# RayforceDB/rayforce

Measured on AMD Instinct MI355X. Metric: rows/s on filter→group-by→sum, 1e9-row i64/f64; % HBM roofline at 1/2/4/8 GPU, higher is better.
Workload: dtype f64

## Files before the change

### include/rfx_hip.h

```cpp
#ifndef RFX_HIP_H
#define RFX_HIP_H

#ifndef __HIPCC_RTC__
#include <stddef.h>
#endif
#include <stdint.h>

#ifdef __cplusplus
extern "C" {
#endif
#ifndef __HIPCC_RTC__
#pragma GCC visibility push(default)
#endif

enum {
    RFX_OK = 0,
    RFX_ENODEV = -1,
    RFX_EINVAL = -2,
    RFX_ENOMEM = -3,
    RFX_EHIP = -4,
    RFX_ELIMIT = -5,
    RFX_ESTATE = -6
};

enum { RFX_B8 = 1, RFX_I64 = 5, RFX_F64 = 10 };

enum { RFX_EQ = 0, RFX_NE = 1, RFX_LT = 2, RFX_GT = 3, RFX_LE = 4, RFX_GE = 5 };

enum { RFX_AND = 0, RFX_OR = 1 };

enum {
    RFX_AGG_SUM = 0,
    RFX_AGG_MIN = 1,
    RFX_AGG_MAX = 2,
    RFX_AGG_COUNT = 3,
    RFX_AGG_AVG = 4,
    RFX_AGG_FIRST = 5
};

#define RFX_MAX_PREDS 8
#define RFX_MAX_AGGS 8
#define RFX_MAX_COLS 8
#define RFX_MAX_KEYS 8
#define RFX_MAX_EXPRS 4

#define RFX_PRED_TREE 256
#define RFX_PRED_LEAF(depth, close) (RFX_PRED_TREE | (depth) | ((close) << 4))
typedef struct rfx_pred {
    const void *d_col;
    const void *d_rhs_col;
    int32_t col_type;
    int32_t rhs_type;
    int32_t op;
    int32_t more;
    union {
        int64_t rhs_i;
        double rhs_f;
    };
} rfx_pred_t;

enum { RFX_X_NONE = 0, RFX_X_ADD = 1, RFX_X_SUB = 2, RFX_X_MUL = 3, RFX_X_FDIV = 4, RFX_X_DIV = 5, RFX_X_MOD = 6 };
#define RFX_XOP_RESULT_F64(op, l_f64, r_f64) ((op) == RFX_X_FDIV ? 1 : ((op) == RFX_X_DIV ? ((l_f64) != 0) : ((l_f64) || (r_f64))))
enum { RFX_XF_SWAP = 1 };

#define RFX_MAX_XNODES 4
enum { RFX_XK_COL = 0, RFX_XK_ATOM = 1, RFX_XK_NODE = 2 };
typedef struct rfx_xoperand {
    int32_t kind;
    int32_t type;
    const void *d_col;
    union {
        int64_t i;
        double f;
        int64_t node;
    };
} rfx_xoperand_t;
typedef struct rfx_xnode {
    int32_t op;
    int32_t _pad;
    rfx_xoperand_t l, r;
} rfx_xnode_t;

typedef struct rfx_agg {
    const void *d_col;
    int32_t col_type;
    int32_t kind;
    int32_t xop;
    int32_t xflags;
    const void *d_xrhs_col;
    int32_t xrhs_type;
    int32_t nxnodes;
    union {
        int64_t xrhs_i;
        double xrhs_f;
    };
    const rfx_xnode_t *xnodes;
} rfx_agg_t;
int rfx_agg_input_type(const rfx_agg_t *a);

typedef struct rfx_partial {
    int64_t isum;
    double fsum;
    int64_t cnt;
    int64_t ext;
    int64_t pos;
    int64_t _rsv[3];
} rfx_partial_t;

typedef struct rfx_value {
    int32_t type;
    int32_t is_null;
    union {
        int64_t i;
        double f;
    };
} rfx_value_t;

typedef struct rfx_ctx rfx_ctx_t;

int rfx_hip_device_count(void);
const char *rfx_hip_last_error(void);
const char *rfx_hip_version(void);
#define RFX_STREAM_LEGACY ((void *)(uintptr_t)1)
int rfx_hip_ctx_create(int device, void *stream, rfx_ctx_t **out);
int rfx_hip_ctx_destroy(rfx_ctx_t *ctx);
int rfx_hip_ctx_sync(rfx_ctx_t *ctx);
int rfx_hip_ctx_set_stream(rfx_ctx_t *ctx, void *stream);
enum {
    RFX_TUNE_NO_LDS_TABLES = 1,
    RFX_TUNE_NO_PARTITION = 2,
    RFX_TUNE_NO_BIG_LDS = 4,
    RFX_TUNE_PART_3WG = 8,
    RFX_TUNE_NO_WRITE_COMBINE = 16,
    RFX_TUNE_DIRECT_WC = 32,
    RFX_TUNE_FUSED_KEYS = 64,
    RFX_TUNE_NO_FUSED_SCOPE = 128,
    RFX_TUNE_NO_SOA_WC = 2048,
    RFX_TUNE_NO_LDS_SPLIT = 1024,
    RFX_TUNE_NO_EMIT_WC = 512,
    RFX_TUNE_NO_SEL_COMPACT = 256,
    RFX_TUNE_NO_DEEP_GROUP = 4096,
    RFX_TUNE_NO_LDS_REPLICAS = 8192,
    RFX_TUNE_NO_CHUNK = 16384,
    RFX_TUNE_CHUNK_SMALL = 32768,
    RFX_TUNE_CHUNK_CONTIG = 65536,
    RFX_TUNE_CHUNK_QUEUE = 131072,
    RFX_TUNE_CHUNK_BINS = 262144,
    RFX_TUNE_NO_RTC = 524288,
    RFX_TUNE_NO_PLANE = 1048576,
    RFX_TUNE_NO_WHERE_ONCE = 2097152
};
int rfx_hip_ctx_tune(rfx_ctx_t *ctx, int blocks_per_cu, int flags);
enum {
    RFX_STAT_PLANE_SCATTER = 0,
    RFX_STAT_PLANE_FALLBACK = 1,
    RFX_STAT_PLANE_AGGREGATE = 2,
    RFX_STAT_CHUNK_SCATTER = 3,
    RFX_STAT_CHUNK_AGGREGATE = 4,
    RFX_STAT_MASK_PASSES = 5,
    RFX_STAT_WHERE_ONCE = 6
};
int64_t rfx_hip_ctx_stat(rfx_ctx_t *ctx, int which);

int rfx_hip_malloc(rfx_ctx_t *ctx, void **d_ptr, size_t bytes);
int rfx_hip_free(rfx_ctx_t *ctx, void *d_ptr);
int rfx_hip_ctx_trim(rfx_ctx_t *ctx);
int rfx_hip_h2d(rfx_ctx_t *ctx, void *d_dst, const void *src, size_t bytes);
int rfx_hip_d2h(rfx_ctx_t *ctx, void *dst, const void *d_src, size_t bytes);
int rfx_hip_d2h_async(rfx_ctx_t *ctx, void *dst, const void *d_src, size_t bytes);
int rfx_hip_memset(rfx_ctx_t *ctx, void *d_dst, int byte, size_t bytes);
int rfx_hip_fill_i64(rfx_ctx_t *ctx, int64_t *d_dst, int64_t n, int64_t value);
void rfx_hip_rtc_stats(int64_t *launches, int64_t *compiles);
void rfx_hip_rtc_cache_stats(int64_t *loaded_from_disk, int64_t *written_to_disk);
int rfx_hip_rtc_prewarm_filter_aggr(const rfx_pred_t *preds, int npred, int logic, const rfx_agg_t *aggs, int nagg);
int rfx_hip_rtc_prewarm_where(const rfx_pred_t *preds, int npred, int logic);

int rfx_hip_h2d_pipelined(rfx_ctx_t *ctx, void *d_dst, const void *src, size_t bytes);
int rfx_hip_d2h_pipelined(rfx_ctx_t *ctx, void *dst, const void *d_src, size_t bytes);
int rfx_column_file_stat(const char *path, int32_t *type, int64_t *len);
int rfx_hip_column_file_load(rfx_ctx_t *ctx, const char *path, void *d_dst, int64_t nrows);
int rfx_hip_widen_i32(rfx_ctx_t *ctx, const int32_t *d_in, int64_t n, int64_t *d_out);
int rfx_hip_widen_b8(rfx_ctx_t *ctx, const int8_t *d_in, int64_t n, int64_t *d_out);

int rfx_hip_timer_start(rfx_ctx_t *ctx);
int rfx_hip_timer_stop(rfx_ctx_t *ctx, float *ms);
int rfx_hip_ctx_profile(rfx_ctx_t *ctx, int enable);
int rfx_hip_last_kernel_ms(rfx_ctx_t *ctx, float *ms);
int rfx_hip_profile_kernels(rfx_ctx_t *ctx, float *ms, int cap, int *n);

int rfx_hip_gen_i64(rfx_ctx_t *ctx, int64_t *d_out, int64_t n, uint64_t seed, int64_t row0, uint64_t modulus);
int rfx_hip_gen_f64(rfx_ctx_t *ctx, double *d_out, int64_t n, uint64_t seed, int64_t row0);

int rfx_hip_filter_aggr(rfx_ctx_t *ctx, const rfx_pred_t *preds, int npred, int logic, const rfx_agg_t *aggs,
                        int nagg, int64_t nrows, int64_t row0, rfx_partial_t *d_out);
void rfx_partial_merge(int kind, int col_type, rfx_partial_t *into, const rfx_partial_t *from);
void rfx_partial_identity(rfx_partial_t *p);
int rfx_agg_finalize(int kind, int col_type, const rfx_partial_t *p, rfx_value_t *out);
int rfx_hip_filter_aggr_host(rfx_ctx_t *ctx, const rfx_pred_t *preds, int npred, int logic, const rfx_agg_t *aggs,
                             int nagg, int64_t nrows, rfx_value_t *values, int64_t *selected);

int rfx_hip_cmp_mask(rfx_ctx_t *ctx, const rfx_pred_t *pred, int64_t nrows, int8_t *d_mask);
int rfx_hip_mask_logic(rfx_ctx_t *ctx, int logic, int8_t *d_acc, const int8_t *d_next, int scalar, int64_t nrows);

int rfx_hip_where_begin(rfx_ctx_t *ctx, const rfx_pred_t *preds, int npred, int logic, const int8_t *d_mask,
                        int64_t nrows, int64_t *count);
int rfx_hip_where_emit(rfx_ctx_t *ctx, int64_t row0, int64_t *d_ids);
int rfx_hip_where_estimate(rfx_ctx_t *ctx, const rfx_pred_t *preds, int npred, int logic, int64_t nrows, int64_t *upper);
int rfx_hip_where_once(rfx_ctx_t *ctx, const rfx_pred_t *preds, int npred, int logic, int64_t nrows, int64_t row0, int64_t *d_ids,
                       int64_t cap, int64_t *count);

int rfx_hip_gather(rfx_ctx_t *ctx, const void *d_col, const int64_t *d_ids, int64_t m, void *d_out);
int rfx_hip_gather_many(rfx_ctx_t *ctx, const void *const *d_cols, int ncols, const int64_t *d_ids, int64_t m, void *const *d_outs);
int rfx_hip_gather_checked(rfx_ctx_t *ctx, const void *d_col, int64_t col_len, int32_t col_type, const int64_t *d_ids, int64_t m, void *d_out);

int rfx_hip_scope_i64(rfx_ctx_t *ctx, const int64_t *d_key, const rfx_pred_t *preds, int npred, int logic,
                      int64_t nrows, int64_t *min, int64_t *max, int64_t *count);

int rfx_hip_group_scope(rfx_ctx_t *ctx, const int64_t *d_key, const rfx_pred_t *preds, int npred, int logic,
                        const rfx_agg_t *aggs, int nagg, int64_t nrows, int64_t *min, int64_t *max, int64_t *count);

typedef struct rfx_group_tables {
    int64_t kmin;
    int64_t range;
    int32_t nagg;
    int32_t _pad;
    int64_t *d_first;
    void *d_acc[RFX_MAX_AGGS];
    int64_t *d_cnt[RFX_MAX_AGGS];
} rfx_group_tables_t;

int rfx_hip_group_table_arrays(const rfx_agg_t *aggs, int nagg, int *n_arrays);
int rfx_hip_group_tables_init(rfx_ctx_t *ctx, const rfx_agg_t *aggs, const rfx_group_tables_t *t);
int rfx_hip_group_dense_accumulate(rfx_ctx_t *ctx, const int64_t *d_key, const rfx_pred_t *preds, int npred,
                                   int logic, const rfx_agg_t *aggs, int64_t nrows, int64_t row0,
                                   const rfx_group_tables_t *t);
int rfx_hip_group_rank(rfx_ctx_t *ctx, const rfx_group_tables_t *t, int64_t total_rows, int64_t *ngroups);
#define RFX_SCOPE_SAMPLE_ROWS (1 << 18)
#define RFX_SCOPE_SAMPLE_MAX_RANGE 16384
int rfx_hip_scope_sample_i64(rfx_ctx_t *ctx, const int64_t *d_key, int64_t nrows, int64_t *min, int64_t *max);
int rfx_hip_ctx_speculative(rfx_ctx_t *ctx, int on);
int rfx_hip_group_out_of_scope(rfx_ctx_t *ctx, int *violated);
#define RFX_RANK_SMALL 2048
int rfx_hip_group_rank_emit_small(rfx_ctx_t *ctx, const rfx_agg_t *aggs, const rfx_group_tables_t *t, int64_t row0, int64_t local_rows, int64_t *d_block);
int rfx_hip_group_emit(rfx_ctx_t *ctx, const rfx_agg_t *aggs, const rfx_group_tables_t *t, int64_t *d_keys,
                       int64_t *d_first_ids, void *const *d_results);
int rfx_hip_group_emit_sharded(rfx_ctx_t *ctx, const rfx_agg_t *aggs, const rfx_group_tables_t *t, int64_t row0, int64_t local_rows,
                               int64_t *d_keys, int64_t *d_first_ids, void *const *d_results);
#define RFX_RANK_EMIT_MAX (1 << 22)
#define RFX_SLICE_G0(g, i, nsl) ((int64_t)(i) * ((g) / (nsl)) + ((int64_t)(i) < (g) % (nsl) ? (int64_t)(i) : (g) % (nsl)))
#define RFX_SLICE_GN(g, i, nsl) ((g) / (nsl) + ((int64_t)(i) < (g) % (nsl) ? 1 : 0))
int rfx_hip_group_rank_emit(rfx_ctx_t *ctx, const rfx_agg_t *aggs, const rfx_group_tables_t *t, int64_t total_rows, int64_t row0, int64_t local_rows,
                            int nsl, int si, int64_t out_cap, int64_t *d_keys, int64_t *d_first_ids, void *const *d_results, int64_t *ngroups);
int rfx_hip_ctx_emit_window(rfx_ctx_t *ctx, int64_t g0, int64_t n);

typedef struct rfx_hash_tables {
    int64_t capacity;
    int32_t nagg;
    int32_t _pad;
    int64_t *d_keys;
    int64_t *d_first;
    void *d_acc[RFX_MAX_AGGS];
    int64_t *d_cnt[RFX_MAX_AGGS];
} rfx_hash_tables_t;
int rfx_hip_hash_tables_init(rfx_ctx_t *ctx, const rfx_agg_t *aggs, const rfx_hash_tables_t *t);
int rfx_hip_group_hash_accumulate(rfx_ctx_t *ctx, const int64_t *d_key, const rfx_pred_t *preds, int npred, int logic,
                                  const rfx_agg_t *aggs, int64_t nrows, int64_t row0, const rfx_hash_tables_t *t);
int rfx_hip_group_hash_accumulate_slots(rfx_ctx_t *ctx, const int64_t *d_key, const rfx_pred_t *preds, int npred, int logic, const rfx_agg_t *aggs, int64_t nrows,
                                        int64_t row0, const rfx_hash_tables_t *t, int64_t *d_row_slots, int *recorded);
int rfx_hip_hash_slot_first(rfx_ctx_t *ctx, const rfx_hash_tables_t *t, const int64_t *d_row_slots, int64_t nrows, int64_t *d_ids);
int rfx_hip_hash_tables_init_packed(rfx_ctx_t *ctx, const rfx_agg_t *aggs, const rfx_hash_tables_t *t, int stride);
int rfx_hip_group_hash_accumulate_packed(rfx_ctx_t *ctx, const int64_t *d_key, const rfx_pred_t *preds, int npred, int logic, const rfx_agg_t *aggs, int64_t nrows,
                                         int64_t row0, const rfx_hash_tables_t *t, int stride, int64_t *d_row_slots);
int rfx_hip_hash_tables_merge(rfx_ctx_t *ctx, const rfx_agg_t *aggs, const rfx_hash_tables_t *into,
                              const rfx_hash_tables_t *from);
int rfx_hip_hash_rank(rfx_ctx_t *ctx, const rfx_hash_tables_t *t, int64_t total_rows, int64_t *ngroups);
int rfx_hip_hash_emit(rfx_ctx_t *ctx, const rfx_agg_t *aggs, const rfx_hash_tables_t *t, int64_t *d_keys,
                      int64_t *d_first_ids, void *const *d_results);
int rfx_hip_hash_emit_sharded(rfx_ctx_t *ctx, const rfx_agg_t *aggs, const rfx_hash_tables_t *t, int64_t row0, int64_t local_rows,
                              int64_t *d_keys, int64_t *d_first_ids, void *const *d_results);
int rfx_hip_hash_rows_begin(rfx_ctx_t *ctx, const int64_t *d_probe_first, int64_t nrows, int64_t *ngroups);
int rfx_hip_hash_rows_emit(rfx_ctx_t *ctx, const rfx_agg_t *aggs, const rfx_hash_tables_t *t, const int64_t *d_row_slots, const int64_t *d_row_keys, int64_t row0,
                           int64_t local_rows, int64_t ngroups, int64_t *d_keys, int64_t *d_first_ids, void *const *d_results);
int rfx_hip_hash_rank_emit(rfx_ctx_t *ctx, const rfx_agg_t *aggs, const rfx_hash_tables_t *t, int64_t total_rows, int64_t row0, int64_t local_rows,
                           int nsl, int si, int64_t out_cap, int64_t *d_keys, int64_t *d_first_ids, void *const *d_results, int64_t *ngroups);

int rfx_hip_group_ids_dense(rfx_ctx_t *ctx, const int64_t *d_key, int64_t nrows, const rfx_group_tables_t *t,
                            int64_t *d_gids);
int rfx_hip_group_ids_table(rfx_ctx_t *ctx, const int64_t *d_key, int64_t nrows, int64_t kmin, int64_t range, const int64_t *d_table, int64_t *d_gids);

int rfx_hip_group_ids_first(rfx_ctx_t *ctx, const int64_t *d_probe_first, int64_t nrows, const int64_t *d_first, int64_t groups, int64_t *d_gids);
int rfx_hip_group_slot_ids(rfx_ctx_t *ctx, const rfx_group_tables_t *t, int64_t *d_out);

int rfx_composite_plan(const int64_t *mins, const int64_t *maxs, int nkeys, int64_t *mults, int64_t *total_max);
int rfx_hip_composite_key(rfx_ctx_t *ctx, const void *const *d_cols, const int64_t *mins, const int64_t *mults, int nkeys,
                          int64_t nrows, int64_t *d_out);
int rfx_hip_composite_decode(rfx_ctx_t *ctx, const int64_t *d_comp, int64_t n, int64_t min, int64_t mult, int64_t range,
                             int64_t *d_out);
int rfx_hip_group_dense_accumulate_keys(rfx_ctx_t *ctx, const void *const *d_keys, const int64_t *mins, const int64_t *mults,
                                        int nkeys, const rfx_pred_t *preds, int npred, int logic, const rfx_agg_t *aggs,
                                        int64_t nrows, int64_t row0, const rfx_group_tables_t *t);

int rfx_hip_row_hash(rfx_ctx_t *ctx, const void *const *d_cols, int nkeys, int64_t nrows, int value_first, int64_t *d_out);
int rfx_hip_replace_null_i64(rfx_ctx_t *ctx, const int64_t *d_col, int64_t nrows, int64_t repl, int64_t *d_out);
int rfx_hip_replace_i64(rfx_ctx_t *ctx, const int64_t *d_col, int64_t nrows, int64_t from, int64_t to, int64_t *d_out);

int rfx_hip_eval_expr(rfx_ctx_t *ctx, const rfx_agg_t *expr, int64_t nrows, void *d_out, int32_t *out_type);

int rfx_hip_join_probe_dense(rfx_ctx_t *ctx, const int64_t *d_left_keys, int64_t nleft, int64_t kmin, int64_t range, const int64_t *d_first,
                             int64_t *d_ids);
int rfx_hip_join_probe_hash(rfx_ctx_t *ctx, const int64_t *d_left_keys, int64_t nleft, const rfx_hash_tables_t *t, int64_t *d_ids);
int rfx_hip_join_probe_hash_slots(rfx_ctx_t *ctx, const int64_t *d_left_keys, int64_t nleft, const rfx_hash_tables_t *t, int64_t *d_ids, int64_t *d_slots);
int rfx_hip_tuple_check(rfx_ctx_t *ctx, const void *const *d_keys, int nk, const int64_t *d_first_of_row, int64_t nrows, int64_t *differ);
int rfx_hip_gather_or(rfx_ctx_t *ctx, const void *d_right, const void *d_left, const int64_t *d_ids, int64_t n, uint64_t fill_bits, void *d_out);

#define RFX_DIST_ID_BYTES 128
int rfx_dist_unique_id(void *id128);
int rfx_dist_init(rfx_ctx_t *ctx, int world, int rank, const void *id128);
int rfx_dist_finalize(rfx_ctx_t *ctx);
int rfx_dist_world(rfx_ctx_t *ctx, int *world, int *rank);
int rfx_dist_scope(rfx_ctx_t *ctx, int64_t *kmin, int64_t *kmax, int64_t *seen);
int rfx_dist_group_tables_allreduce(rfx_ctx_t *ctx, const rfx_agg_t *aggs, const rfx_group_tables_t *t);
int rfx_dist_partials_allgather(rfx_ctx_t *ctx, const rfx_partial_t *d_local, int n, rfx_partial_t *d_all);
int rfx_dist_filter_aggr_host(rfx_ctx_t *ctx, const rfx_pred_t *preds, int npred, int logic, const rfx_agg_t *aggs, int nagg,
                              int64_t nrows, int64_t row0, rfx_value_t *values, int64_t *selected);
int rfx_dist_allreduce_i64(rfx_ctx_t *ctx, int64_t *d_buf, int64_t n, int op);
int rfx_dist_allgather(rfx_ctx_t *ctx, const void *d_in, size_t bytes, void *d_out);
int64_t rfx_dist_calls(rfx_ctx_t *ctx);

// ... 52 lines not shown
```

### rayforce_amd/_lib.py

```python
from __future__ import annotations

import ctypes as C
import os

RFX_OK = 0
RFX_ELIMIT = -5
RFX_ESTATE = -6
RFX_B8, RFX_I64, RFX_F64 = 1, 5, 10
RFX_EQ, RFX_NE, RFX_LT, RFX_GT, RFX_LE, RFX_GE = range(6)
RFX_AND, RFX_OR = 0, 1
RFX_AGG_SUM, RFX_AGG_MIN, RFX_AGG_MAX, RFX_AGG_COUNT, RFX_AGG_AVG, RFX_AGG_FIRST = range(6)
RFX_MAX_PREDS = RFX_MAX_AGGS = RFX_MAX_COLS = RFX_MAX_KEYS = 8
RFX_RANK_SMALL = 2048
RFX_MAX_EXPRS = 4
NULL_I64 = -(2**63)
INF_I64 = 2**63 - 1

OPS = {"==": RFX_EQ, "!=": RFX_NE, "<": RFX_LT, ">": RFX_GT, "<=": RFX_LE, ">=": RFX_GE}
AGGS = {"sum": RFX_AGG_SUM, "min": RFX_AGG_MIN, "max": RFX_AGG_MAX, "count": RFX_AGG_COUNT, "avg": RFX_AGG_AVG,
        "first": RFX_AGG_FIRST}


class RfxError(RuntimeError):
    pass
# ... 7 lines not shown
    _anonymous_ = ("u",)
    _fields_ = [("d_col", C.c_void_p), ("d_rhs_col", C.c_void_p), ("col_type", C.c_int32), ("rhs_type", C.c_int32),
                ("op", C.c_int32), ("more", C.c_int32), ("u", _RhsUnion)]


class _XRhsUnion(C.Union):
    _fields_ = [("xrhs_i", C.c_int64), ("xrhs_f", C.c_double)]


class _XOpUnion(C.Union):
    _fields_ = [("i", C.c_int64), ("f", C.c_double), ("node", C.c_int64)]


class XOperand(C.Structure):
    _anonymous_ = ("u",)
    _fields_ = [("kind", C.c_int32), ("type", C.c_int32), ("d_col", C.c_void_p), ("u", _XOpUnion)]


class XNode(C.Structure):
    _fields_ = [("op", C.c_int32), ("_pad", C.c_int32), ("l", XOperand), ("r", XOperand)]


class Agg(C.Structure):
    _anonymous_ = ("xu",)
    _fields_ = [("d_col", C.c_void_p), ("col_type", C.c_int32), ("kind", C.c_int32), ("xop", C.c_int32), ("xflags", C.c_int32),
                ("d_xrhs_col", C.c_void_p), ("xrhs_type", C.c_int32), ("nxnodes", C.c_int32), ("xu", _XRhsUnion), ("xnodes", C.POINTER(XNode))]


RFX_XK_COL, RFX_XK_ATOM, RFX_XK_NODE = 0, 1, 2
RFX_MAX_XNODES = 4
XOPS = {"+": 1, "-": 2, "*": 3, "div": 4, "/": 5, "%": 6}
RFX_XF_SWAP = 1


def agg_input_type(a: "Agg") -> int:
    if a.xop == 0 and a.nxnodes == 0:
        return a.col_type
    return load_library().rfx_agg_input_type(C.byref(a))


class Partial(C.Structure):
    _fields_ = [("isum", C.c_int64), ("fsum", C.c_double), ("cnt", C.c_int64), ("ext", C.c_int64), ("pos", C.c_int64),
                ("_rsv", C.c_int64 * 3)]


class _ValUnion(C.Union):
    _fields_ = [("i", C.c_int64), ("f", C.c_double)]


RFX_MED_GROUPED, RFX_MED_SCALAR = 0, 1


class MedRows(C.Structure):
    _fields_ = [("preds", C.c_void_p), ("npred", C.c_int32), ("logic", C.c_int32), ("d_mask", C.c_void_p), ("d_gids", C.c_void_p),
                ("d_key", C.c_void_p), ("d_table", C.c_void_p), ("kmin", C.c_int64), ("range", C.c_int64)]


class Value(C.Structure):
    _anonymous_ = ("u",)
    _fields_ = [("type", C.c_int32), ("is_null", C.c_int32), ("u", _ValUnion)]


class GroupTables(C.Structure):
    _fields_ = [("kmin", C.c_int64), ("range", C.c_int64), ("nagg", C.c_int32), ("_pad", C.c_int32),
                ("d_first", C.c_void_p), ("d_acc", C.c_void_p * RFX_MAX_AGGS), ("d_cnt", C.c_void_p * RFX_MAX_AGGS)]


class HashTables(C.Structure):
    _fields_ = [("capacity", C.c_int64), ("nagg", C.c_int32), ("_pad", C.c_int32), ("d_keys", C.c_void_p),
                ("d_first", C.c_void_p), ("d_acc", C.c_void_p * RFX_MAX_AGGS), ("d_cnt", C.c_void_p * RFX_MAX_AGGS)]


assert C.sizeof(Pred) == 40 and C.sizeof(Agg) == 56 and C.sizeof(XNode) == 56 and C.sizeof(Partial) == 64 and C.sizeof(Value) == 16

RFX_MAX_SHARDS = 16
RFX_EXEC_MAX_AGGS = 32
RFX_PRED_TREE = 256
RFX_Q_NO_SAMPLED_SCOPE, RFX_Q_REFUSE_NULL_KEY, RFX_Q_WANT_FIRST, RFX_Q_NO_SMALL, RFX_Q_PROBE_FIRST, RFX_Q_SLICED = 1, 2, 4, 8, 16, 32
RFX_PATH_DENSE, RFX_PATH_DENSE_SMALL, RFX_PATH_HASH, RFX_PATH_ROWHASH = 1, 2, 3, 4
RFX_XSTAT_SCOPE_SAMPLED, RFX_XSTAT_SCOPE_RETRIED, RFX_XSTAT_SCOPE_REMEMBERED, RFX_XSTAT_HASH_GROWN, RFX_XSTAT_MERGES_KERNEL, RFX_XSTAT_MERGES_RCCL, \
    RFX_XSTAT_MERGES_TRANSPORT, RFX_XSTAT_QUERIES, RFX_XSTAT_SLICED, RFX_XSTAT_NS_SCOPE, RFX_XSTAT_NS_PASS, RFX_XSTAT_NS_MERGE, RFX_XSTAT_NS_RANK, \
    RFX_XSTAT_NS_EMIT, RFX_XSTAT_NS_FETCH, RFX_XSTAT_NS_TOTAL = range(16)
RFX_XSTAT_PHASES = (("scope", 9), ("pass", 10), ("merge", 11), ("rank", 12), ("emit", 13), ("fetch", 14), ("total", 15))


class QCol(C.Structure):
    _fields_ = [("d", C.c_void_p * RFX_MAX_SHARDS)]


class Query(C.Structure):
    _fields_ = [("preds", C.POINTER(Pred)), ("npred", C.c_int32), ("logic", C.c_int32), ("d_mask", C.c_void_p), ("aggs", C.POINTER(Agg)),
                ("nagg", C.c_int32), ("nkeys", C.c_int32), ("d_keys", C.POINTER(C.c_void_p)), ("kxbar", C.POINTER(C.c_int64)), ("nrows", C.c_int64),
                ("cols", C.POINTER(QCol)), ("ncols", C.c_int32), ("flags", C.c_int32), ("key_scope", C.POINTER(C.c_int64)), ("row0", C.c_int64),
                ("d_sel_ids", C.POINTER(C.c_void_p)), ("sel_count", C.POINTER(C.c_int64))]


class Ids(C.Structure):
    _fields_ = [("nshards", C.c_int32), ("total", C.c_int64), ("count", C.c_int64 * RFX_MAX_SHARDS), ("d_ids", C.c_void_p * RFX_MAX_SHARDS)]


class GSlice(C.Structure):
    _fields_ = [("shard", C.c_int32), ("g0", C.c_int64), ("n", C.c_int64), ("d_keys", C.c_void_p), ("d_first", C.c_void_p),
                ("d_keycols", C.c_void_p * RFX_MAX_KEYS), ("d_results", C.c_void_p * RFX_EXEC_MAX_AGGS)]


_GROUPS_OWN = RFX_MAX_SHARDS * (4 + 2 * RFX_MAX_KEYS + RFX_EXEC_MAX_AGGS)


class Groups(C.Structure):
    _fields_ = [("groups", C.c_int64), ("path", C.c_int32), ("nkeys", C.c_int32), ("nagg", C.c_int32), ("d_keys", C.c_void_p),
                ("d_keycols", C.c_void_p * RFX_MAX_KEYS), ("d_first", C.c_void_p), ("d_results", C.c_void_p * RFX_EXEC_MAX_AGGS),
                ("result_type", C.c_int32 * RFX_EXEC_MAX_AGGS), ("d_probe", C.c_void_p), ("capacity", C.c_int64), ("d_block", C.c_void_p),
                ("h_block", C.c_void_p), ("block_bytes", C.c_size_t), ("own", C.c_void_p * _GROUPS_OWN), ("own_shard", C.c_int8 * _GROUPS_OWN), ("nown", C.c_int32),
                ("nslices", C.c_int32), ("slice", GSlice * RFX_MAX_SHARDS)]


TR_WORLD_RANK = C.CFUNCTYPE(C.c_int, C.c_void_p, C.POINTER(C.c_int), C.POINTER(C.c_int))
TR_ALLGATHER_HOST = C.CFUNCTYPE(C.c_int, C.c_void_p, C.c_void_p, C.c_size_t, C.c_void_p)
TR_ALLREDUCE = C.CFUNCTYPE(C.c_int, C.c_void_p, C.c_void_p, C.c_int64, C.c_int, C.c_int)
TR_ALLGATHER_DEV = C.CFUNCTYPE(C.c_int, C.c_void_p, C.c_void_p, C.c_size_t, C.c_void_p)


class Transport(C.Structure):
    _fields_ = [("user", C.c_void_p), ("world_rank", TR_WORLD_RANK), ("allgather_host", TR_ALLGATHER_HOST), ("allreduce", TR_ALLREDUCE),
                ("allgather_dev", TR_ALLGATHER_DEV)]


_P = C.POINTER
_ctx = C.c_void_p

PROTOTYPES = {
    "rfx_hip_device_count": (C.c_int, []),
    "rfx_hip_last_error": (C.c_char_p, []),
    "rfx_hip_version": (C.c_char_p, []),
    "rfx_hip_ctx_create": (C.c_int, [C.c_int, C.c_void_p, _P(_ctx)]),
    "rfx_hip_ctx_destroy": (C.c_int, [_ctx]),
    "rfx_hip_ctx_sync": (C.c_int, [_ctx]),
    "rfx_hip_ctx_set_stream": (C.c_int, [_ctx, C.c_void_p]),
    "rfx_hip_ctx_tune": (C.c_int, [_ctx, C.c_int, C.c_int]),
    "rfx_hip_ctx_stat": (C.c_int64, [_ctx, C.c_int]),
    "rfx_hip_malloc": (C.c_int, [_ctx, _P(C.c_void_p), C.c_size_t]),
    "rfx_hip_free": (C.c_int, [_ctx, C.c_void_p]),
    "rfx_hip_ctx_trim": (C.c_int, [_ctx]),
    "rfx_hip_h2d": (C.c_int, [_ctx, C.c_void_p, C.c_void_p, C.c_size_t]),
    "rfx_hip_d2h": (C.c_int, [_ctx, C.c_void_p, C.c_void_p, C.c_size_t]),
    "rfx_hip_d2h_async": (C.c_int, [_ctx, C.c_void_p, C.c_void_p, C.c_size_t]),
    "rfx_hip_d2h_pipelined": (C.c_int, [_ctx, C.c_void_p, C.c_void_p, C.c_size_t]),
    "rfx_hip_memset": (C.c_int, [_ctx, C.c_void_p, C.c_int, C.c_size_t]),
    "rfx_hip_fill_i64": (C.c_int, [_ctx, C.c_void_p, C.c_int64, C.c_int64]),
    "rfx_hip_rtc_stats": (None, [_P(C.c_int64), _P(C.c_int64)]),
    "rfx_hip_rtc_cache_stats": (None, [_P(C.c_int64), _P(C.c_int64)]),
    "rfx_hip_rtc_prewarm_filter_aggr": (C.c_int, [_P(Pred), C.c_int, C.c_int, _P(Agg), C.c_int]),
    "rfx_hip_rtc_prewarm_where": (C.c_int, [_P(Pred), C.c_int, C.c_int]),
    "rfx_hip_timer_start": (C.c_int, [_ctx]),
    "rfx_hip_timer_stop": (C.c_int, [_ctx, _P(C.c_float)]),
    "rfx_hip_ctx_profile": (C.c_int, [_ctx, C.c_int]),
    "rfx_hip_last_kernel_ms": (C.c_int, [_ctx, _P(C.c_float)]),
    "rfx_hip_profile_kernels": (C.c_int, [_ctx, _P(C.c_float), C.c_int, _P(C.c_int)]),
    "rfx_hip_gen_i64": (C.c_int, [_ctx, C.c_void_p, C.c_int64, C.c_uint64, C.c_int64, C.c_uint64]),
    "rfx_hip_gen_f64": (C.c_int, [_ctx, C.c_void_p, C.c_int64, C.c_uint64, C.c_int64]),
    "rfx_hip_filter_aggr": (C.c_int, [_ctx, _P(Pred), C.c_int, C.c_int, _P(Agg), C.c_int, C.c_int64, C.c_int64, C.c_void_p]),
    "rfx_partial_merge": (None, [C.c_int, C.c_int, _P(Partial), _P(Partial)]),
    "rfx_partial_identity": (None, [_P(Partial)]),
    "rfx_agg_finalize": (C.c_int, [C.c_int, C.c_int, _P(Partial), _P(Value)]),
    "rfx_hip_filter_aggr_host": (C.c_int, [_ctx, _P(Pred), C.c_int, C.c_int, _P(Agg), C.c_int, C.c_int64, _P(Value), _P(C.c_int64)]),
    "rfx_hip_cmp_mask": (C.c_int, [_ctx, _P(Pred), C.c_int64, C.c_void_p]),
    "rfx_hip_mask_logic": (C.c_int, [_ctx, C.c_int, C.c_void_p, C.c_void_p, C.c_int, C.c_int64]),
    "rfx_hip_where_begin": (C.c_int, [_ctx, _P(Pred), C.c_int, C.c_int, C.c_void_p, C.c_int64, _P(C.c_int64)]),
    "rfx_hip_where_emit": (C.c_int, [_ctx, C.c_int64, C.c_void_p]),
    "rfx_hip_widen_i32": (C.c_int, [_ctx, C.c_void_p, C.c_int64, C.c_void_p]),
    "rfx_hip_widen_b8": (C.c_int, [_ctx, C.c_void_p, C.c_int64, C.c_void_p]),
    "rfx_hip_where_estimate": (C.c_int, [_ctx, _P(Pred), C.c_int, C.c_int, C.c_int64, _P(C.c_int64)]),
    "rfx_hip_where_once": (C.c_int, [_ctx, _P(Pred), C.c_int, C.c_int, C.c_int64, C.c_int64, C.c_void_p, C.c_int64, _P(C.c_int64)]),
    "rfx_hip_gather": (C.c_int, [_ctx, C.c_void_p, C.c_void_p, C.c_int64, C.c_void_p]),
    "rfx_hip_gather_many": (C.c_int, [_ctx, _P(C.c_void_p), C.c_int, C.c_void_p, C.c_int64, _P(C.c_void_p)]),
    "rfx_hip_gather_checked": (C.c_int, [_ctx, C.c_void_p, C.c_int64, C.c_int32, C.c_void_p, C.c_int64, C.c_void_p]),
    "rfx_hip_scope_i64": (C.c_int, [_ctx, C.c_void_p, _P(Pred), C.c_int, C.c_int, C.c_int64, _P(C.c_int64), _P(C.c_int64), _P(C.c_int64)]),
    "rfx_hip_group_scope": (C.c_int, [_ctx, C.c_void_p, _P(Pred), C.c_int, C.c_int, _P(Agg), C.c_int, C.c_int64, _P(C.c_int64), _P(C.c_int64), _P(C.c_int64)]),
    "rfx_hip_group_table_arrays": (C.c_int, [_P(Agg), C.c_int, _P(C.c_int)]),
    "rfx_hip_group_tables_init": (C.c_int, [_ctx, _P(Agg), _P(GroupTables)]),
    "rfx_hip_group_dense_accumulate": (C.c_int, [_ctx, C.c_void_p, _P(Pred), C.c_int, C.c_int, _P(Agg), C.c_int64, C.c_int64, _P(GroupTables)]),
    "rfx_hip_group_rank": (C.c_int, [_ctx, _P(GroupTables), C.c_int64, _P(C.c_int64)]),
    "rfx_hip_group_emit": (C.c_int, [_ctx, _P(Agg), _P(GroupTables), C.c_void_p, C.c_void_p, _P(C.c_void_p)]),
    "rfx_hip_scope_sample_i64": (C.c_int, [_ctx, C.c_void_p, C.c_int64, _P(C.c_int64), _P(C.c_int64)]),
    "rfx_hip_ctx_speculative": (C.c_int, [_ctx, C.c_int]),
    "rfx_hip_ctx_emit_window": (C.c_int, [_ctx, C.c_int64, C.c_int64]),
    "rfx_hip_group_rank_emit": (C.c_int, [_ctx, _P(Agg), _P(GroupTables), C.c_int64, C.c_int64, C.c_int64, C.c_int, C.c_int, C.c_int64, C.c_void_p, C.c_void_p,
                                          _P(C.c_void_p), _P(C.c_int64)]),
    "rfx_hip_hash_rank_emit": (C.c_int, [_ctx, _P(Agg), _P(HashTables), C.c_int64, C.c_int64, C.c_int64, C.c_int, C.c_int, C.c_int64, C.c_void_p, C.c_void_p,
                                         _P(C.c_void_p), _P(C.c_int64)]),
    "rfx_hip_group_out_of_scope": (C.c_int, [_ctx, _P(C.c_int)]),
    "rfx_hip_group_rank_emit_small": (C.c_int, [_ctx, _P(Agg), _P(GroupTables), C.c_int64, C.c_int64, C.c_void_p]),
    "rfx_hip_group_emit_sharded": (C.c_int, [_ctx, _P(Agg), _P(GroupTables), C.c_int64, C.c_int64, C.c_void_p, C.c_void_p, _P(C.c_void_p)]),
    "rfx_hip_hash_emit_sharded": (C.c_int, [_ctx, _P(Agg), _P(HashTables), C.c_int64, C.c_int64, C.c_void_p, C.c_void_p, _P(C.c_void_p)]),
    "rfx_hip_hash_tables_init": (C.c_int, [_ctx, _P(Agg), _P(HashTables)]),
    "rfx_hip_group_hash_accumulate": (C.c_int, [_ctx, C.c_void_p, _P(Pred), C.c_int, C.c_int, _P(Agg), C.c_int64, C.c_int64, _P(HashTables)]),
    "rfx_hip_group_hash_accumulate_slots": (C.c_int, [_ctx, C.c_void_p, _P(Pred), C.c_int, C.c_int, _P(Agg), C.c_int64, C.c_int64, _P(HashTables), C.c_void_p, _P(C.c_int)]),
    "rfx_hip_hash_slot_first": (C.c_int, [_ctx, _P(HashTables), C.c_void_p, C.c_int64, C.c_void_p]),
    "rfx_hip_hash_tables_init_packed": (C.c_int, [_ctx, _P(Agg), _P(HashTables), C.c_int]),
    "rfx_hip_group_hash_accumulate_packed": (C.c_int, [_ctx, C.c_void_p, _P(Pred), C.c_int, C.c_int, _P(Agg), C.c_int64, C.c_int64, _P(HashTables), C.c_int, C.c_void_p]),
    "rfx_hip_hash_tables_merge": (C.c_int, [_ctx, _P(Agg), _P(HashTables), _P(HashTables)]),
    "rfx_hip_hash_rank": (C.c_int, [_ctx, _P(HashTables), C.c_int64, _P(C.c_int64)]),
    "rfx_hip_hash_emit": (C.c_int, [_ctx, _P(Agg), _P(HashTables), C.c_void_p, C.c_void_p, _P(C.c_void_p)]),
    "rfx_hip_group_slot_ids": (C.c_int, [_ctx, _P(GroupTables), C.c_void_p]),
    "rfx_hip_group_ids_dense": (C.c_int, [_ctx, C.c_void_p, C.c_int64, _P(GroupTables), C.c_void_p]),
    "rfx_hip_group_ids_table": (C.c_int, [_ctx, C.c_void_p, C.c_int64, C.c_int64, C.c_int64, C.c_void_p, C.c_void_p]),
    "rfx_hip_group_ids_first": (C.c_int, [_ctx, C.c_void_p, C.c_int64, C.c_void_p, C.c_int64, C.c_void_p]),
    "rfx_hip_update_set": (C.c_int, [_ctx, C.c_void_p, C.c_void_p, C.c_int64, C.c_void_p, C.c_uint64]),
    "rfx_hip_update_select": (C.c_int, [_ctx, C.c_void_p, C.c_void_p, C.c_uint64, C.c_void_p, C.c_void_p, C.c_uint64, C.c_int64]),
    "rfx_hip_absmax_f64": (C.c_int, [_ctx, C.c_void_p, C.c_int64, _P(C.c_double), _P(C.c_int)]),
    "rfx_hip_fix_f64": (C.c_int, [_ctx, C.c_void_p, C.c_int64, C.c_int, C.c_void_p]),
    "rfx_hip_fix_f64_low": (C.c_int, [_ctx, C.c_void_p, C.c_int64, C.c_int, C.c_int, C.c_void_p]),
    "rfx_hip_unfix_f64": (C.c_int, [_ctx, C.c_void_p, C.c_void_p, C.c_void_p, C.c_int64, C.c_double, C.c_double]),
    "rfx_hip_update_group": (C.c_int, [_ctx, C.c_void_p, C.c_void_p, C.c_void_p, C.c_int64, _P(Agg), _P(GroupTables)]),
    "rfx_dist_unique_id": (C.c_int, [C.c_void_p]),
    "rfx_dist_init": (C.c_int, [_ctx, C.c_int, C.c_int, C.c_void_p]),
    "rfx_dist_finalize": (C.c_int, [_ctx]),
    "rfx_dist_world": (C.c_int, [_ctx, _P(C.c_int), _P(C.c_int)]),
    "rfx_dist_scope": (C.c_int, [_ctx, _P(C.c_int64), _P(C.c_int64), _P(C.c_int64)]),
    "rfx_dist_group_tables_allreduce": (C.c_int, [_ctx, _P(Agg), _P(GroupTables)]),
    "rfx_dist_partials_allgather": (C.c_int, [_ctx, C.c_void_p, C.c_int, C.c_void_p]),
    "rfx_dist_filter_aggr_host": (C.c_int, [_ctx, _P(Pred), C.c_int, C.c_int, _P(Agg), C.c_int, C.c_int64, C.c_int64, _P(Value), _P(C.c_int64)]),
    "rfx_dist_allreduce_i64": (C.c_int, [_ctx, C.c_void_p, C.c_int64, C.c_int]),
    "rfx_dist_allgather": (C.c_int, [_ctx, C.c_void_p, C.c_size_t, C.c_void_p]),
    "rfx_dist_calls": (C.c_int64, [_ctx]),
    "rfx_hip_hash_fnv1a_i64": (C.c_int, [_ctx, C.c_void_p, C.c_int64, C.c_void_p]),
    "rfx_hip_hash_mix_u64": (C.c_int, [_ctx, C.c_void_p, C.c_int64, C.c_uint64, C.c_void_p]),
    "rfx_agg_input_type": (C.c_int, [_P(Agg)]),
    "rfx_hip_xbar_i64": (C.c_int, [_ctx, C.c_void_p, C.c_int64, C.c_int64, C.c_void_p]),
    "rfx_hip_group_median": (C.c_int, [_ctx, _P(MedRows), C.c_void_p, C.c_int32, C.c_int64, C.c_int64, C.c_int32, C.c_void_p]),
    "rfx_hip_median": (C.c_int, [_ctx, C.c_void_p, C.c_int, C.c_int, C.c_void_p, C.c_void_p, C.c_int64, _P(Value)]),
    "rfx_hip_median_keys": (C.c_int, [_ctx, C.c_void_p, C.c_int32, C.c_int64, C.c_void_p]),
    "rfx_hip_key_slot_table": (C.c_int, [_ctx, C.c_void_p, C.c_int64, C.c_int64, C.c_int64, C.c_void_p]),
    "rfx_hip_eval_expr": (C.c_int, [_ctx, _P(Agg), C.c_int64, C.c_void_p, _P(C.c_int32)]),
    "rfx_hip_join_probe_dense": (C.c_int, [_ctx, C.c_void_p, C.c_int64, C.c_int64, C.c_int64, C.c_void_p, C.c_void_p]),
    "rfx_hip_join_probe_hash": (C.c_int, [_ctx, C.c_void_p, C.c_int64, _P(HashTables), C.c_void_p]),
    "rfx_hip_join_probe_hash_slots": (C.c_int, [_ctx, C.c_void_p, C.c_int64, C.c_void_p, C.c_void_p, C.c_void_p]),
    "rfx_hip_tuple_check": (C.c_int, [_ctx, _P(C.c_void_p), C.c_int, C.c_void_p, C.c_int64, _P(C.c_int64)]),
    "rfx_hip_hash_rows_begin": (C.c_int, [_ctx, C.c_void_p, C.c_int64, _P(C.c_int64)]),
    "rfx_hip_hash_rows_emit": (C.c_int, [_ctx, C.c_void_p, C.c_void_p, C.c_void_p, C.c_void_p, C.c_int64, C.c_int64, C.c_int64, C.c_void_p, C.c_void_p, _P(C.c_void_p)]),
    "rfx_hip_gather_or": (C.c_int, [_ctx, C.c_void_p, C.c_void_p, C.c_void_p, C.c_int64, C.c_uint64, C.c_void_p]),
    "rfx_hip_row_hash": (C.c_int, [_ctx, C.POINTER(C.c_void_p), C.c_int, C.c_int64, C.c_int, C.c_void_p]),
    "rfx_hip_replace_null_i64": (C.c_int, [_ctx, C.c_void_p, C.c_int64, C.c_int64, C.c_void_p]),
    "rfx_hip_replace_i64": (C.c_int, [_ctx, C.c_void_p, C.c_int64, C.c_int64, C.c_int64, C.c_void_p]),
    "rfx_hip_h2d_pipelined": (C.c_int, [_ctx, C.c_void_p, C.c_void_p, C.c_size_t]),
    "rfx_column_file_stat": (C.c_int, [C.c_char_p, C.POINTER(C.c_int32), C.POINTER(C.c_int64)]),
    "rfx_hip_column_file_load": (C.c_int, [_ctx, C.c_char_p, C.c_void_p, C.c_int64]),
    "rfx_composite_plan": (C.c_int, [C.POINTER(C.c_int64), C.POINTER(C.c_int64), C.c_int, C.POINTER(C.c_int64), C.POINTER(C.c_int64)]),
    "rfx_hip_composite_key": (C.c_int, [_ctx, C.POINTER(C.c_void_p), C.POINTER(C.c_int64), C.POINTER(C.c_int64), C.c_int, C.c_int64, C.c_void_p]),
    "rfx_hip_group_dense_accumulate_keys": (C.c_int, [_ctx, C.POINTER(C.c_void_p), C.POINTER(C.c_int64), C.POINTER(C.c_int64), C.c_int, _P(Pred),
                                                      C.c_int, C.c_int, _P(Agg), C.c_int64, C.c_int64, _P(GroupTables)]),
    "rfx_hip_composite_decode": (C.c_int, [_ctx, C.c_void_p, C.c_int64, C.c_int64, C.c_int64, C.c_int64, C.c_void_p]),
    "rfx_dist_init_all": (C.c_int, [_P(_ctx), C.c_int]),
    "rfx_dist_is_local": (C.c_int, [_ctx]),
    "rfx_dist_has_comm": (C.c_int, [_ctx]),
    "rfx_dist_group_tables_allreduce_all": (C.c_int, [_P(_ctx), C.c_int, _P(Agg), _P(_P(GroupTables))]),
    "rfx_dist_allreduce_i64_all": (C.c_int, [_P(_ctx), C.c_int, _P(C.c_void_p), C.c_int64, C.c_int]),
    "rfx_dist_allgather_all": (C.c_int, [_P(_ctx), C.c_int, _P(C.c_void_p), C.c_size_t, _P(C.c_void_p)]),
    "rfx_dist_allgather_host": (C.c_int, [_ctx, C.c_void_p, C.c_size_t, C.c_void_p]),
    "rfx_hip_group_tables_merge": (C.c_int, [_ctx, _P(Agg), _P(GroupTables), _P(GroupTables)]),
    "rfx_hip_add_i64": (C.c_int, [_ctx, C.c_void_p, C.c_void_p, C.c_int64]),
    "rfx_hip_d2d": (C.c_int, [_ctx, C.c_void_p, C.c_void_p, C.c_size_t]),
    "rfx_hip_ctx_bind_thread": (C.c_int, [_ctx]),
    "rfx_hip_ctx_device": (C.c_int, [_ctx]),
}

_exec = C.c_void_p
EXEC_PROTOTYPES = {
    "rfx_exec_create": (C.c_int, [_P(_ctx), C.c_int, _P(_exec)]),
    "rfx_exec_destroy": (C.c_int, [_exec]),
    "rfx_exec_shards": (C.c_int, [_exec]),
    "rfx_exec_ctx": (_ctx, [_exec, C.c_int]),
    "rfx_exec_split": (None, [C.c_int64, C.c_int, C.c_int, _P(C.c_int64), _P(C.c_int64)]),
    "rfx_exec_comm_init_all": (C.c_int, [_exec]),
    "rfx_exec_set_transport": (C.c_int, [_exec, _P(Transport)]),
    "rfx_exec_ranks": (C.c_int, [_exec, _P(C.c_int)]),
    "rfx_exec_groups_window": (C.c_int, [_P(Groups), C.c_int64, C.c_int64, _P(Groups)]),
    "rfx_exec_allgather_host": (C.c_int, [_exec, C.c_void_p, C.c_size_t, C.c_void_p]),
    "rfx_exec_filter_aggr": (C.c_int, [_exec, _P(Query), _P(Value), _P(C.c_int64)]),
    "rfx_exec_where": (C.c_int, [_exec, _P(Query), _P(Ids)]),
    "rfx_exec_ids_free": (None, [_exec, _P(Ids)]),
    "rfx_exec_group_by": (C.c_int, [_exec, _P(Query), _P(Groups)]),
    "rfx_exec_groups_fetch": (C.c_int, [_exec, _P(Groups), C.c_void_p, C.c_void_p, C.c_size_t]),
    "rfx_exec_groups_fetch_all": (C.c_int, [_exec, _P(Groups), C.c_int, _P(C.c_void_p), _P(C.c_void_p)]),
    "rfx_exec_groups_free": (None, [_exec, _P(Groups)]),
    "rfx_exec_timing": (None, [_exec, C.c_int]),
    "rfx_exec_probe_handover_us": (C.c_double, [C.c_int, C.c_int]),
    "rfx_exec_median": (C.c_int, [_exec, C.c_void_p, C.c_void_p, C.c_int32, _P(Value)]),
    "rfx_exec_group_median": (C.c_int, [_exec, C.c_void_p, C.c_void_p, C.c_void_p, C.c_int32, C.c_void_p]),
    "rfx_exec_join_index": (C.c_int, [_exec, _P(C.c_void_p), _P(C.c_void_p), C.c_int, C.c_int64, C.c_int64, C.c_void_p, _P(C.c_int)]),
    "rfx_exec_join_index_shard": (C.c_int, [_exec, C.c_int, _P(C.c_void_p), _P(C.c_void_p), C.c_int, C.c_int64, C.c_int64, C.c_void_p, _P(C.c_int)]),
    "rfx_exec_stat": (C.c_int64, [_exec, C.c_int]),
    "rfx_exec_run": (C.c_int, [_exec, C.c_void_p, C.c_void_p]),
    "rfx_exec_forget_scopes": (None, [_exec]),
    "rfx_exec_last_error": (C.c_char_p, [_exec]),
}
PROTOTYPES.update(EXEC_PROTOTYPES)

_LIB = None


def lib_path() -> str:
    return os.environ.get("RFX_LIB") or os.path.join(os.path.dirname(os.path.abspath(__file__)), "librfx.so")


def load_library() -> C.CDLL:
# ... 27 lines not shown
```

### rayforce_amd/csrc/rfx_common.hpp

```cpp
#pragma once
#ifndef __HIPCC_RTC__
#include <hip/hip_runtime.h>
#include <stdio.h>
#include <string.h>
#endif
#include <stdint.h>
#include "../../include/rfx_hip.h"

#define RFX_WAVE 64
#define RFX_BLOCK 256
#define RFX_NULL_I64_D ((int64_t)0x8000000000000000LL)
#define RFX_INF_I64_D ((int64_t)0x7FFFFFFFFFFFFFFFLL)
#define RFX_NAN_BITS 0x7FF8000000000000ULL
#define RFX_PINF_BITS 0x7FF0000000000000ULL

typedef unsigned long long u64;
typedef long long i64;

#ifndef __HIPCC_RTC__
void rfx_set_error(const char *fmt, ...);

#define RFX_HIP_CHECK(expr)                                                                       \
    do {                                                                                          \
        hipError_t _e = (expr);                                                                   \
        if (_e != hipSuccess) {                                                                   \
            rfx_set_error("%s:%d: %s -> %s", __FILE__, __LINE__, #expr, hipGetErrorString(_e));   \
            return (_e == hipErrorOutOfMemory) ? RFX_ENOMEM : RFX_EHIP;                           \
        }                                                                                         \
    } while (0)

#define RFX_REQUIRE(cond, code, msg)                      \
    do {                                                  \
        if (!(cond)) {                                    \
            rfx_set_error("%s: %s", __func__, msg);       \
            return (code);                                \
        }                                                 \
    } while (0)

struct rfx_ctx {
    int device;
    hipStream_t stream;
    bool own_stream;
    int num_cus;
    int blocks_per_cu;
    int flags;
    hipEvent_t ev0, ev1;
    hipEvent_t evk[8][2];
    int evk_n;
    int profile;
    int evk_valid;
    void *d_ws;
    size_t ws_bytes;
    void *h_pin;
    size_t pin_bytes;
    u64 *d_bitmap;
    size_t bitmap_cap;
    i64 *d_blksum;
    size_t blksum_cap;
    i64 where_n;
    i64 where_count;
    i64 rank_rows;
    i64 rank_groups;
    i64 *d_gid;
    size_t gid_cap;
    void *d_part;
    size_t part_bytes;
    void *d_comp;
    size_t comp_bytes;
    void *io_stage[4];
    hipEvent_t io_done[4];
    void *d_expr;
    size_t expr_bytes;
    void *d_sel;
    size_t sel_bytes;
    u64 *d_pc_counts;
    int pc_valid, pc_npred, pc_logic, pc_nwg;
    int pc_bitmap;
    const void *pc_key;
    i64 pc_nrows;
    i64 pc_seen;
    u64 pc_sig[RFX_MAX_PREDS][6];
    void *d_chunk;
    size_t chunk_bytes;
    int ck_valid, ck_npred, ck_logic, ck_nwg, ck_chs;
    const void *ck_key, *ck_val;
    i64 ck_nrows, ck_tpw;
    size_t ck_max_chunks;
    u64 ck_sig[RFX_MAX_PREDS][6];
    void *comm;
    int world, rank;
    void *d_dist;
    size_t dist_bytes;
    i64 dist_calls;
    void *ext_p[8];
    i64 ext_i[8];
};

struct CtxExt {
    i64 emit_g0, emit_gn;
    i64 spare[30];
};
static inline CtxExt *rfx_ext(rfx_ctx *c) { return (CtxExt *)c->ext_p[7]; }

int rfx_ws_reserve(rfx_ctx *ctx, size_t bytes);
int rfx_bitmap_reserve(rfx_ctx *ctx, i64 nrows);
int rfx_gid_reserve(rfx_ctx *ctx, i64 slots);
int rfx_part_reserve(rfx_ctx *ctx, size_t bytes);
int rfx_comp_reserve(rfx_ctx *ctx, size_t bytes);
int rfx_expr_reserve(rfx_ctx *ctx, size_t bytes);
void rfx_io_release(rfx_ctx *ctx);
int rfx_sel_reserve(rfx_ctx *ctx, size_t bytes);
int rfx_chunk_reserve(rfx_ctx *ctx, size_t bytes);
int rfx_plan_add_col(struct Plan *P, const void *col);
#define RFX_KERNEL_BEGIN(c) do { if ((c)->profile) { (void)hipEventRecord((c)->evk[(c)->evk_n & 7][0], (c)->stream); } } while (0)
#define RFX_KERNEL_END(c) do { if ((c)->profile) { (void)hipEventRecord((c)->evk[(c)->evk_n & 7][1], (c)->stream); (c)->evk_n++; (c)->evk_valid = 1; } } while (0)
static inline int rfx_grid(const rfx_ctx *ctx) { return ctx->num_cus * ctx->blocks_per_cu; }
int rfx_rtc_filter_aggr(rfx_ctx *c, const struct Plan &P, int grid, void *ws, int *na_stride);
#else
struct rfx_ctx;
#endif

struct PlanPred {
    int col;
    int rhs_col;
    int op;
    int dom_f64;
    int lhs_cvt;
    int rhs_cvt;
    u64 rhs_bits;
    int more;
    int tree;
};
#define RFX_XCOL 64
struct PlanAgg {
    int col;
    int f64;
    int kind;
    int skipnull;
};
struct PlanXNode {
    int op;
    int o_f64;
    int l_kind, r_kind;
    int l_idx, r_idx;
    int l_f64, r_f64;
    u64 l_atom, r_atom;
};
struct PlanExpr {
    int nops;
    int out_f64;
    PlanXNode ops[RFX_MAX_XNODES];
};
struct Plan {
    int ncols, npred, nagg, logic;
    const u64 *cols[RFX_MAX_COLS];
    PlanPred preds[RFX_MAX_PREDS];
    PlanAgg aggs[RFX_MAX_AGGS];
    i64 nrows;
    i64 row0;
    int nx, _pad;
    PlanExpr xs[RFX_MAX_EXPRS];
};
int rfx_plan_materialise_exprs(rfx_ctx *c, Plan *P);
static inline bool rfx_plan_has_deep_expr(const Plan &P) {
    for (int i = 0; i < P.nx; i++)
        if (P.xs[i].nops > 1) return true;
    return false;
}

int rfx_plan_build(Plan *P, const rfx_pred_t *preds, int npred, int logic, const rfx_agg_t *aggs, int nagg,
                   const void *extra_col, int *extra_idx, i64 nrows, i64 row0);

__device__ __forceinline__ double rfx_as_f64(u64 b) { return __longlong_as_double((i64)b); }
__device__ __forceinline__ u64 rfx_as_u64(double d) { return (u64)__double_as_longlong(d); }

__device__ __forceinline__ bool rfx_isnan_bits(u64 u) {
    return (u & 0x7FF0000000000000ULL) == 0x7FF0000000000000ULL && (u & 0x000FFFFFFFFFFFFFULL) != 0;
}
__device__ __forceinline__ u64 rfx_i64_to_f64_bits(u64 x) {
    return ((i64)x == RFX_NULL_I64_D) ? RFX_NAN_BITS : rfx_as_u64((double)(i64)x);
}

__device__ __forceinline__ u64 rfx_expr_eval(int op, int out_f64, int l_f64, int r_f64, u64 lx, u64 rx) {
    if (op >= RFX_X_DIV) {
        if (!l_f64 && !r_f64) {
            const i64 x = (i64)lx, y = (i64)rx;
            if (y == 0 || x == RFX_NULL_I64_D || y == RFX_NULL_I64_D) return (u64)RFX_NULL_I64_D;
            i64 q = x / y;
            if (((x < 0) != (y < 0)) && q * y != x) q -= 1;
            return op == RFX_X_DIV ? (u64)q : (u64)(x - q * y);
        }
        const u64 lb = l_f64 ? lx : rfx_i64_to_f64_bits(lx), rb = r_f64 ? rx : rfx_i64_to_f64_bits(rx);
        const double a = rfx_as_f64(lb), b = rfx_as_f64(rb);
        double r = 0.0;
        bool null = b == 0.0 || rfx_isnan_bits(lb) || rfx_isnan_bits(rb);
        if (!null) {
            const double q = floor(a / b);
            r = op == RFX_X_DIV ? q : fma(-q, b, a);
            null = rfx_isnan_bits(rfx_as_u64(r));
        }
        if (out_f64) return null ? RFX_NAN_BITS : rfx_as_u64(r);
        if (null || !(r > -9223372036854775808.0 && r < 9223372036854775808.0)) return (u64)RFX_NULL_I64_D;
        return (u64)(i64)r;
    }
    if (!out_f64) {
        if ((i64)lx == RFX_NULL_I64_D || (i64)rx == RFX_NULL_I64_D) return (u64)RFX_NULL_I64_D;
        return op == RFX_X_ADD ? lx + rx : (op == RFX_X_SUB ? lx - rx : lx * rx);
    }
    const u64 lb = l_f64 ? lx : rfx_i64_to_f64_bits(lx), rb = r_f64 ? rx : rfx_i64_to_f64_bits(rx);
    if (rfx_isnan_bits(lb) || rfx_isnan_bits(rb)) return RFX_NAN_BITS;
    const double a = rfx_as_f64(lb), b = rfx_as_f64(rb);
    double r;
    switch (op) {
        case RFX_X_ADD: r = a + b; break;
        case RFX_X_SUB: r = a - b; break;
        case RFX_X_MUL: r = a * b; break;
        default:
            if (b == 0.0) return RFX_NAN_BITS;
            r = a / b;
            break;
    }
    return rfx_as_u64(r);
}

__device__ __forceinline__ bool rfx_cmp_i64(int op, i64 x, i64 y) {
    switch (op) {
        case RFX_EQ: return x == y;
        case RFX_NE: return x != y;
        case RFX_LT: return x < y;
        case RFX_GT: return x > y;
        case RFX_LE: return x <= y;
        default: return x >= y;
    }
}
__device__ __forceinline__ bool rfx_ltf64(u64 xb, u64 yb) {
    bool xn = rfx_isnan_bits(xb), yn = rfx_isnan_bits(yb);
    return xn ? !yn : (yn ? false : rfx_as_f64(xb) < rfx_as_f64(yb));
}
__device__ __forceinline__ bool rfx_gtf64(u64 xb, u64 yb) {
    bool xn = rfx_isnan_bits(xb), yn = rfx_isnan_bits(yb);
    return yn ? !xn : (xn ? false : rfx_as_f64(xb) > rfx_as_f64(yb));
}
__device__ __forceinline__ bool rfx_eqf64(u64 xb, u64 yb) {
    bool xn = rfx_isnan_bits(xb), yn = rfx_isnan_bits(yb);
    return xn ? yn : (yn ? false : rfx_as_f64(xb) == rfx_as_f64(yb));
}
__device__ __forceinline__ bool rfx_cmp_f64(int op, u64 x, u64 y) {
    switch (op) {
        case RFX_EQ: return rfx_eqf64(x, y);
        case RFX_NE: return !rfx_eqf64(x, y);
        case RFX_LT: return rfx_ltf64(x, y);
        case RFX_GT: return rfx_gtf64(x, y);
        case RFX_LE: return !rfx_gtf64(x, y);
// ... 28 lines not shown
```

### rayforce_amd/csrc/rfx_ctx.hip

```cpp
#include <pthread.h>
#include "rfx_common.hpp"
#include <stdarg.h>
#include <stdlib.h>

static thread_local char g_err[512] = "";

void rfx_set_error(const char *fmt, ...) {
    va_list ap;
    va_start(ap, fmt);
    vsnprintf(g_err, sizeof(g_err), fmt, ap);
    va_end(ap);
}

extern "C" const char *rfx_hip_last_error(void) { return g_err; }
extern "C" const char *rfx_hip_version(void) { return "rfx-hip 0.1 (gfx950)"; }

extern "C" int rfx_hip_device_count(void) {
    int n = 0;
    if (hipGetDeviceCount(&n) != hipSuccess) return 0;
    return n;
}

extern "C" int rfx_hip_ctx_create(int device, void *stream, rfx_ctx_t **out) {
    RFX_REQUIRE(out != NULL, RFX_EINVAL, "out is NULL");
    int n = 0;
    if (hipGetDeviceCount(&n) != hipSuccess || n <= 0) {
        rfx_set_error("no HIP device visible (hipGetDeviceCount failed or returned 0) -- the MI355X path has no CPU fallback");
        return RFX_ENODEV;
    }
    RFX_REQUIRE(device >= 0 && device < n, RFX_EINVAL, "device ordinal out of range");
    RFX_HIP_CHECK(hipSetDevice(device));
    hipDeviceProp_t prop;
    RFX_HIP_CHECK(hipGetDeviceProperties(&prop, device));
    rfx_ctx *c = (rfx_ctx *)calloc(1, sizeof(rfx_ctx));
    RFX_REQUIRE(c != NULL, RFX_ENOMEM, "host calloc failed");
    c->device = device;
    c->ext_p[7] = calloc(1, sizeof(CtxExt));
    RFX_REQUIRE(c->ext_p[7] != NULL, RFX_ENOMEM, "host calloc failed");
    c->num_cus = prop.multiProcessorCount > 0 ? prop.multiProcessorCount : 256;
    c->blocks_per_cu = 2;
    if (stream) {
        c->stream = (stream == RFX_STREAM_LEGACY) ? (hipStream_t)0 : (hipStream_t)stream;
        c->own_stream = false;
    } else {
        RFX_HIP_CHECK(hipStreamCreateWithFlags(&c->stream, hipStreamNonBlocking));
        c->own_stream = true;
    }
    RFX_HIP_CHECK(hipEventCreate(&c->ev0));
    RFX_HIP_CHECK(hipEventCreate(&c->ev1));
    for (int i = 0; i < 8; i++) {
        RFX_HIP_CHECK(hipEventCreate(&c->evk[i][0]));
        RFX_HIP_CHECK(hipEventCreate(&c->evk[i][1]));
    }
    c->pin_bytes = 1 << 16;
    RFX_HIP_CHECK(hipHostMalloc(&c->h_pin, c->pin_bytes, hipHostMallocDefault));
    int rc = rfx_ws_reserve(c, 4u << 20);
    if (rc != RFX_OK) return rc;
    *out = c;
    return RFX_OK;
}

static void pool_release(rfx_ctx *c);
void rfx_plane_release(rfx_ctx *c);
void rfx_plane_invalidate(rfx_ctx *c);
extern "C" int rfx_hip_ctx_destroy(rfx_ctx_t *c) {
    if (!c) return RFX_OK;
    (void)hipSetDevice(c->device);
    (void)hipStreamSynchronize(c->stream);
    (void)rfx_dist_finalize(c);
    if (c->d_dist) (void)hipFree(c->d_dist);
    if (c->d_ws) (void)hipFree(c->d_ws);
    if (c->d_bitmap) (void)hipFree(c->d_bitmap);
    if (c->d_blksum) (void)hipFree(c->d_blksum);
    if (c->d_gid) (void)hipFree(c->d_gid);
    if (c->d_part) (void)hipFree(c->d_part);
    if (c->d_comp) (void)hipFree(c->d_comp);
    if (c->d_sel) (void)hipFree(c->d_sel);
    if (c->d_expr) (void)hipFree(c->d_expr);
    if (c->d_chunk) (void)hipFree(c->d_chunk);
    rfx_io_release(c);
    pool_release(c);
    if (c->ext_p[1]) (void)hipFree(c->ext_p[1]);
    free(c->ext_p[7]);
    free(c->ext_p[5]);
    free(c->ext_p[6]);
    rfx_plane_release(c);
    if (c->d_pc_counts) (void)hipFree(c->d_pc_counts);
    if (c->h_pin) (void)hipHostFree(c->h_pin);
    (void)hipEventDestroy(c->ev0);
    (void)hipEventDestroy(c->ev1);
    for (int i = 0; i < 8; i++) {
        (void)hipEventDestroy(c->evk[i][0]);
        (void)hipEventDestroy(c->evk[i][1]);
    }
    if (c->own_stream) (void)hipStreamDestroy(c->stream);
    free(c);
    return RFX_OK;
}

extern "C" int64_t rfx_hip_ctx_stat(rfx_ctx_t *c, int which) {
    if (!c || which < 0 || which > 6) return -1;
    if (which == 6) return (int64_t)(uintptr_t)c->ext_p[4];
    return which == RFX_STAT_MASK_PASSES ? c->ext_i[0] : c->ext_i[3 + which];
}

extern "C" int rfx_hip_ctx_sync(rfx_ctx_t *c) {
    RFX_REQUIRE(c, RFX_EINVAL, "ctx is NULL");
    RFX_HIP_CHECK(hipStreamSynchronize(c->stream));
    return RFX_OK;
}

extern "C" int rfx_hip_ctx_set_stream(rfx_ctx_t *c, void *stream) {
    RFX_REQUIRE(c, RFX_EINVAL, "ctx is NULL");
    RFX_REQUIRE(stream, RFX_EINVAL, "stream is NULL");
    if (c->own_stream) {
        (void)hipStreamSynchronize(c->stream);
        (void)hipStreamDestroy(c->stream);
        c->own_stream = false;
    }
    c->stream = (stream == RFX_STREAM_LEGACY) ? (hipStream_t)0 : (hipStream_t)stream;
    return RFX_OK;
}

extern "C" int rfx_hip_ctx_tune(rfx_ctx_t *c, int blocks_per_cu, int flags) {
    RFX_REQUIRE(c, RFX_EINVAL, "ctx is NULL");
    if (blocks_per_cu > 0) {
        RFX_REQUIRE(blocks_per_cu <= 64, RFX_EINVAL, "blocks_per_cu > 64");
        c->blocks_per_cu = blocks_per_cu;
    }
    c->flags = flags;
    return RFX_OK;
}

int rfx_ws_reserve(rfx_ctx *c, size_t bytes) {
    if (c->ws_bytes >= bytes) return RFX_OK;
    RFX_HIP_CHECK(hipStreamSynchronize(c->stream));
    if (c->d_ws) RFX_HIP_CHECK(hipFree(c->d_ws));
    c->d_ws = NULL;
    c->ws_bytes = 0;
    RFX_HIP_CHECK(hipMalloc(&c->d_ws, bytes));
    c->ws_bytes = bytes;
    return RFX_OK;
}

int rfx_bitmap_reserve(rfx_ctx *c, i64 nrows) {
    size_t words = (size_t)((nrows + 63) / 64) + 64;
    size_t blocks = (size_t)((nrows + 2047) / 2048) + 2;
    if (c->bitmap_cap < words) {
        RFX_HIP_CHECK(hipStreamSynchronize(c->stream));
        if (c->d_bitmap) RFX_HIP_CHECK(hipFree(c->d_bitmap));
        c->d_bitmap = NULL;
        c->bitmap_cap = 0;
        RFX_HIP_CHECK(hipMalloc((void **)&c->d_bitmap, words * 8));
        c->bitmap_cap = words;
    }
    if (c->blksum_cap < blocks) {
        RFX_HIP_CHECK(hipStreamSynchronize(c->stream));
        if (c->d_blksum) RFX_HIP_CHECK(hipFree(c->d_blksum));
        c->d_blksum = NULL;
        c->blksum_cap = 0;
        RFX_HIP_CHECK(hipMalloc((void **)&c->d_blksum, blocks * 8));
        c->blksum_cap = blocks;
    }
    return RFX_OK;
}

int rfx_gid_reserve(rfx_ctx *c, i64 slots) {
    if (c->gid_cap >= (size_t)slots) return RFX_OK;
    RFX_HIP_CHECK(hipStreamSynchronize(c->stream));
    if (c->d_gid) RFX_HIP_CHECK(hipFree(c->d_gid));
    c->d_gid = NULL;
    c->gid_cap = 0;
    RFX_HIP_CHECK(hipMalloc((void **)&c->d_gid, (size_t)slots * 8));
    c->gid_cap = (size_t)slots;
    return RFX_OK;
}

int rfx_part_reserve(rfx_ctx *c, size_t bytes) {
    if (c->part_bytes >= bytes) return RFX_OK;
    RFX_HIP_CHECK(hipStreamSynchronize(c->stream));
    if (c->d_part) RFX_HIP_CHECK(hipFree(c->d_part));
    c->d_part = NULL;
    c->part_bytes = 0;
    RFX_HIP_CHECK(hipMalloc(&c->d_part, bytes));
    c->part_bytes = bytes;
    return RFX_OK;
}

int rfx_expr_reserve(rfx_ctx *c, size_t bytes) {
    if (c->expr_bytes >= bytes) return RFX_OK;
    RFX_HIP_CHECK(hipStreamSynchronize(c->stream));
    if (c->d_expr) RFX_HIP_CHECK(hipFree(c->d_expr));
    c->d_expr = NULL;
    c->expr_bytes = 0;
    RFX_HIP_CHECK(hipMalloc(&c->d_expr, bytes));
    c->expr_bytes = bytes;
    return RFX_OK;
}

int rfx_sel_reserve(rfx_ctx *c, size_t bytes) {
    if (c->sel_bytes >= bytes) return RFX_OK;
    RFX_HIP_CHECK(hipStreamSynchronize(c->stream));
    if (c->d_sel) RFX_HIP_CHECK(hipFree(c->d_sel));
    c->d_sel = NULL;
    c->sel_bytes = 0;
    RFX_HIP_CHECK(hipMalloc(&c->d_sel, bytes));
    c->sel_bytes = bytes;
    return RFX_OK;
}

int rfx_chunk_reserve(rfx_ctx *c, size_t bytes) {
    if (c->chunk_bytes >= bytes) return RFX_OK;
    RFX_HIP_CHECK(hipStreamSynchronize(c->stream));
    if (c->d_chunk) RFX_HIP_CHECK(hipFree(c->d_chunk));
    c->d_chunk = NULL;
    c->chunk_bytes = 0;
    RFX_HIP_CHECK(hipMalloc(&c->d_chunk, bytes));
    c->chunk_bytes = bytes;
    return RFX_OK;
}

int rfx_comp_reserve(rfx_ctx *c, size_t bytes) {
    if (c->comp_bytes >= bytes) return RFX_OK;
    RFX_HIP_CHECK(hipStreamSynchronize(c->stream));
    if (c->d_comp) RFX_HIP_CHECK(hipFree(c->d_comp));
    c->d_comp = NULL;
    c->comp_bytes = 0;
    RFX_HIP_CHECK(hipMalloc(&c->d_comp, bytes));
    c->comp_bytes = bytes;
    return RFX_OK;
}

struct DeriveArgs {
    PlanExpr x;
    const u64 *cols[RFX_MAX_COLS];
    u64 *out;
};
__device__ __forceinline__ u64 derive_operand(int kind, u64 colval, u64 atom, int idx, const u64 (&res)[RFX_MAX_XNODES]) {
    if (kind == RFX_XK_COL) return colval;
    if (kind == RFX_XK_ATOM) return atom;
    return res[idx];
}
__global__ __launch_bounds__(RFX_BLOCK) void k_derive(const DeriveArgs A, i64 nrows) {
    const i64 npairs = nrows / 2;
    const int nops = A.x.nops;
    for (i64 i = blockIdx.x * (i64)RFX_BLOCK + threadIdx.x; i < npairs; i += (i64)gridDim.x * RFX_BLOCK) {
        u64 r0[RFX_MAX_XNODES] = {0, 0, 0, 0}, r1[RFX_MAX_XNODES] = {0, 0, 0, 0};
        for (int k = 0; k < nops; k++) {
            const PlanXNode n = A.x.ops[k];
            u64x2 lc, rc;
            lc.x = lc.y = rc.x = rc.y = 0;
            if (n.l_kind == RFX_XK_COL) lc = rfx_ld2(A.cols[n.l_idx] + 2 * i);
            if (n.r_kind == RFX_XK_COL) rc = rfx_ld2(A.cols[n.r_idx] + 2 * i);
            r0[k] = rfx_expr_eval(n.op, n.o_f64, n.l_f64, n.r_f64, derive_operand(n.l_kind, lc.x, n.l_atom, n.l_idx, r0),
// ... 547 lines not shown
```

### rayforce_amd/csrc/rfx_group_plane.hip

```cpp
#include "rfx_part_common.hpp"
#include <stdlib.h>

#define PL_T 1024
#define PL_WAVES (PL_T / RFX_WAVE)
#define PL_WROWS 512
#define PL_BLOCK_ROWS (1 << 18)
#define PL_DELTA_BITS 18
#define PL_SLOT_BITS 14
#define PL_QCAP 320
#define PL_QFLUSH 24
#define PL_SPIN_LIMIT (1u << 14)
#define PL_MAX_NV 3
#ifndef PL_META64_PLAIN
#define PL_META64_PLAIN 1
#endif

struct PlaneArgs {
    int nblk;
    int nv;
    unsigned pmask;
    i64 block_rows;
    unsigned c0;
    u64 *vals[PL_MAX_NV];
    unsigned *meta;
    unsigned *cnt;
    unsigned *ctl;
};
struct PlSh {
    unsigned dead, _pad[3];
    i64 red[3][PL_WAVES];
};
template <int PBITS, int VGL, bool HK>
__host__ __device__ constexpr int pl_parts() { return (HK && PBITS == 8 && VGL == 4) ? 192 : (1 << PBITS); }
template <int NV, int PBITS, int VGL, bool HK = false>
__host__ __device__ constexpr size_t pl_lds_bytes() {
    return (size_t)pl_parts<PBITS, VGL, HK>() * ((size_t)(2 << VGL) * (NV * 8 + 4) + 8 + 4) + (size_t)PL_WAVES * PL_QCAP * 4 + sizeof(PlSh) + 64;
}
typedef u64 pl_v2 __attribute__((ext_vector_type(2)));
typedef unsigned pl_m2 __attribute__((ext_vector_type(2)));
#define PL_LD(ptr) __hip_atomic_load((ptr), __ATOMIC_RELAXED, __HIP_MEMORY_SCOPE_WORKGROUP)
#define PL_ST(ptr, v) __hip_atomic_store((ptr), (v), __ATOMIC_RELAXED, __HIP_MEMORY_SCOPE_WORKGROUP)

template <int NC, int NP, int NV, int PBITS, int VGL, bool HK = false>
__global__ __launch_bounds__(PL_T) void k_plane_scatter(const Plan P, const PlaneArgs A) {
    constexpr int PARTS = pl_parts<PBITS, VGL, HK>();
    constexpr bool P192 = PARTS != (1 << PBITS);
    constexpr unsigned VG = 1u << VGL, RING = 2u << VGL;
    constexpr bool KVI = HK && NV == 2 && PBITS == 8 && VGL == 3;
    constexpr unsigned LPD = VG / 2;
    extern __shared__ __attribute__((aligned(16))) unsigned char pl_smem[];
    u64 *vring = (u64 *)pl_smem;
    unsigned *mring = (unsigned *)(vring + (size_t)NV * PARTS * RING);
    unsigned *words = mring + (size_t)PARTS * RING;
    unsigned *tail = words + PARTS * 2;
    unsigned *fq = tail + PARTS;
    PlSh &L = *(PlSh *)(fq + PL_WAVES * PL_QCAP);
    PredSet<NP> S;
    predset_load<NP>(P, S);
    const int tid = threadIdx.x, lane = tid & 63, wv = tid >> 6;
    unsigned *myq = fq + wv * PL_QCAP;
    const i64 r0 = (i64)blockIdx.x * A.block_rows;
    const i64 r1 = (r0 + A.block_rows < P.nrows) ? r0 + A.block_rows : P.nrows;
    const u64 region = ((u64)blockIdx.x * (u64)PARTS) * A.c0;
    for (int i = tid; i < PARTS; i += PL_T) {
        tail[i] = 0;
        words[2 * i] = 0;
        words[2 * i + 1] = 0;
    }
    if (tid == 0) L.dead = 0;
    __syncthreads();
    i64 mn = RFX_INF_I64_D, mx = RFX_NULL_I64_D;
    unsigned nsel = 0;
    int qn = 0;

    auto flush_queue = [&]() __attribute__((always_inline)) {
        asm volatile("" ::: "memory");
        for (int i0 = 0; i0 < qn; i0 += 64 / (int)LPD) {
            const int idx = i0 + (lane / (int)LPD);
            if (idx < qn) {
                const unsigned d = myq[idx];
                const unsigned p = d & 0xFFu, gi = (d >> 8) & 0x3FFFFFu, pl = d >> 30, sub = lane & (LPD - 1u);
                if (pl < 3) {
                    const pl_v2 x = *(const pl_v2 *)(vring + ((size_t)pl * PARTS + p) * RING + (gi & 1u) * VG + sub * 2);
                    if constexpr (KVI) {
                        __builtin_nontemporal_store(x, (pl_v2 *)(A.vals[0] + 2 * (region + (u64)p * A.c0 + (u64)gi * VG) + (u64)pl * VG + sub * 2));
                    } else {
                        u64 *dst = (NV == 1 ? A.vals[0] : (pl == 0 ? A.vals[0] : (pl == 1 ? A.vals[1] : A.vals[2])));
                        __builtin_nontemporal_store(x, (pl_v2 *)(dst + region + (u64)p * A.c0 + (u64)gi * VG + sub * 2));
                    }
                } else if (sub < LPD / 2) {
                    const pl_v2 x = *(const pl_v2 *)(mring + (size_t)p * RING + (gi & 1u) * VG + sub * 4);
                    if constexpr (KVI || (VGL == 4 && PL_META64_PLAIN)) *(pl_v2 *)(A.meta + region + (u64)p * A.c0 + (u64)gi * VG + sub * 4) = x;
                    else __builtin_nontemporal_store(x, (pl_v2 *)(A.meta + region + (u64)p * A.c0 + (u64)gi * VG + sub * 4));
                }
            }
        }
        asm volatile("" ::: "memory");
        for (int i = lane; i < qn; i += 64) {
            const unsigned d = myq[i];
            if ((d >> 30) == 3u) atomicAdd(&words[2 * (d & 0xFFu) + ((d >> 8) & 1u)], 256u - VG);
        }
        qn = 0;
    };

    auto place = [&](const bool on, const u64 key, const u64 (&val)[NV], const unsigned delta) __attribute__((always_inline)) {
        const u64 kh = HK ? rfx_hash_index_u64(RFX_U64_HASH_SEED, key) : key;
        const unsigned p = P192 ? (unsigned)(((kh >> 32) * (u64)PARTS) >> 32) : (HK ? (unsigned)(kh >> (64 - PBITS)) : ((unsigned)key & (unsigned)(PARTS - 1)));
        unsigned seq = 0;
        if (on) {
            const i64 k = (i64)key;
            mn = k < mn ? k : mn;
            mx = k > mx ? k : mx;
            seq = atomicAdd(&tail[p], 1u);
            if (seq >= A.c0) PL_ST(&L.dead, 1u);
        }
        const unsigned g = seq >> VGL;
        unsigned *w = &words[2 * p + (g & 1u)];
        bool todo = on && seq < A.c0;
        for (unsigned it = 0;; it++) {
            bool ready = false;
            if (todo) ready = (PL_LD(w) >> 8) == (g >> 1);
            bool comp = false;
            if (ready) {
                const unsigned at = p * RING + (seq & (RING - 1u));
#pragma unroll
                for (int j = 0; j < NV; j++) vring[(size_t)j * PARTS * RING + at] = val[j];
                mring[at] = ((unsigned)(P192 ? (kh >> 18) : (HK ? (kh >> (64 - PBITS - PL_SLOT_BITS)) : (key >> PBITS))) & ((1u << PL_SLOT_BITS) - 1u)) | (delta << PL_SLOT_BITS);
                asm volatile("" ::: "memory");
                comp = (atomicAdd(w, 1u) & 0xFFu) == VG - 1u;
                todo = false;
            }
            const u64 cb = __ballot(comp);
            if (cb) {
                if (comp) {
                    const unsigned at = (unsigned)qn + (unsigned)(NV + 1) * __builtin_amdgcn_mbcnt_hi((unsigned)(cb >> 32), __builtin_amdgcn_mbcnt_lo((unsigned)cb, 0u));
#pragma unroll
                    for (int j = 0; j < NV; j++) myq[at + j] = p | (g << 8) | ((unsigned)j << 30);
                    myq[at + NV] = p | (g << 8) | (3u << 30);
                }
                qn += (NV + 1) * __popcll(cb);
            }
            if (!__any(todo)) break;
            flush_queue();
            if (PL_LD(&L.dead) || it > PL_SPIN_LIMIT) {
                PL_ST(&L.dead, 1u);
                break;
            }
            if (it) __builtin_amdgcn_s_sleep(4);
        }
        if (qn >= PL_QFLUSH) flush_queue();
    };

    bool alive = true;
    auto step = [&](const u64 (&v)[NC][8], const unsigned m, const i64 sbase) __attribute__((always_inline)) {
        const unsigned dbase = (unsigned)(sbase - r0);
        const unsigned valid = m;
        if constexpr (NP == 0) {
            nsel += (unsigned)__popc(valid);
#pragma unroll
            for (int e = 0; e < 8; e++) {
                u64 val[NV];
#pragma unroll
                for (int j = 0; j < NV; j++) val[j] = v[1 + j][e];
                place((valid >> e) & 1u, v[0][e], val, dbase + (unsigned)((e >> 1) * 128 + (e & 1)));
            }
        } else {
            unsigned rem = m;
            nsel += (unsigned)__popc(rem);
            u64 t[1 + NV][8];
#pragma unroll
            for (int c = 0; c < 1 + NV; c++) {
#pragma unroll
                for (int q = 0; q < 8; q++) {
                    t[c][q] = v[c][q];
                    if constexpr (NV > 1) asm volatile("" : "+v"(t[c][q]));
                }
            }
            while (__any(rem != 0u)) {
                const bool on = rem != 0u;
                const unsigned e = (unsigned)__builtin_ctz(rem | 0x100u);
                rem &= rem - 1u;
                u64 key = t[0][0], val[NV];
#pragma unroll
                for (int j = 0; j < NV; j++) val[j] = t[1 + j][0];
#pragma unroll
                for (int q = 1; q < 8; q++) {
                    const bool is = e == (unsigned)q;
                    key = is ? t[0][q] : key;
#pragma unroll
                    for (int j = 0; j < NV; j++) val[j] = is ? t[1 + j][q] : val[j];
                }
                place(on, key, val, dbase + (e >> 1) * 128u + (e & 1u));
            }
        }
        flush_queue();
        if (PL_LD(&L.dead)) alive = false;
    };

    const i64 nsteps = (r1 - r0 + PL_WROWS - 1) / PL_WROWS;
    const i64 nfull = (r1 - r0) / PL_WROWS;
    {
        u64 va[NC][8];
        for (i64 s = wv; s < nfull && alive; s += PL_WAVES) {
            const i64 base = r0 + s * PL_WROWS + lane * 2;
            if constexpr (NP == 0) {
#pragma unroll
                for (int c = 0; c < NC; c++) {
#pragma unroll
                    for (int j = 0; j < 4; j++) {
                        const u64x2 t = rfx_ld2(P.cols[c] + base + j * 128);
                        va[c][2 * j] = t.x;
                        va[c][2 * j + 1] = t.y;
                    }
                }
                step(va, 0xffu, base);
            } else {
#pragma unroll
                for (int c = 0; c < NC; c++) {
                    if ((A.pmask >> c) & 1u) {
#pragma unroll
                        for (int j = 0; j < 4; j++) {
                            const u64x2 t = rfx_ld2(P.cols[c] + base + j * 128);
                            va[c][2 * j] = t.x;
                            va[c][2 * j + 1] = t.y;
                        }
                    } else {
#pragma unroll
                        for (int e = 0; e < 8; e++) va[c][e] = 0;
                    }
                }
                const unsigned m = eval_preds<NC, 8, NP>(S, va, 0xffu);
#pragma unroll
                for (int c = 0; c < NC; c++) {
                    if (!((A.pmask >> c) & 1u)) {
#pragma unroll
                        for (int j = 0; j < 4; j++) {
                            if ((m >> (2 * j)) & 3u) {
                                const u64x2 t = rfx_ld2(P.cols[c] + base + j * 128);
                                va[c][2 * j] = t.x;
                                va[c][2 * j + 1] = t.y;
                            }
                        }
                    }
                }
                step(va, m, base);
            }
        }
    }
    if (nfull < nsteps && (nfull % PL_WAVES) == wv && alive) {
        u64 va[NC][8];
        const i64 base = r0 + nfull * PL_WROWS + lane * 2;
        unsigned valid = 0;
#pragma unroll
        for (int e = 0; e < 8; e++) {
            const i64 row = base + (e >> 1) * 128 + (e & 1);
            const bool in = row < r1;
            valid |= (unsigned)in << e;
#pragma unroll
            for (int c = 0; c < NC; c++) va[c][e] = in ? P.cols[c][row] : 0ULL;
        }
        step(va, (NP == 0) ? valid : eval_preds<NC, 8, NP>(S, va, valid), base);
    }
    __syncthreads();
    if (L.dead) {
        if (tid == 0) atomicExch(&A.ctl[1], 1u);
        return;
    }
    for (int i = tid; i < PARTS * (NV + 1) * (int)LPD; i += PL_T) {
        const unsigned sub = (unsigned)i & (LPD - 1u), p = ((unsigned)i / LPD) % (unsigned)PARTS, pl = ((unsigned)i / LPD) / (unsigned)PARTS;
        const unsigned t = tail[p];
        if (!(t & (VG - 1u))) continue;
        const unsigned gi = t >> VGL;
        if (pl < (unsigned)NV) {
            const pl_v2 x = *(const pl_v2 *)(vring + ((size_t)pl * PARTS + p) * RING + (gi & 1u) * VG + sub * 2);
            if constexpr (KVI) {
                *(pl_v2 *)(A.vals[0] + 2 * (region + (u64)p * A.c0 + (u64)gi * VG) + (u64)pl * VG + sub * 2) = x;
            } else {
                u64 *dst = (NV == 1 ? A.vals[0] : (pl == 0 ? A.vals[0] : (pl == 1 ? A.vals[1] : A.vals[2])));
                *(pl_v2 *)(dst + region + (u64)p * A.c0 + (u64)gi * VG + sub * 2) = x;
            }
        } else if (sub < LPD / 2) {
            const pl_v2 x = *(const pl_v2 *)(mring + (size_t)p * RING + (gi & 1u) * VG + sub * 4);
            *(pl_v2 *)(A.meta + region + (u64)p * A.c0 + (u64)gi * VG + sub * 4) = x;
        }
    }
    for (int i = tid; i < PARTS; i += PL_T) A.cnt[(size_t)blockIdx.x * PARTS + i] = tail[i];
    i64 sel = (i64)nsel;
    for (int s2 = 32; s2 >= 1; s2 >>= 1) {
        const i64 omn = (i64)rfx_shfl_xor_u64((u64)mn, s2), omx = (i64)rfx_shfl_xor_u64((u64)mx, s2);
        mn = omn < mn ? omn : mn;
        mx = omx > mx ? omx : mx;
        sel += (i64)rfx_shfl_xor_u64((u64)sel, s2);
    }
    if (lane == 0) {
        L.red[0][wv] = mn;
        L.red[1][wv] = mx;
        L.red[2][wv] = sel;
    }
    __syncthreads();
    if (tid == 0) {
        for (int w2 = 1; w2 < PL_WAVES; w2++) {
            mn = L.red[0][w2] < mn ? L.red[0][w2] : mn;
            mx = L.red[1][w2] > mx ? L.red[1][w2] : mx;
            sel += L.red[2][w2];
        }
        unsigned long long *g = (unsigned long long *)A.ctl + 8;
        if (sel > 0) {
            atomicMax(&g[0], ~((unsigned long long)mn ^ 0x8000000000000000ULL));
            atomicMax(&g[1], (unsigned long long)mx ^ 0x8000000000000000ULL);
            atomicAdd(&g[2], (unsigned long long)sel);
        }
    }
}

struct PlaneAggArgs {
    i64 kmin, range;
    i64 local;
    int split;
    int excl;
    int first_read;
    int nblk, pbits;
    int agg_pl[RFX_MAX_AGGS];
    i64 block_rows;
    unsigned c0;
    const u64 *vals[PL_MAX_NV];
    const unsigned *meta;
    const unsigned *cnt;
    u64 *first;
    u64 *acc[RFX_MAX_AGGS];
    u64 *cntt[RFX_MAX_AGGS];
};
#define PL_FIRST_NONE 0xFFFFFFFFu

template <int THREADS, int NVL, bool FAST>
__global__ __launch_bounds__(THREADS) void k_plane_aggregate(const Plan P, const PlaneAggArgs A) {
    extern __shared__ __attribute__((aligned(16))) u64 pl_agg_smem[];
    const int tid = threadIdx.x;
    const int p = blockIdx.x / A.split, s = blockIdx.x % A.split;
    const i64 local = A.local;
    int kind[RFX_MAX_AGGS], f64[RFX_MAX_AGGS], skip[RFX_MAX_AGGS], cnt_of[RFX_MAX_AGGS], apl[RFX_MAX_AGGS];
    int ncnt = 0;
#pragma unroll
    for (int a = 0; a < RFX_MAX_AGGS; a++) {
        kind[a] = (a < P.nagg) ? P.aggs[a].kind : -1;
        f64[a] = (a < P.nagg) ? P.aggs[a].f64 : 0;
        skip[a] = (a < P.nagg) ? P.aggs[a].skipnull : 0;
        apl[a] = (a < P.nagg) ? A.agg_pl[a] : -1;
        cnt_of[a] = -1;
        if (kind[a] >= 0 && agg_has_cnt(kind[a], f64[a])) cnt_of[a] = ncnt++;
    }
    u64 *accs = pl_agg_smem;
    unsigned *first = (unsigned *)(accs + (i64)P.nagg * local);
    unsigned *cnts = first + local;
    for (i64 i = tid; i < local; i += THREADS) first[i] = PL_FIRST_NONE;
#pragma unroll
    for (int a = 0; a < RFX_MAX_AGGS; a++) {
        if (kind[a] < 0) continue;
        const u64 id = acc_identity(kind[a], f64[a]);
        for (i64 i = tid; i < local; i += THREADS) accs[(i64)a * local + i] = id;
        if (cnt_of[a] >= 0) {
            for (i64 i = tid; i < local; i += THREADS) cnts[(i64)cnt_of[a] * local + i] = 0u;
        }
    }
    __syncthreads();
    const unsigned shift = (unsigned)(((i64)p - A.kmin) >> A.pbits);
    auto apply = [&](unsigned mm, i64 rbase, const u64 (&x)[NVL]) __attribute__((always_inline)) {
        const unsigned mask = (1u << PL_SLOT_BITS) - 1u;
        const unsigned slot = ((mm & mask) + shift) & mask;
        if ((i64)slot >= local) return;
        const unsigned row = (unsigned)(rbase + (i64)(mm >> PL_SLOT_BITS));
        if (A.first_read) {
            if (row < first[slot]) atomicMin(&first[slot], row);
        } else __hip_atomic_fetch_min(&first[slot], row, __ATOMIC_RELAXED, __HIP_MEMORY_SCOPE_WORKGROUP);
        if constexpr (FAST) {
            unsafeAtomicAdd((double *)&accs[slot], rfx_as_f64(x[0]));
            return;
        }
#pragma unroll
        for (int a = 0; a < RFX_MAX_AGGS; a++) {
            if (kind[a] < 0) continue;
            u64 xv = 0;
#pragma unroll
            for (int j = 0; j < NVL; j++)
                if (apl[a] == j) xv = x[j];
            group_apply(&accs[(i64)a * local + slot], cnt_of[a] >= 0 ? &cnts[(i64)cnt_of[a] * local + slot] : (unsigned *)0, kind[a], f64[a], xv, skip[a]);
        }
    };
    const int lane = tid & 63;
    constexpr int NW = THREADS / 64;
    const int Q = A.split * NW;
    struct Batch {
        pl_v2 val[NVL][2];
        pl_m2 m[2];
        unsigned n, i0;
        int b;
    };
    auto load = [&](bool live, int b, unsigned i0, unsigned n, Batch &B) __attribute__((always_inline)) {
        B.b = live ? b : 0;
        B.i0 = live ? i0 : 0u;
        B.n = live ? n : 0u;
        const u64 base = (((u64)B.b << A.pbits) + (u64)p) * A.c0;
#pragma unroll
        for (int k = 0; k < 2; k++) {
            unsigned i = B.i0 + ((unsigned)k * 64u + (unsigned)lane) * 2u;
            i = i < A.c0 - 2u ? i : A.c0 - 2u;
#pragma unroll
            for (int j = 0; j < NVL; j++) B.val[j][k] = __builtin_nontemporal_load((const pl_v2 *)(A.vals[j] + base + i));
            B.m[k] = __builtin_nontemporal_load((const pl_m2 *)(A.meta + base + i));
        }
    };
    auto consume = [&](const Batch &B) __attribute__((always_inline)) {
        const i64 rbase = (i64)B.b * A.block_rows;
#pragma unroll
        for (int k = 0; k < 2; k++) {
            const unsigned i = B.i0 + ((unsigned)k * 64u + (unsigned)lane) * 2u;
            if (i < B.n) {
                u64 x[NVL];
#pragma unroll
                for (int j = 0; j < NVL; j++) x[j] = B.val[j][k].x;
                apply(B.m[k].x, rbase, x);
                if (i + 1 < B.n) {
#pragma unroll
                    for (int j = 0; j < NVL; j++) x[j] = B.val[j][k].y;
                    apply(B.m[k].y, rbase, x);
                }
            }
        }
    };
    const int q = __builtin_amdgcn_readfirstlane(s * NW + (tid >> 6));
    const int nreg = q < A.nblk ? (A.nblk - q + Q - 1) / Q : 0;
    unsigned *wcnt = cnts + (i64)ncnt * local + (tid >> 6) * 64;
    int r = -1;
    int b = q;
    unsigned i0 = 0, n = 0;
    auto advance = [&]() __attribute__((always_inline)) {
        for (;;) {
            if (r >= 0 && i0 < n) return true;
            r++;
            if (r >= nreg) return false;
            if ((r & 63) == 0) {
                const int r0 = r + lane;
                wcnt[lane] = (r0 < nreg) ? A.cnt[((size_t)(q + r0 * Q) << A.pbits) + p] : 0u;
            }
            n = (unsigned)__builtin_amdgcn_readfirstlane((int)wcnt[r & 63]);
            b = q + r * Q;
            i0 = 0;
        }
    };
    Batch B0, B1;
    bool h0 = advance();
    load(h0, b, i0, n, B0);
    i0 += 256u;
    while (h0) {
        const bool h1 = advance();
        load(h1, b, i0, n, B1);
        i0 += 256u;
        consume(B0);
        if (!h1) break;
        h0 = advance();
        load(h0, b, i0, n, B0);
        i0 += 256u;
        consume(B1);
    }
    __syncthreads();
    for (i64 i = tid; i < local; i += THREADS) {
        const unsigned f = first[i];
        if (f == PL_FIRST_NONE) continue;
        const i64 g = (i << A.pbits) | (i64)(((u64)p - (u64)A.kmin) & (u64)((1 << A.pbits) - 1));
        if (g >= A.range) continue;
        const u64 fr = (u64)P.row0 + (u64)f;
        if (A.excl) {
            if (fr < A.first[g]) A.first[g] = fr;
#pragma unroll
            for (int a = 0; a < RFX_MAX_AGGS; a++) {
                if (kind[a] < 0) continue;
                const bool hc = cnt_of[a] >= 0;
                group_merge_cell_plain(&A.acc[a][g], hc ? &A.cntt[a][g] : (u64 *)0, kind[a], f64[a], accs[(i64)a * local + i], hc ? (u64)cnts[(i64)cnt_of[a] * local + i] : 0ULL);
            }
            continue;
        }
        if (fr < A.first[g]) atomicMin((unsigned long long *)&A.first[g], (unsigned long long)fr);
#pragma unroll
        for (int a = 0; a < RFX_MAX_AGGS; a++) {
            if (kind[a] < 0) continue;
            const bool hc = cnt_of[a] >= 0;
            group_merge_cell(&A.acc[a][g], hc ? &A.cntt[a][g] : (u64 *)0, kind[a], f64[a], accs[(i64)a * local + i], hc ? (u64)cnts[(i64)cnt_of[a] * local + i] : 0ULL);
        }
    }
}

int rfx_chunk_reserve(rfx_ctx *c, size_t bytes);
static size_t pl_al256(size_t x) { return (x + 255) & ~(size_t)255; }

static void plane_layout(rfx_ctx *c, int nblk, int pbits, unsigned c0, int nv, PlaneArgs *A, size_t *total, int parts = 0) {
    const size_t regions = parts ? (size_t)nblk * (size_t)parts : (size_t)nblk << pbits;
    const size_t o_cnt = 256;
    const size_t o_meta = o_cnt + pl_al256(regions * 4), o_val = o_meta + pl_al256(regions * c0 * 4);
    const size_t plane = pl_al256(regions * c0 * 8);
    if (total) *total = o_val + plane * nv;
    char *w = (char *)c->d_chunk;
    A->nblk = nblk;
    A->nv = nv;
    A->c0 = c0;
    A->ctl = (unsigned *)w;
    A->cnt = (unsigned *)(w + o_cnt);
    A->meta = (unsigned *)(w + o_meta);
    for (int j = 0; j < nv; j++) A->vals[j] = (u64 *)(w + o_val + plane * j);
}

template <int NC, int NP, int NV, int PBITS, int VGL, bool HK = false>
static int launch_plane_scatter_inst(rfx_ctx *c, const Plan &P, const PlaneArgs &A) {
    constexpr size_t lds = pl_lds_bytes<NV, PBITS, VGL, HK>();
    static_assert(lds <= 160 * 1024, "rings beyond a CU's LDS");
    static unsigned long long attr_set = 0;
    if (!((attr_set >> (c->device & 63)) & 1ull)) {
        RFX_HIP_CHECK(hipFuncSetAttribute((const void *)k_plane_scatter<NC, NP, NV, PBITS, VGL, HK>, hipFuncAttributeMaxDynamicSharedMemorySize, (int)lds));
        __atomic_fetch_or(&attr_set, 1ull << (c->device & 63), __ATOMIC_RELAXED);
    }
    hipLaunchKernelGGL((k_plane_scatter<NC, NP, NV, PBITS, VGL, HK>), dim3(A.nblk), dim3(PL_T), lds, c->stream, P, A);
    return RFX_OK;
}
template <int NC, int NV, int PBITS, int VGL, bool HK = false>
static int launch_plane_scatter_np(rfx_ctx *c, const Plan &P, const PlaneArgs &A) {
    if (P.npred == 0) return launch_plane_scatter_inst<NC, 0, NV, PBITS, VGL, HK>(c, P, A);
    if (P.npred == 1) return launch_plane_scatter_inst<NC, 1, NV, PBITS, VGL, HK>(c, P, A);
    if (P.npred <= 3) return launch_plane_scatter_inst<NC, 3, NV, PBITS, VGL, HK>(c, P, A);
    return launch_plane_scatter_inst<NC, RFX_MAX_PREDS, NV, PBITS, VGL, HK>(c, P, A);
}
static int launch_plane_scatter(rfx_ctx *c, const Plan &P, const PlaneArgs &A, int pbits) {
    const int extra = P.ncols - 1 - A.nv;
    if (extra < 0 || extra > 2) return RFX_ESTATE;
    if (A.nv == 1) {
        if (pbits == 7) return extra == 0 ? launch_plane_scatter_np<2, 1, 7, 5>(c, P, A) : (extra == 1 ? launch_plane_scatter_np<3, 1, 7, 5>(c, P, A) : launch_plane_scatter_np<4, 1, 7, 5>(c, P, A));
        return extra == 0 ? launch_plane_scatter_np<2, 1, 8, 4>(c, P, A) : (extra == 1 ? launch_plane_scatter_np<3, 1, 8, 4>(c, P, A) : launch_plane_scatter_np<4, 1, 8, 4>(c, P, A));
    }
    if (pbits != 7 || extra > 1) return RFX_ESTATE;
    if (A.nv == 2) return extra == 0 ? launch_plane_scatter_np<3, 2, 7, 4>(c, P, A) : launch_plane_scatter_np<4, 2, 7, 4>(c, P, A);
    return extra == 0 ? launch_plane_scatter_np<4, 3, 7, 4>(c, P, A) : launch_plane_scatter_np<5, 3, 7, 4>(c, P, A);
}

static int plane_value_cols(const Plan &P, int *vcol, int *agg_plane) {
    int nv = 0;
    for (int a = 0; a < P.nagg; a++) {
        const PlanAgg &ag = P.aggs[a];
        agg_plane[a] = -1;
        if (ag.kind == RFX_AGG_COUNT || ag.kind == RFX_AGG_FIRST || ag.col < 0) continue;
        if (ag.col >= RFX_XCOL) return -1;
        int j = 0;
        for (; j < nv; j++)
            if (vcol[j] == ag.col) break;
        if (j == nv) {
            if (nv >= PL_MAX_NV) return -1;
            vcol[nv++] = ag.col;
        }
        agg_plane[a] = j;
    }
    return nv;
}
static size_t plane_agg_lds(const Plan &P, int a0, int a1, i64 local) {
    size_t cells8 = 0, cells4 = 1;
    for (int a = a0; a < a1; a++) {
        cells8++;
        if (agg_has_cnt(P.aggs[a].kind, P.aggs[a].f64)) cells4++;
    }
    return (size_t)local * (cells8 * 8 + cells4 * 4) + 16 * 64 * 4 + 64;
}
#define PL_AGG_LDS_MAX (150 * 1024)
static bool plane_agg_fits(const Plan &P, i64 local) {
    for (int a = 0; a < P.nagg; a++)
        if (plane_agg_lds(P, a, a + 1, local) > PL_AGG_LDS_MAX) return false;
    return P.nagg >= 1;
}

struct PlaneState {
    int valid, npred, logic, nblk, pbits, nv;
    unsigned c0;
    const void *key;
    const void *val[PL_MAX_NV];
    i64 nrows;
    i64 seen;
    u64 sig[RFX_MAX_PREDS][6];
};
static PlaneState *plane_state(rfx_ctx *c) {
    if (!c->ext_p[2]) c->ext_p[2] = calloc(1, sizeof(PlaneState));
    return (PlaneState *)c->ext_p[2];
}
void rfx_plane_invalidate(rfx_ctx *c) {
    if (c->ext_p[2]) ((PlaneState *)c->ext_p[2])->valid = 0;
}
void rfx_plane_release(rfx_ctx *c) {
    free(c->ext_p[2]);
    c->ext_p[2] = NULL;
}
static void plane_pred_sig(const Plan &P, u64 (*sig)[6]) {
    for (int i = 0; i < P.npred; i++) {
        const PlanPred &q = P.preds[i];
        sig[i][0] = (u64)(uintptr_t)P.cols[q.col];
        sig[i][1] = q.rhs_col >= 0 ? (u64)(uintptr_t)P.cols[q.rhs_col] : 0;
        sig[i][2] = (u64)q.op;
        sig[i][3] = (u64)(q.dom_f64 | (q.lhs_cvt << 1) | (q.rhs_cvt << 2) | (q.more << 3) | ((u64)q.tree << 4));
        sig[i][4] = q.rhs_bits;
        sig[i][5] = 0;
    }
}

int rfx_plane_scope(rfx_ctx *c, const Plan &P, int key_idx, const void *d_key, int npred, int logic, unsigned long long est_range, double frac,
                    i64 *kmin, i64 *kmax, i64 *seen) {
    PlaneState *st = plane_state(c);
    if (!st) return RFX_ESTATE;
    st->valid = 0;
    if (c->flags & RFX_TUNE_NO_PLANE) return RFX_ESTATE;
    int vcol[PL_MAX_NV], agg_plane[RFX_MAX_AGGS];
    const int nv = plane_value_cols(P, vcol, agg_plane);
    if (nv < 1 || P.nx > 0) return RFX_ESTATE;
    int pbits = 7;
    {
        static const char *force = getenv("RFX_PLANE_PBITS");
        const i64 l7 = (i64)((est_range + 127) >> 7);
        if (l7 + l7 / 16 > (1 << PL_SLOT_BITS) || !plane_agg_fits(P, l7 + l7 / 16)) pbits = 8;
        if (force && nv == 1) pbits = atoi(force) == 7 ? 7 : 8;
    }
    if (pbits == 8 && nv > 1) return RFX_ESTATE;
    const i64 est_local = (i64)((est_range + (1ULL << pbits) - 1) >> pbits);
    if (est_local > (1 << PL_SLOT_BITS) || !plane_agg_fits(P, est_local)) return RFX_ESTATE;
    const i64 nrows = P.nrows;
    const i64 nblk64 = (nrows + PL_BLOCK_ROWS - 1) / PL_BLOCK_ROWS;
    if (nblk64 > (1 << 20) || nrows >= 0xFFFFFFF0LL) return RFX_ESTATE;
    double share = (double)PL_BLOCK_ROWS / (double)(1 << pbits);
    if (npred > 0) share *= (frac * 1.3 + 0.01 < 1.0 ? frac * 1.3 + 0.01 : 1.0);
    unsigned c0 = (unsigned)(share * 1.25 + 160.0);
    c0 = (c0 + 127u) & ~127u;
    PlaneArgs A;
    memset(&A, 0, sizeof(A));
    size_t need = 0;
    plane_layout(c, (int)nblk64, pbits, c0, nv, &A, &need);
    if (rfx_chunk_reserve(c, need) != RFX_OK) return RFX_ESTATE;
    plane_layout(c, (int)nblk64, pbits, c0, nv, &A, NULL);
    A.block_rows = PL_BLOCK_ROWS;
    Plan Pc = P;
    {
        int perm[RFX_MAX_COLS + PL_MAX_NV], inv[RFX_MAX_COLS], n2 = 0;
        for (int i = 0; i < P.ncols; i++) inv[i] = -1;
        perm[n2++] = key_idx;
        inv[key_idx] = 0;
        for (int j = 0; j < nv; j++) {
            if (inv[vcol[j]] < 0) inv[vcol[j]] = n2;
            perm[n2++] = vcol[j];
        }
        for (int i = 0; i < P.ncols; i++)
            if (inv[i] < 0) {
                inv[i] = n2;
                perm[n2++] = i;
            }
        if (n2 > 1 + nv + 2 || n2 > RFX_MAX_COLS) return RFX_ESTATE;
        Pc.ncols = n2;
        for (int i = 0; i < n2; i++) Pc.cols[i] = P.cols[perm[i]];
        for (int i = 0; i < P.npred; i++) {
            Pc.preds[i].col = inv[P.preds[i].col];
            if (P.preds[i].rhs_col >= 0) Pc.preds[i].rhs_col = inv[P.preds[i].rhs_col];
        }
    }
    for (int i = 0; i < Pc.npred; i++) {
        A.pmask |= 1u << Pc.preds[i].col;
        if (Pc.preds[i].rhs_col >= 0) A.pmask |= 1u << Pc.preds[i].rhs_col;
    }
    if (getenv("RFX_PLANE_LOAD_ALL")) A.pmask = 0xFFu;
    RFX_HIP_CHECK(hipMemsetAsync(A.ctl, 0, 256, c->stream));
    c->ext_i[3 + RFX_STAT_PLANE_SCATTER]++;
    RFX_KERNEL_BEGIN(c);
    int rc = launch_plane_scatter(c, Pc, A, pbits);
    RFX_KERNEL_END(c);
    if (rc != RFX_OK) return rc;
    RFX_HIP_CHECK(hipGetLastError());
    unsigned *hctl = (unsigned *)c->h_pin;
    RFX_HIP_CHECK(hipMemcpyAsync(hctl, A.ctl, 256, hipMemcpyDeviceToHost, c->stream));
    RFX_HIP_CHECK(hipStreamSynchronize(c->stream));
    if (hctl[1]) {
        c->ext_i[3 + RFX_STAT_PLANE_FALLBACK]++;
        return RFX_ESTATE;
    }
    const u64 *hs = (const u64 *)hctl + 8;
    *seen = (i64)hs[2];
    plane_state(c)->seen = *seen;
    *kmin = (i64)(~hs[0] ^ 0x8000000000000000ULL);
    *kmax = (i64)(hs[1] ^ 0x8000000000000000ULL);
    if (*seen > 0 && *kmin == RFX_NULL_I64_D) return RFX_ESTATE;
    if (*seen == 0) return RFX_OK;
    st->valid = 1;
    st->key = d_key;
    for (int j = 0; j < nv; j++) st->val[j] = (const void *)P.cols[vcol[j]];
    st->nrows = nrows;
    st->npred = npred;
    st->logic = logic;
    st->nblk = (int)nblk64;
    st->pbits = pbits;
    st->nv = nv;
    st->c0 = c0;
    plane_pred_sig(P, st->sig);
    return RFX_OK;
}

template <int THREADS, int NVL, bool FAST>
static int launch_plane_aggregate_inst(rfx_ctx *c, const Plan &P, const PlaneAggArgs &G, int grid, size_t lds, int lds_max) {
    static unsigned long long attr_set = 0;
    if (!((attr_set >> (c->device & 63)) & 1ull)) {
        RFX_HIP_CHECK(hipFuncSetAttribute((const void *)k_plane_aggregate<THREADS, NVL, FAST>, hipFuncAttributeMaxDynamicSharedMemorySize, lds_max));
        __atomic_fetch_or(&attr_set, 1ull << (c->device & 63), __ATOMIC_RELAXED);
    }
    hipLaunchKernelGGL((k_plane_aggregate<THREADS, NVL, FAST>), dim3(grid), dim3(THREADS), lds, c->stream, P, G);
    return RFX_OK;
}
template <int THREADS>
static int launch_plane_aggregate(rfx_ctx *c, const Plan &P, const PlaneAggArgs &G, int nvl, bool fast, int grid, size_t lds, int lds_max) {
    if (nvl <= 1) return fast ? launch_plane_aggregate_inst<THREADS, 1, true>(c, P, G, grid, lds, lds_max) : launch_plane_aggregate_inst<THREADS, 1, false>(c, P, G, grid, lds, lds_max);
    if (nvl == 2) return launch_plane_aggregate_inst<THREADS, 2, false>(c, P, G, grid, lds, lds_max);
    return launch_plane_aggregate_inst<THREADS, 3, false>(c, P, G, grid, lds, lds_max);
}

int rfx_plane_accumulate(rfx_ctx *c, const Plan &P, int key_idx, const rfx_group_tables_t *t) {
    PlaneState *st = (PlaneState *)c->ext_p[2];
    if (!st || !st->valid) return RFX_ESTATE;
    int vcol[PL_MAX_NV], agg_plane[RFX_MAX_AGGS];
    bool ok = st->key == (const void *)P.cols[key_idx] && st->nrows == P.nrows && st->npred == P.npred && st->logic == P.logic && P.nx == 0;
    const int nv = ok ? plane_value_cols(P, vcol, agg_plane) : -1;
    ok = ok && nv == st->nv;
    for (int j = 0; ok && j < nv; j++) ok = st->val[j] == (const void *)P.cols[vcol[j]];
    if (ok && P.npred > 0) {
        u64 sig[RFX_MAX_PREDS][6];
        plane_pred_sig(P, sig);
        ok = memcmp(sig, st->sig, sizeof(u64) * 6 * (size_t)P.npred) == 0;
    }
    st->valid = 0;
    if (!ok || t->range <= (1 << st->pbits)) return RFX_ESTATE;
    const i64 local = (t->range + (1 << st->pbits) - 1) >> st->pbits;
    if (local > (1 << PL_SLOT_BITS) || !plane_agg_fits(P, local)) return RFX_ESTATE;
    PlaneArgs A;
    memset(&A, 0, sizeof(A));
    plane_layout(c, st->nblk, st->pbits, st->c0, st->nv, &A, NULL);
    const int nparts = 1 << st->pbits;
    RFX_KERNEL_BEGIN(c);
    int rc = RFX_OK;
    for (int a0 = 0; a0 < P.nagg && rc == RFX_OK;) {
        int a1 = a0 + 1;
        while (a1 < P.nagg && plane_agg_lds(P, a0, a1 + 1, local) <= PL_AGG_LDS_MAX) a1++;
        Plan Ps = P;
        Ps.nagg = a1 - a0;
        PlaneAggArgs G;
        memset(&G, 0, sizeof(G));
        G.kmin = t->kmin;
        G.range = t->range;
        G.local = local;
        {
            static const char *fr = getenv("RFX_PL_FIRST_READ");
            G.first_read = fr ? atoi(fr) : 1;
        }
        G.nblk = st->nblk;
        G.pbits = st->pbits;
        G.block_rows = PL_BLOCK_ROWS;
        G.c0 = st->c0;
        G.meta = A.meta;
        G.cnt = A.cnt;
        G.first = (u64 *)t->d_first;
        int used[PL_MAX_NV] = {-1, -1, -1}, nvl = 0;
        for (int a = a0; a < a1; a++) {
            Ps.aggs[a - a0] = P.aggs[a];
            G.acc[a - a0] = (u64 *)t->d_acc[a];
            G.cntt[a - a0] = (u64 *)t->d_cnt[a];
            G.agg_pl[a - a0] = -1;
            if (agg_plane[a] < 0) continue;
            int j = 0;
            for (; j < nvl; j++)
                if (used[j] == agg_plane[a]) break;
            if (j == nvl) {
                used[nvl] = agg_plane[a];
                G.vals[nvl] = A.vals[agg_plane[a]];
                nvl++;
            }
            G.agg_pl[a - a0] = j;
        }
        for (int a = a1 - a0; a < RFX_MAX_AGGS; a++) {
            Ps.aggs[a].kind = -1;
            G.agg_pl[a] = -1;
        }
        if (nvl == 0) {
            G.vals[0] = A.vals[0];
            nvl = 1;
        }
        const size_t lds = plane_agg_lds(P, a0, a1, local);
        const bool fast = Ps.nagg == 1 && Ps.aggs[0].kind == RFX_AGG_SUM && Ps.aggs[0].f64 && !Ps.aggs[0].skipnull && G.agg_pl[0] == 0;
        c->ext_i[3 + RFX_STAT_PLANE_AGGREGATE]++;
        if (lds > 52 * 1024) {
            G.split = (c->num_cus + nparts - 1) / nparts;
            if (G.split < 1) G.split = 1;
            {
                static const char *fs = getenv("RFX_PLANE_AGG_SPLIT");
                if (fs && atoi(fs) >= 1) G.split = atoi(fs);
                else if (st->seen > 0 && st->seen <= 40000000) G.split = 1;
            }
            G.excl = G.split == 1;
            rc = launch_plane_aggregate<1024>(c, Ps, G, nvl, fast, nparts * G.split, lds, 160 * 1024);
        } else {
            const int per_cu = (int)((156 * 1024) / lds) < 4 ? (int)((156 * 1024) / lds) : 4;
            G.split = (per_cu * c->num_cus + nparts - 1) / nparts;
            if (G.split < 1) G.split = 1;
            rc = launch_plane_aggregate<512>(c, Ps, G, nvl, fast, nparts * G.split, lds, 64 * 1024);
        }
        a0 = a1;
    }
    RFX_KERNEL_END(c);
    if (rc != RFX_OK) return rc;
    RFX_HIP_CHECK(hipGetLastError());
    return RFX_OK;
}

struct PlaneHashArgs {
    HashArgs H;
    int nblk, pbits, hbits;
    int parts;
// ... 226 lines not shown
                const u64 old = atomicCAS((unsigned long long *)&lkey[(size_t)b * 4 + e], (unsigned long long)RFX_NULL_I64_D, (unsigned long long)key);
                if ((i64)old == RFX_NULL_I64_D || old == key) return (int)(b * 4u) + e;
                continue;
            }
            if (++steps >= nb) break;
            b = (b + 1 == nb) ? 0 : b + 1;
        }
        return -1;
    };
    auto consume2 = [&](const Batch &B) __attribute__((always_inline)) {
        const i64 rbase = (i64)B.b * X.block_rows;
        unsigned mm[4], sb[4], lrow[4];
        u64 key[4], val[4];
        pl_v2 q0[4], q1[4];
        bool on[4], cold[4];
        int idx[4];
#pragma unroll
        for (int k = 0; k < 2; k++) {
            const unsigned i = B.i0 + ((unsigned)k * 64u + (unsigned)lane) * 2u;
            mm[2 * k] = B.m[k].x, mm[2 * k + 1] = B.m[k].y;
            key[2 * k] = B.key[k].x, key[2 * k + 1] = B.key[k].y;
            val[2 * k] = B.val[k].x, val[2 * k + 1] = B.val[k].y;
            on[2 * k] = i < B.n && mine_of(mm[2 * k]);
            on[2 * k + 1] = i + 1 < B.n && mine_of(mm[2 * k + 1]);
        }
#pragma unroll
        for (int j = 0; j < 4; j++) {
            sb[j] = start_of(mm[j]) >> 2;
            q0[j] = *(const pl_v2 *)&lkey[(size_t)sb[j] * 4];
            q1[j] = *(const pl_v2 *)&lkey[(size_t)sb[j] * 4 + 2];
        }
#pragma unroll
        for (int j = 0; j < 4; j++) idx[j] = on[j] ? bucket_find(key[j], sb[j], q0[j], q1[j]) : -1;
#pragma unroll
        for (int j = 0; j < 4; j++) {
            lrow[j] = (unsigned)(rbase + (i64)(mm[j] >> PL_SLOT_BITS));
            cold[j] = on[j] && idx[j] < 0;
            if (!on[j] || idx[j] < 0) continue;
            __hip_atomic_fetch_min(&lfirst[idx[j]], lrow[j], __ATOMIC_RELAXED, __HIP_MEMORY_SCOPE_WORKGROUP);
            if constexpr (FAST) unsafeAtomicAdd((double *)&larr[idx[j]], rfx_as_f64(val[j]));
            else {
#pragma unroll
                for (int a = 0; a < RFX_MAX_AGGS; a++) {
                    if (kind[a] < 0) continue;
                    group_apply(&larr[(size_t)arr_of[a] * C + idx[j]], &larr[(size_t)(arr_of[a] + 1) * C + idx[j]], kind[a], f64[a], apl[a] == 1 ? val[j] : 0ULL, skip[a]);
                }
            }
        }
        while (__builtin_expect(__builtin_amdgcn_ballot_w64(cold[0] | cold[1] | cold[2] | cold[3]) != 0, 0)) {
            const bool any = cold[0] | cold[1] | cold[2] | cold[3];
            const int pick = cold[0] ? 0 : cold[1] ? 1 : cold[2] ? 2 : 3;
            const u64 ck = pick == 0 ? key[0] : pick == 1 ? key[1] : pick == 2 ? key[2] : key[3];
            const u64 cv = pick == 0 ? val[0] : pick == 1 ? val[1] : pick == 2 ? val[2] : val[3];
            const unsigned cr = pick == 0 ? lrow[0] : pick == 1 ? lrow[1] : pick == 2 ? lrow[2] : lrow[3];
            cold[0] = cold[0] && pick != 0;
            cold[1] = cold[1] && pick != 1;
            cold[2] = cold[2] && pick != 2;
            cold[3] = cold[3] && pick != 3;
            if (any) fold(-1, cr, 0u, ck, cv);
        }
    };
    auto consume_v = [&](const Batch &B) __attribute__((always_inline)) {
        if constexpr (VAR == 1) consume1(B);
        else if constexpr (VAR == 2) consume2(B);
        else consume(B);
    };
    const int q = __builtin_amdgcn_readfirstlane(tid >> 6);
    const int nreg = q < X.nblk ? (X.nblk - q + NW - 1) / NW : 0;
    unsigned *mywcnt = wcnt + (tid >> 6) * 64;
    int r = -1;
    int b = q;
    unsigned i0 = 0, n = 0;
    auto advance = [&]() __attribute__((always_inline)) {
        for (;;) {
            if (r >= 0 && i0 < n) return true;
            r++;
            if (r >= nreg) return false;
            if ((r & 63) == 0) {
                const int r0 = r + lane;
                mywcnt[lane] = (r0 < nreg) ? X.cnt[(size_t)(q + r0 * NW) * (size_t)X.parts + p] : 0u;
            }
            n = (unsigned)__builtin_amdgcn_readfirstlane((int)mywcnt[r & 63]);
            b = q + r * NW;
            i0 = 0;
        }
    };
    Batch B0, B1;
    bool h0 = advance();
    load(h0, b, i0, n, B0);
    i0 += 256u;
    while (h0) {
        const bool h1 = advance();
        load(h1, b, i0, n, B1);
        i0 += 256u;
        consume_v(B0);
        if (!h1) break;
        h0 = advance();
        load(h0, b, i0, n, B0);
        i0 += 256u;
        consume_v(B1);
    }
    __syncthreads();
    for (unsigned i = tid; i < C; i += PLH_T) {
        const u64 key = lkey[i];
        if ((i64)key == RFX_NULL_I64_D) continue;
        const i64 g = hash_slot(X.H.keys, X.H.capacity, key);
        if (g < 0) {
            atomicExch(X.overflow, 1);
            continue;
        }
        const u64 row = (u64)P.row0 + lfirst[i];
        if (row < X.H.first[g]) atomicMin((unsigned long long *)&X.H.first[g], (unsigned long long)row);
#pragma unroll
        for (int a = 0; a < RFX_MAX_AGGS; a++) {
            if (kind[a] < 0) continue;
            const bool hc = agg_has_cnt(kind[a], f64[a]);
            group_merge_cell(&X.H.acc[a][g], hc ? &X.H.cnt[a][g] : (u64 *)0, kind[a], f64[a], larr[(size_t)arr_of[a] * C + i],
                             hc ? larr[(size_t)(arr_of[a] + 1) * C + i] : 0ULL);
        }
    }
}

static int plh_var() {
    static const char *var_env = getenv("RFX_PLH_VAR");
    return var_env ? atoi(var_env) : 2;
}
int rfx_plane_hash_accumulate(rfx_ctx *c, const Plan &P, int key_idx, const HashArgs &H, double est, int *d_overflow) {
    if (c->flags & (RFX_TUNE_NO_PLANE | RFX_TUNE_NO_PARTITION)) return RFX_ESTATE;
    const i64 nrows = P.nrows;
    if (nrows < ((c->flags & RFX_TUNE_CHUNK_SMALL) ? (1LL << 16) : (1LL << 22)) || nrows >= 0xFFFFFFF0LL || P.nx > 0 || P.nagg < 1) return RFX_ESTATE;
    int vcol[PL_MAX_NV], agg_plane[RFX_MAX_AGGS];
    const int nv = plane_value_cols(P, vcol, agg_plane);
    if (nv < 0 || nv > 1) return RFX_ESTATE;
    int narr = 0;
    for (int a = 0; a < P.nagg; a++) narr += agg_has_cnt(P.aggs[a].kind, P.aggs[a].f64) ? 2 : 1;
    const size_t entry = 8 + (size_t)narr * 8 + 4;
    const unsigned lcap = (unsigned)((((size_t)150 * 1024) - 16 * 64 * 4) / entry) & ~63u;
    if (est < 4096.0) return RFX_ESTATE;
    const double HEAD = plh_var() == 2 ? 1.3 : 1.6;
    int pbits = 7, hbits = 0, parts = 128;
    static const char *force = getenv("RFX_PLANE_HASH_PARTS");
    if (force && atoi(force) == 192 && est * HEAD / 128.0 > (double)lcap && est * 1.2 / 192.0 <= (double)lcap) {
        pbits = 8;
        parts = 192;
    } else {
        if (est * HEAD / (128.0 * 4.0) > (double)lcap) pbits = 8;
        if (est * HEAD / 128.0 > (double)lcap && est * HEAD / 256.0 <= (double)lcap && !(force && atoi(force) == 128)) pbits = 8;
        while (hbits < 2 && est * HEAD / (double)((1 << pbits) << hbits) > (double)lcap) hbits++;
        if (est * HEAD / (double)((1 << pbits) << hbits) > (double)lcap) return RFX_ESTATE;
        parts = 1 << pbits;
    }
    const i64 nblk64 = (nrows + PL_BLOCK_ROWS - 1) / PL_BLOCK_ROWS;
    if (nblk64 > (1 << 20)) return RFX_ESTATE;
    Plan Pc = P;
    {
        int perm[RFX_MAX_COLS + 2], inv[RFX_MAX_COLS], n2 = 0;
        for (int i = 0; i < P.ncols; i++) inv[i] = -1;
        perm[n2++] = key_idx;
        inv[key_idx] = 0;
        perm[n2++] = key_idx;
        perm[n2++] = nv == 1 ? vcol[0] : key_idx;
        if (nv == 1 && inv[vcol[0]] < 0) inv[vcol[0]] = 2;
        for (int i = 0; i < P.ncols; i++)
            if (inv[i] < 0) {
                inv[i] = n2;
                perm[n2++] = i;
            }
        if (n2 > 4 || n2 > RFX_MAX_COLS) return RFX_ESTATE;
        Pc.ncols = n2;
        for (int i = 0; i < n2; i++) Pc.cols[i] = P.cols[perm[i]];
        for (int i = 0; i < P.npred; i++) {
            Pc.preds[i].col = inv[P.preds[i].col];
            if (P.preds[i].rhs_col >= 0) Pc.preds[i].rhs_col = inv[P.preds[i].rhs_col];
        }
    }
    double share = (double)PL_BLOCK_ROWS / (double)parts;
    unsigned c0 = (unsigned)(share * 1.25 + 160.0);
    c0 = (c0 + 127u) & ~127u;
    PlaneArgs A;
    memset(&A, 0, sizeof(A));
    size_t need = 0;
    plane_layout(c, (int)nblk64, pbits, c0, 2, &A, &need, parts);
    if (rfx_chunk_reserve(c, need) != RFX_OK) return RFX_ESTATE;
    plane_layout(c, (int)nblk64, pbits, c0, 2, &A, NULL, parts);
    A.block_rows = PL_BLOCK_ROWS;
    for (int i = 0; i < Pc.npred; i++) {
        A.pmask |= 1u << Pc.preds[i].col;
        if (Pc.preds[i].rhs_col >= 0) A.pmask |= 1u << Pc.preds[i].rhs_col;
    }
    c->ck_valid = 0;
    rfx_plane_invalidate(c);
    RFX_HIP_CHECK(hipMemsetAsync(A.ctl, 0, 256, c->stream));
    c->ext_i[3 + RFX_STAT_PLANE_SCATTER]++;
    RFX_KERNEL_BEGIN(c);
    int rc;
    if (parts == 192) rc = Pc.ncols == 3 ? launch_plane_scatter_np<3, 2, 8, 4, true>(c, Pc, A) : launch_plane_scatter_np<4, 2, 8, 4, true>(c, Pc, A);
    else if (pbits == 7) rc = Pc.ncols == 3 ? launch_plane_scatter_np<3, 2, 7, 4, true>(c, Pc, A) : launch_plane_scatter_np<4, 2, 7, 4, true>(c, Pc, A);
    else rc = Pc.ncols == 3 ? launch_plane_scatter_np<3, 2, 8, 3, true>(c, Pc, A) : launch_plane_scatter_np<4, 2, 8, 3, true>(c, Pc, A);
    if (rc != RFX_OK) return rc;
    RFX_HIP_CHECK(hipGetLastError());
    unsigned *hctl = (unsigned *)c->h_pin;
    RFX_HIP_CHECK(hipMemcpyAsync(hctl, A.ctl, 256, hipMemcpyDeviceToHost, c->stream));
    RFX_HIP_CHECK(hipStreamSynchronize(c->stream));
    if (hctl[1]) {
        c->ext_i[3 + RFX_STAT_PLANE_FALLBACK]++;
        return RFX_ESTATE;
    }
    PlaneHashArgs X;
    memset(&X, 0, sizeof(X));
    X.H = H;
    X.nblk = (int)nblk64;
    X.pbits = pbits;
    X.hbits = hbits;
    X.parts = parts;
    X.block_rows = PL_BLOCK_ROWS;
    X.c0 = c0;
    X.lcap = lcap;
    X.narr = narr;
    for (int a = 0; a < RFX_MAX_AGGS; a++) X.agg_pl[a] = (a < P.nagg && agg_plane[a] == 0) ? 1 : -1;
    X.keys = A.vals[0];
    X.vals = A.vals[1];
    X.kvi = (parts == 256);
    {
        static const char *dbg = getenv("RFX_PLH_DBG");
        X.dbg = dbg ? atoi(dbg) : 0;
    }
    X.meta = A.meta;
    X.cnt = A.cnt;
    X.overflow = d_overflow;
    const size_t lds = (size_t)lcap * entry + 16 * 64 * 4 + 64;
    static unsigned long long attr_set = 0;
    if (!((attr_set >> (c->device & 63)) & 1ull)) {
        RFX_HIP_CHECK(hipFuncSetAttribute((const void *)k_plane_hash_aggregate<false, 0>, hipFuncAttributeMaxDynamicSharedMemorySize, 160 * 1024));
        RFX_HIP_CHECK(hipFuncSetAttribute((const void *)k_plane_hash_aggregate<true, 0>, hipFuncAttributeMaxDynamicSharedMemorySize, 160 * 1024));
        RFX_HIP_CHECK(hipFuncSetAttribute((const void *)k_plane_hash_aggregate<false, 1>, hipFuncAttributeMaxDynamicSharedMemorySize, 160 * 1024));
        RFX_HIP_CHECK(hipFuncSetAttribute((const void *)k_plane_hash_aggregate<true, 1>, hipFuncAttributeMaxDynamicSharedMemorySize, 160 * 1024));
        RFX_HIP_CHECK(hipFuncSetAttribute((const void *)k_plane_hash_aggregate<false, 2>, hipFuncAttributeMaxDynamicSharedMemorySize, 160 * 1024));
        RFX_HIP_CHECK(hipFuncSetAttribute((const void *)k_plane_hash_aggregate<true, 2>, hipFuncAttributeMaxDynamicSharedMemorySize, 160 * 1024));
        __atomic_fetch_or(&attr_set, 1ull << (c->device & 63), __ATOMIC_RELAXED);
    }
    c->ext_i[3 + RFX_STAT_PLANE_AGGREGATE]++;
    const bool fast = P.nagg == 1 && P.aggs[0].kind == RFX_AGG_SUM && P.aggs[0].f64 && !P.aggs[0].skipnull && X.agg_pl[0] == 1;
    const int var = plh_var();
    if (var == 0) {
        if (fast) hipLaunchKernelGGL((k_plane_hash_aggregate<true, 0>), dim3(parts << hbits), dim3(PLH_T), lds, c->stream, Pc, X);
        else hipLaunchKernelGGL((k_plane_hash_aggregate<false, 0>), dim3(parts << hbits), dim3(PLH_T), lds, c->stream, Pc, X);
    } else if (var == 2) {
        if (fast) hipLaunchKernelGGL((k_plane_hash_aggregate<true, 2>), dim3(parts << hbits), dim3(PLH_T), lds, c->stream, Pc, X);
        else hipLaunchKernelGGL((k_plane_hash_aggregate<false, 2>), dim3(parts << hbits), dim3(PLH_T), lds, c->stream, Pc, X);
    } else {
        if (fast) hipLaunchKernelGGL((k_plane_hash_aggregate<true, 1>), dim3(parts << hbits), dim3(PLH_T), lds, c->stream, Pc, X);
        else hipLaunchKernelGGL((k_plane_hash_aggregate<false, 1>), dim3(parts << hbits), dim3(PLH_T), lds, c->stream, Pc, X);
    }
    RFX_KERNEL_END(c);
    RFX_HIP_CHECK(hipGetLastError());
    return RFX_OK;
}
```

### rayforce_amd/csrc/rfx_rtc.hip

```cpp
#include <dlfcn.h>
#include <stdlib.h>
#include <dirent.h>
#include <sys/stat.h>
#include <unistd.h>
#include <functional>
#include <map>
#include <mutex>
#include <string>
#include "rfx_group_common.hpp"
#include "rfx_where_once_kernel.hpp"
#include "build/rfx_rtc_headers.inc"

typedef struct _hiprtcProgram *rtcProgram;
static struct {
    int state;
    int (*create)(rtcProgram *, const char *, const char *, int, const char **, const char **);
    int (*compile)(rtcProgram, int, const char **);
    int (*log_size)(rtcProgram, size_t *);
    int (*log)(rtcProgram, char *);
    int (*code_size)(rtcProgram, size_t *);
    int (*code)(rtcProgram, char *);
    int (*destroy)(rtcProgram *);
    int (*version)(int *, int *);
    std::string cache_dir;
    u64 env_hash[2];
    int cache_files;
} R;
static std::map<std::string, hipFunction_t> *g_cache;
static long long g_launches, g_compiles, g_disk_loads, g_disk_writes;
extern "C" void rfx_hip_rtc_stats(int64_t *launches, int64_t *compiles) {
    if (launches) *launches = g_launches;
    if (compiles) *compiles = g_compiles;
}
extern "C" void rfx_hip_rtc_cache_stats(int64_t *loaded_from_disk, int64_t *written_to_disk) {
    if (loaded_from_disk) *loaded_from_disk = g_disk_loads;
    if (written_to_disk) *written_to_disk = g_disk_writes;
}
static const char *const RTC_OPTS[] = {"--offload-arch=gfx950", "-O3", "-std=c++17", "-fno-fast-math", "-ffp-contract=off"};
static void fnv2(u64 h[2], const void *p, size_t n) {
    const unsigned char *b = (const unsigned char *)p;
    for (size_t i = 0; i < n; i++) {
        h[0] = (h[0] ^ b[i]) * 0x100000001B3ULL;
        h[1] = (h[1] ^ (b[i] + 0x9Eu)) * 0x00000100000001B3ULL + 0x9E3779B97F4A7C15ULL;
    }
}

static bool trace() { return getenv("RFX_TRACE") != NULL; }
static bool rtc_ready_once();
static bool rtc_ready() {
    static std::mutex once;
    std::lock_guard<std::mutex> hold(once);
    return rtc_ready_once();
}
static bool rtc_ready_once() {
    if (R.state) return R.state > 0;
    R.state = -1;
    if (getenv("RFX_NO_RTC")) return false;
    void *h = dlopen("libhiprtc.so", RTLD_NOW | RTLD_LOCAL);
    if (!h) h = dlopen("/opt/rocm/lib/libhiprtc.so", RTLD_NOW | RTLD_LOCAL);
    if (!h) {
        if (trace()) fprintf(stderr, "[rfx] rtc: libhiprtc.so not loadable (%s)\n", dlerror());
        return false;
    }
    *(void **)&R.create = dlsym(h, "hiprtcCreateProgram");
    *(void **)&R.compile = dlsym(h, "hiprtcCompileProgram");
    *(void **)&R.log_size = dlsym(h, "hiprtcGetProgramLogSize");
    *(void **)&R.log = dlsym(h, "hiprtcGetProgramLog");
    *(void **)&R.code_size = dlsym(h, "hiprtcGetCodeSize");
    *(void **)&R.code = dlsym(h, "hiprtcGetCode");
    *(void **)&R.destroy = dlsym(h, "hiprtcDestroyProgram");
    *(void **)&R.version = dlsym(h, "hiprtcVersion");
    if (!R.create || !R.compile || !R.log_size || !R.log || !R.code_size || !R.code || !R.destroy) return false;
    R.env_hash[0] = 0xCBF29CE484222325ULL;
    R.env_hash[1] = 0x84222325CBF29CE4ULL;
    int vmaj = 0, vmin = 0;
    if (R.version) R.version(&vmaj, &vmin);
    fnv2(R.env_hash, &vmaj, sizeof(vmaj));
    fnv2(R.env_hash, &vmin, sizeof(vmin));
    for (size_t i = 0; i < sizeof(RTC_OPTS) / sizeof(RTC_OPTS[0]); i++) fnv2(R.env_hash, RTC_OPTS[i], strlen(RTC_OPTS[i]) + 1);
    for (int i = 0; i < RTC_NHDR; i++) fnv2(R.env_hash, RTC_HDR_TEXTS[i], strlen(RTC_HDR_TEXTS[i]) + 1);
    const char *env = getenv("RFX_RTC_CACHE");
    R.cache_dir.clear();
    if (!env || (strcmp(env, "0") != 0 && env[0])) {
        std::string cand[3];
        int nc = 0;
        if (env) cand[nc++] = env;
        else {
            Dl_info di;
            if (dladdr((const void *)&rtc_ready, &di) && di.dli_fname) {
                std::string so(di.dli_fname);
                const size_t cut = so.find_last_of('/');
                cand[nc++] = (cut == std::string::npos ? std::string(".") : so.substr(0, cut)) + "/rtc_cache";
            }
            const char *xdg = getenv("XDG_CACHE_HOME"), *home = getenv("HOME");
            if (xdg && xdg[0] == '/') cand[nc++] = std::string(xdg) + "/rfx_rtc";
            else if (home && home[0] == '/') cand[nc++] = std::string(home) + "/.cache/rfx_rtc";
            char tmp[64];
            snprintf(tmp, sizeof(tmp), "/tmp/rfx_rtc_cache_%u", (unsigned)getuid());
            cand[nc++] = tmp;
        }
        for (int i = 0; i < nc && R.cache_dir.empty(); i++) {
            (void)mkdir(cand[i].c_str(), 0700);
            struct stat st;
            if (lstat(cand[i].c_str(), &st) != 0 || !S_ISDIR(st.st_mode) || st.st_uid != geteuid() || (st.st_mode & (S_IWGRP | S_IWOTH))) continue;
            if (access(cand[i].c_str(), W_OK | X_OK) == 0) R.cache_dir = cand[i];
        }
        if (!R.cache_dir.empty()) {
            R.cache_files = 0;
            if (DIR *d = opendir(R.cache_dir.c_str())) {
                while (readdir(d)) R.cache_files++;
                closedir(d);
            }
        }
    }
    if (trace()) fprintf(stderr, "[rfx] rtc: ready, code objects cached in %s\n", R.cache_dir.empty() ? "(memory only)" : R.cache_dir.c_str());
    R.state = 1;
    return true;
}

static std::string cache_path(const std::string &src) {
    if (R.cache_dir.empty()) return std::string();
    u64 h[2] = {R.env_hash[0], R.env_hash[1]};
    fnv2(h, src.data(), src.size());
    char name[48];
    snprintf(name, sizeof(name), "/%016llx%016llx.co", h[0], h[1]);
    return R.cache_dir + name;
}
static bool read_code(const std::string &path, std::string &code) {
    FILE *f = path.empty() ? NULL : fopen(path.c_str(), "rb");
    if (!f) return false;
    char buf[1 << 16];
    size_t got;
    code.clear();
    while ((got = fread(buf, 1, sizeof(buf), f)) > 0) code.append(buf, got);
    fclose(f);
    return code.size() > 64 && memcmp(code.data(), "\177ELF", 4) == 0;
}
static void write_code(const std::string &path, const std::string &code) {
    if (path.empty() || R.cache_files > 4096) return;
    char tmp[32];
    snprintf(tmp, sizeof(tmp), ".%d.tmp", (int)getpid());
    const std::string t = path + tmp;
    FILE *f = fopen(t.c_str(), "wb");
    if (!f) return;
    const bool ok = fwrite(code.data(), 1, code.size(), f) == code.size();
    if (fclose(f) != 0 || !ok || rename(t.c_str(), path.c_str()) != 0) {
        (void)unlink(t.c_str());
        return;
    }
    R.cache_files++;
    g_disk_writes++;
}

static void plan_text(const Plan &P, const GroupArgs *G, std::string &o) {
    char b[512];
#define ADD(...) do { snprintf(b, sizeof(b), __VA_ARGS__); o += b; } while (0)
    ADD("#define RTC_PLAN { %d, %d, %d, %d, {}, { ", P.ncols, P.npred, P.nagg, P.logic);
    for (int i = 0; i < P.npred; i++) {
        const bool cnan = P.preds[i].rhs_col < 0 && P.preds[i].dom_f64 && (P.preds[i].rhs_bits & 0x7FF0000000000000ULL) == 0x7FF0000000000000ULL && (P.preds[i].rhs_bits & 0x000FFFFFFFFFFFFFULL) != 0;
        ADD("{ %d, %d, %d, %d, %d, %d, %s, %d, %d }, ", P.preds[i].col, P.preds[i].rhs_col, P.preds[i].op, P.preds[i].dom_f64, P.preds[i].lhs_cvt, P.preds[i].rhs_cvt,
            cnan ? "0x7FF8000000000000ULL" : "0ULL", P.preds[i].more, P.preds[i].tree);
    }
    o += "}, { ";
// ... 32 lines not shown
        return false;
    }
    size_t cs = 0;
    R.code_size(prog, &cs);
    code.assign(cs, 0);
    R.code(prog, &code[0]);
    R.destroy(&prog);
    return cs > 0;
}
static hipFunction_t load(const std::string &code, const char *name) {
    hipModule_t mod;
    hipFunction_t fn = NULL;
    if (hipModuleLoadData(&mod, code.data()) != hipSuccess || hipModuleGetFunction(&fn, mod, name) != hipSuccess) {
        if (trace()) fprintf(stderr, "[rfx] rtc: module load failed\n");
        return NULL;
    }
    return fn;
}

static std::mutex g_rtc_lock;
static hipFunction_t plan_kernel_locked(const std::string &sig, const std::string &src, const char *name, i64 nrows, const char *what);
static hipFunction_t plan_kernel(int device, const std::string &sig0, const std::string &src, const char *name, i64 nrows, const char *what) {
    std::lock_guard<std::mutex> hold(g_rtc_lock);
    char dv[24];
    snprintf(dv, sizeof(dv), "//dev%d\n", device);
    return plan_kernel_locked(std::string(dv) + sig0, src, name, nrows, what);
}
static hipFunction_t plan_kernel_locked(const std::string &sig, const std::string &src, const char *name, i64 nrows, const char *what) {
    if (!g_cache) g_cache = new std::map<std::string, hipFunction_t>();
    auto it = g_cache->find(sig);
    if (it != g_cache->end()) return it->second;
    static std::map<std::string, int> *seen;
    if (!seen) seen = new std::map<std::string, int>();
    const int times = ++(*seen)[sig];
    const std::string path = cache_path(src);
    if (times == 1) {
        if (const char *dump = getenv("RFX_RTC_DUMP")) {
            char fn[512];
            snprintf(fn, sizeof(fn), "%s/%s_%zx.hip", dump, name, std::hash<std::string>()(src));
            if (FILE *f = fopen(fn, "w")) {
                fwrite(src.data(), 1, src.size(), f);
                fclose(f);
            }
        }
    }
    std::string code;
    if (times == 1 && read_code(path, code)) {
        hipFunction_t fn = load(code, name);
        if (fn) {
            g_disk_loads++;
            (*g_cache)[sig] = fn;
            if (trace()) fprintf(stderr, "[rfx] rtc: %s loaded from %s\n", what, path.c_str());
            return fn;
        }
    }
    if (!getenv("RFX_RTC_EAGER") && (times < 2 || nrows < (1LL << 24))) return NULL;
    if (trace()) fprintf(stderr, "[rfx] rtc: compiling %s ...\n", what);
    hipFunction_t fn = NULL;
    if (compile(src, code)) {
        fn = load(code, name);
        if (fn) write_code(path, code);
    }
    (*g_cache)[sig] = fn;
    if (trace()) fprintf(stderr, "[rfx] rtc: %s\n", fn ? "ready" : "not available for this plan: the prebuilt kernel runs");
    return fn;
}

static void filter_aggr_text(const Plan &P, std::string &sig, std::string &src) {
    bool deep = false;
    for (int i = 0; i < P.nx; i++) deep |= P.xs[i].nops > 1;
    const int nc = P.ncols < 1 ? 1 : P.ncols;
    int u = nc <= 4 ? 4 : (nc <= 6 ? 2 : 1);
    if (getenv("RFX_FA_U")) u = atoi(getenv("RFX_FA_U")) >= 4 ? 4 : (atoi(getenv("RFX_FA_U")) >= 2 ? 2 : 1);
    char head[256];
    snprintf(head, sizeof(head), "#define FA_NC %d\n#define FA_NA %d\n#define FA_U %d\n#define FA_NP %d\n#define FA_NX %d\n#define FA_DEEP %s\n", nc, P.nagg, u, P.npred, P.nx,
             deep ? "true" : "false");
    std::string cond;
    plan_text(P, NULL, cond);
    sig = std::string(head) + cond;
    src = sig +
                            "#include \"rfx_scalar_kernel.hpp\"\n"
                            "extern \"C\" __global__ __launch_bounds__(RFX_BLOCK) void k_filter_aggr_plan(const Plan P0, Acc *__restrict__ ws) {\n"
                            "    constexpr Plan D = RTC_PLAN;\n"
                            "    filter_aggr_body<FA_NC, FA_NA, FA_U, FA_NP, FA_NX, FA_DEEP>(D, P0, ws);\n"
                            "}\n";
}

int rfx_rtc_filter_aggr(rfx_ctx *c, const Plan &P, int grid, void *ws, int *na_stride) {
    if (P.nagg < 1 || (c->flags & RFX_TUNE_NO_RTC) || !rtc_ready()) return RFX_ESTATE;
    std::string sig, src;
    filter_aggr_text(P, sig, src);
    hipFunction_t fn = plan_kernel(c->device, sig, src, "k_filter_aggr_plan", P.nrows, "a fused filter + aggregate kernel for this plan");
    if (!fn) return RFX_ESTATE;
    Plan Pv = P;
    void *wsv = ws;
    void *args[] = {&Pv, &wsv};
    RFX_HIP_CHECK(hipModuleLaunchKernel(fn, (unsigned)grid, 1, 1, RFX_BLOCK, 1, 1, 0, c->stream, args, NULL));
    __atomic_fetch_add(&g_launches, 1, __ATOMIC_RELAXED);
    *na_stride = P.nagg + 1;
    return RFX_OK;
}

int rfx_rtc_group_few(rfx_ctx *c, const Plan &P, const GroupArgs &G, int grid) {
    if (G.range < 1 || G.range > RFX_FEW_MAX_GROUPS || P.nagg < 1 || P.nrows >= (1LL << 32)) return RFX_ESTATE;
    if (!rtc_ready()) return RFX_ESTATE;
    const int npt = P.npred == 0 ? 0 : (P.npred <= 2 ? 2 : RFX_MAX_PREDS);
    int u = P.ncols <= 4 ? 2 : 1;
    if (getenv("RFX_FEW_U")) u = atoi(getenv("RFX_FEW_U")) >= 2 ? 2 : 1;
    char head[256];
    snprintf(head, sizeof(head), "#define FEW_NC %d\n#define FEW_NA %d\n#define FEW_NG %d\n#define FEW_NPT %d\n#define FEW_U %d\n#define FEW_FMA %d\n#define FEW_PREFETCH %d\n", P.ncols, P.nagg, (int)G.range, npt, u,
             getenv("RFX_FEW_NO_FMA") ? atoi(getenv("RFX_FEW_NO_FMA")) : 1,
             getenv("RFX_FEW_PREFETCH") ? atoi(getenv("RFX_FEW_PREFETCH")) : 1);
    std::string cond;
    plan_text(P, &G, cond);
    const std::string sig = std::string(head) + cond;
    const std::string src = std::string(head) + cond + "#include \"rfx_group_few_rtc.hpp\"\n";
    hipFunction_t fn = plan_kernel(c->device, sig, src, "k_group_few", P.nrows, "a register-accumulator group-by kernel for this plan");
    if (!fn) return RFX_ESTATE;
    Plan Pv = P;
    GroupArgs Gv = G;
    void *args[] = {&Pv, &Gv};
    RFX_HIP_CHECK(hipModuleLaunchKernel(fn, (unsigned)grid, 1, 1, RFX_BLOCK, 1, 1, 0, c->stream, args, NULL));
    __atomic_fetch_add(&g_launches, 1, __ATOMIC_RELAXED);
    return RFX_OK;
}

static void where_once_text(const Plan &P, std::string &sig, std::string &src) {
    const int nc = P.ncols < 1 ? 1 : P.ncols;
    char head[128];
    snprintf(head, sizeof(head), "#define WOP_NC %d\n#define WOP_NP %d\n", nc, P.npred < 1 ? 1 : P.npred);
    std::string cond;
    plan_text(P, NULL, cond);
    sig = std::string("//where_once\n") + head + cond;
    src = sig +
          "#include \"rfx_where_once_kernel.hpp\"\n"
          "extern \"C\" __global__ __launch_bounds__(WO_T) __attribute__((amdgpu_waves_per_eu(WOP_NC <= 2 ? 5 : 3))) void k_where_once_plan(const Plan P0, const WoArgs A) {\n"
          "    constexpr Plan D = RTC_PLAN;\n"
          "    where_once_body<WOP_NC, WOP_NP>(D, P0, A);\n"
          "}\n";
}
int rfx_rtc_where_once(rfx_ctx *c, const Plan &P, const WoArgs &A, int grid) {
    if (P.npred < 1 || P.npred > 4 || P.ncols > 4 || (c->flags & RFX_TUNE_NO_RTC) || !rtc_ready()) return RFX_ESTATE;
    std::string sig, src;
    where_once_text(P, sig, src);
    hipFunction_t fn = plan_kernel(c->device, sig, src, "k_where_once_plan", P.nrows, "a one-pass where kernel for this plan");
    if (!fn) return RFX_ESTATE;
    Plan Pv = P;
    WoArgs Av = A;
    void *args[] = {&Pv, &Av};
    RFX_HIP_CHECK(hipModuleLaunchKernel(fn, (unsigned)grid, 1, 1, WO_T, 1, 1, 0, c->stream, args, NULL));
    __atomic_fetch_add(&g_launches, 1, __ATOMIC_RELAXED);
    return RFX_OK;
}
extern "C" int rfx_hip_rtc_prewarm_where(const rfx_pred_t *preds, int npred, int logic) {
    Plan P;
    int rc = rfx_plan_build(&P, preds, npred, logic, NULL, 0, NULL, NULL, 1, 0);
    if (rc != RFX_OK) return rc;
    if (P.npred < 1 || P.npred > 4 || P.ncols > 4 || !rtc_ready() || R.cache_dir.empty()) return RFX_ESTATE;
    std::string sig, src, code;
    where_once_text(P, sig, src);
    const std::string path = cache_path(src);
    if (read_code(path, code)) return RFX_OK;
    if (!compile(src, code)) return RFX_ESTATE;
    write_code(path, code);
    return read_code(path, code) ? RFX_OK : RFX_ESTATE;
}

extern "C" int rfx_hip_rtc_prewarm_filter_aggr(const rfx_pred_t *preds, int npred, int logic, const rfx_agg_t *aggs, int nagg) {
    Plan P;
    int rc = rfx_plan_build(&P, preds, npred, logic, aggs, nagg, NULL, NULL, 1, 0);
    if (rc != RFX_OK) return rc;
    if (P.nagg < 1 || !rtc_ready() || R.cache_dir.empty()) return RFX_ESTATE;
    std::string sig, src, code;
    filter_aggr_text(P, sig, src);
    const std::string path = cache_path(src);
    if (read_code(path, code)) return RFX_OK;
    if (!compile(src, code)) return RFX_ESTATE;
    write_code(path, code);
    return read_code(path, code) ? RFX_OK : RFX_ESTATE;
}
```

### rayforce_amd/prewarm.py

```python
from __future__ import annotations

import ctypes as C
from typing import Dict, Optional, Sequence, Tuple

from . import _lib as L

_TYPES = {"i64": L.RFX_I64, "f64": L.RFX_F64}


def _flat(where):
    if where is None:
        return L.RFX_AND, []
    if where[0] in L.OPS:
        return L.RFX_AND, [(where, 0)]
    top = where[0]
    out = []
    for arm in where[1:]:
        if arm[0] in L.OPS:
            out.append((arm, 0))
        else:
            out.extend((s, 1) for s in arm[1:-1])
            out.append((arm[-1], 0))
    return (L.RFX_AND if top == "and" else L.RFX_OR), out


def _preds(where, types, ident):
    logic, preds = _flat(where)
    parr = (L.Pred * max(1, len(preds)))()
    for p, ((op, lhs, rhs), more) in zip(parr, preds):
        p.d_col, p.col_type, p.op, p.more = ident[lhs], _TYPES[types[lhs]], L.OPS[op], more
        if isinstance(rhs, str):
            p.d_rhs_col, p.rhs_type = ident[rhs], _TYPES[types[rhs]]
        elif isinstance(rhs, float):
            p.rhs_type, p.rhs_f = L.RFX_F64, rhs
        else:
            p.rhs_type, p.rhs_i = L.RFX_I64, int(rhs)
    return parr, len(preds), logic


def where(where, types: Dict[str, str]) -> bool:
    lib = L.load_library()
    ident = {name: 4096 * (i + 1) for i, name in enumerate(types)}
    parr, n, logic = _preds(where, types, ident)
    return lib.rfx_hip_rtc_prewarm_where(parr, n, logic) == L.RFX_OK


def filter_aggr(where, aggs: Sequence[Tuple[str, Optional[str]]], types: Dict[str, str]) -> bool:
    lib = L.load_library()
    ident = {name: 4096 * (i + 1) for i, name in enumerate(types)}
    parr, npred, logic = _preds(where, types, ident)
    aarr = (L.Agg * max(1, len(aggs)))()
    for a, (fn, col) in zip(aarr, aggs):
        a.kind = L.AGGS[fn]
        a.d_col, a.col_type = (ident[col], _TYPES[types[col]]) if col is not None else (None, L.RFX_I64)
    return lib.rfx_hip_rtc_prewarm_filter_aggr(parr, npred, logic, aarr, len(aggs)) == L.RFX_OK


BASELINE_PLANS = {
    "c1": (None, [("sum", "v")], {"v": "f64"}),
    "c2": (("<", "a", 100_000), [("sum", "a")], {"a": "i64"}),
    "c2b": (("<", "a", 100_000), [("sum", "b")], {"a": "i64", "b": "f64"}),
    "c5": (("and", ("<", "a", 0.316228), (">", "b", 0.683772), ("!=", "c", 0.25)), [("avg", "d"), ("min", "d"), ("max", "d")],
           {"a": "f64", "b": "f64", "c": "f64", "d": "f64"}),
}


WHERE_PLANS = {
    "w2": (("<", "a", 100_000), {"a": "i64"}),
}


def baseline() -> Dict[str, bool]:
    done = {name: filter_aggr(*plan) for name, plan in BASELINE_PLANS.items()}
    done.update({name: where(*plan) for name, plan in WHERE_PLANS.items()})
    return done


def cache_stats() -> Tuple[int, int]:
    a, b = C.c_int64(), C.c_int64()
    L.load_library().rfx_hip_rtc_cache_stats(C.byref(a), C.byref(b))
    return int(a.value), int(b.value)
```

Baseline: 214.9 billion.

## JIT-compile plane scatter kernel specialized to the query plan via RTC

Moves the plane scatter kernel body into a shared header and adds a runtime-compiled variant that bakes the plan (predicate constants, column mask, shape) in as compile-time constants. The launcher tries the RTC kernel first and falls back to the templated kernel. The aim is to cut per-row predicate evaluation overhead and register pressure in the scatter phase of group-by. In exchange it adds compile latency on first use, plus prewarm and stats plumbing and an ablation env hook.

Result: no change. 215.0 billion (median of 4 runs) (+0.0%).

```diff
diff --git a/include/rfx_hip.h b/include/rfx_hip.h
--- a/include/rfx_hip.h
+++ b/include/rfx_hip.h
@@ -158,7 +158,9 @@
     RFX_STAT_CHUNK_SCATTER = 3,
     RFX_STAT_CHUNK_AGGREGATE = 4,
     RFX_STAT_MASK_PASSES = 5,
-    RFX_STAT_WHERE_ONCE = 6
+    RFX_STAT_WHERE_ONCE = 6,
+    RFX_STAT_PLANE_SCATTER_PLAN = 7,
+    RFX_STAT_PLANE_SCATTER_COMPILES = 8
 };
 int64_t rfx_hip_ctx_stat(rfx_ctx_t *ctx, int which);
 
@@ -174,6 +176,8 @@
 void rfx_hip_rtc_cache_stats(int64_t *loaded_from_disk, int64_t *written_to_disk);
 int rfx_hip_rtc_prewarm_filter_aggr(const rfx_pred_t *preds, int npred, int logic, const rfx_agg_t *aggs, int nagg);
 int rfx_hip_rtc_prewarm_where(const rfx_pred_t *preds, int npred, int logic);
+int rfx_hip_rtc_prewarm_plane_scatter(const rfx_pred_t *preds, int npred, int logic, const rfx_agg_t *aggs, int nagg, const void *d_key,
+                                      int64_t key_range, int sparse_parts);
 
 int rfx_hip_h2d_pipelined(rfx_ctx_t *ctx, void *d_dst, const void *src, size_t bytes);
 int rfx_hip_d2h_pipelined(rfx_ctx_t *ctx, void *dst, const void *d_src, size_t bytes);
diff --git a/rayforce_amd/_lib.py b/rayforce_amd/_lib.py
--- a/rayforce_amd/_lib.py
+++ b/rayforce_amd/_lib.py
@@ -183,6 +183,7 @@
     "rfx_hip_rtc_cache_stats": (None, [_P(C.c_int64), _P(C.c_int64)]),
     "rfx_hip_rtc_prewarm_filter_aggr": (C.c_int, [_P(Pred), C.c_int, C.c_int, _P(Agg), C.c_int]),
     "rfx_hip_rtc_prewarm_where": (C.c_int, [_P(Pred), C.c_int, C.c_int]),
+    "rfx_hip_rtc_prewarm_plane_scatter": (C.c_int, [_P(Pred), C.c_int, C.c_int, _P(Agg), C.c_int, C.c_void_p, C.c_int64, C.c_int]),
     "rfx_hip_timer_start": (C.c_int, [_ctx]),
     "rfx_hip_timer_stop": (C.c_int, [_ctx, _P(C.c_float)]),
     "rfx_hip_ctx_profile": (C.c_int, [_ctx, C.c_int]),
diff --git a/rayforce_amd/csrc/rfx_common.hpp b/rayforce_amd/csrc/rfx_common.hpp
--- a/rayforce_amd/csrc/rfx_common.hpp
+++ b/rayforce_amd/csrc/rfx_common.hpp
@@ -98,7 +98,8 @@
 
 struct CtxExt {
     i64 emit_g0, emit_gn;
-    i64 spare[30];
+    i64 plane_plan_launches, plane_plan_compiles;
+    i64 spare[28];
 };
 static inline CtxExt *rfx_ext(rfx_ctx *c) { return (CtxExt *)c->ext_p[7]; }
 
diff --git a/rayforce_amd/csrc/rfx_ctx.hip b/rayforce_amd/csrc/rfx_ctx.hip
--- a/rayforce_amd/csrc/rfx_ctx.hip
+++ b/rayforce_amd/csrc/rfx_ctx.hip
@@ -99,7 +99,9 @@
 }
 
 extern "C" int64_t rfx_hip_ctx_stat(rfx_ctx_t *c, int which) {
-    if (!c || which < 0 || which > 6) return -1;
+    if (!c || which < 0 || which > 8) return -1;
+    if (which == RFX_STAT_PLANE_SCATTER_PLAN) return rfx_ext(c)->plane_plan_launches;
+    if (which == RFX_STAT_PLANE_SCATTER_COMPILES) return rfx_ext(c)->plane_plan_compiles;
     if (which == 6) return (int64_t)(uintptr_t)c->ext_p[4];
     return which == RFX_STAT_MASK_PASSES ? c->ext_i[0] : c->ext_i[3 + which];
 }
diff --git a/rayforce_amd/csrc/rfx_group_plane.hip b/rayforce_amd/csrc/rfx_group_plane.hip
--- a/rayforce_amd/csrc/rfx_group_plane.hip
+++ b/rayforce_amd/csrc/rfx_group_plane.hip
@@ -1,316 +1,10 @@
 #include "rfx_part_common.hpp"
+#include "rfx_group_plane_kernel.hpp"
 #include <stdlib.h>
-
-#define PL_T 1024
-#define PL_WAVES (PL_T / RFX_WAVE)
-#define PL_WROWS 512
-#define PL_BLOCK_ROWS (1 << 18)
-#define PL_DELTA_BITS 18
-#define PL_SLOT_BITS 14
-#define PL_QCAP 320
-#define PL_QFLUSH 24
-#define PL_SPIN_LIMIT (1u << 14)
-#define PL_MAX_NV 3
-#ifndef PL_META64_PLAIN
-#define PL_META64_PLAIN 1
-#endif
-
-struct PlaneArgs {
-    int nblk;
-    int nv;
-    unsigned pmask;
-    i64 block_rows;
-    unsigned c0;
-    u64 *vals[PL_MAX_NV];
-    unsigned *meta;
-    unsigned *cnt;
-    unsigned *ctl;
-};
-struct PlSh {
-    unsigned dead, _pad[3];
-    i64 red[3][PL_WAVES];
-};
-template <int PBITS, int VGL, bool HK>
-__host__ __device__ constexpr int pl_parts() { return (HK && PBITS == 8 && VGL == 4) ? 192 : (1 << PBITS); }
-template <int NV, int PBITS, int VGL, bool HK = false>
-__host__ __device__ constexpr size_t pl_lds_bytes() {
-    return (size_t)pl_parts<PBITS, VGL, HK>() * ((size_t)(2 << VGL) * (NV * 8 + 4) + 8 + 4) + (size_t)PL_WAVES * PL_QCAP * 4 + sizeof(PlSh) + 64;
-}
-typedef u64 pl_v2 __attribute__((ext_vector_type(2)));
-typedef unsigned pl_m2 __attribute__((ext_vector_type(2)));
-#define PL_LD(ptr) __hip_atomic_load((ptr), __ATOMIC_RELAXED, __HIP_MEMORY_SCOPE_WORKGROUP)
-#define PL_ST(ptr, v) __hip_atomic_store((ptr), (v), __ATOMIC_RELAXED, __HIP_MEMORY_SCOPE_WORKGROUP)
 
 template <int NC, int NP, int NV, int PBITS, int VGL, bool HK = false>
 __global__ __launch_bounds__(PL_T) void k_plane_scatter(const Plan P, const PlaneArgs A) {
-    constexpr int PARTS = pl_parts<PBITS, VGL, HK>();
-    constexpr bool P192 = PARTS != (1 << PBITS);
-    constexpr unsigned VG = 1u << VGL, RING = 2u << VGL;
-    constexpr bool KVI = HK && NV == 2 && PBITS == 8 && VGL == 3;
-    constexpr unsigned LPD = VG / 2;
-    extern __shared__ __attribute__((aligned(16))) unsigned char pl_smem[];
-    u64 *vring = (u64 *)pl_smem;
-    unsigned *mring = (unsigned *)(vring + (size_t)NV * PARTS * RING);
-    unsigned *words = mring + (size_t)PARTS * RING;
-    unsigned *tail = words + PARTS * 2;
-    unsigned *fq = tail + PARTS;
-    PlSh &L = *(PlSh *)(fq + PL_WAVES * PL_QCAP);
-    PredSet<NP> S;
-    predset_load<NP>(P, S);
-    const int tid = threadIdx.x, lane = tid & 63, wv = tid >> 6;
-    unsigned *myq = fq + wv * PL_QCAP;
-    const i64 r0 = (i64)blockIdx.x * A.block_rows;
-    const i64 r1 = (r0 + A.block_rows < P.nrows) ? r0 + A.block_rows : P.nrows;
-    const u64 region = ((u64)blockIdx.x * (u64)PARTS) * A.c0;
-    for (int i = tid; i < PARTS; i += PL_T) {
-        tail[i] = 0;
-        words[2 * i] = 0;
-        words[2 * i + 1] = 0;
-    }
-    if (tid == 0) L.dead = 0;
-    __syncthreads();
-    i64 mn = RFX_INF_I64_D, mx = RFX_NULL_I64_D;
-    unsigned nsel = 0;
-    int qn = 0;
-
-    auto flush_queue = [&]() __attribute__((always_inline)) {
-        asm volatile("" ::: "memory");
-        for (int i0 = 0; i0 < qn; i0 += 64 / (int)LPD) {
-            const int idx = i0 + (lane / (int)LPD);
-            if (idx < qn) {
-                const unsigned d = myq[idx];
-                const unsigned p = d & 0xFFu, gi = (d >> 8) & 0x3FFFFFu, pl = d >> 30, sub = lane & (LPD - 1u);
-                if (pl < 3) {
-                    const pl_v2 x = *(const pl_v2 *)(vring + ((size_t)pl * PARTS + p) * RING + (gi & 1u) * VG + sub * 2);
-                    if constexpr (KVI) {
-                        __builtin_nontemporal_store(x, (pl_v2 *)(A.vals[0] + 2 * (region + (u64)p * A.c0 + (u64)gi * VG) + (u64)pl * VG + sub * 2));
-                    } else {
-                        u64 *dst = (NV == 1 ? A.vals[0] : (pl == 0 ? A.vals[0] : (pl == 1 ? A.vals[1] : A.vals[2])));
-                        __builtin_nontemporal_store(x, (pl_v2 *)(dst + region + (u64)p * A.c0 + (u64)gi * VG + sub * 2));
-                    }
-                } else if (sub < LPD / 2) {
-                    const pl_v2 x = *(const pl_v2 *)(mring + (size_t)p * RING + (gi & 1u) * VG + sub * 4);
-                    if constexpr (KVI || (VGL == 4 && PL_META64_PLAIN)) *(pl_v2 *)(A.meta + region + (u64)p * A.c0 + (u64)gi * VG + sub * 4) = x;
-                    else __builtin_nontemporal_store(x, (pl_v2 *)(A.meta + region + (u64)p * A.c0 + (u64)gi * VG + sub * 4));
-                }
-            }
-        }
-        asm volatile("" ::: "memory");
-        for (int i = lane; i < qn; i += 64) {
-            const unsigned d = myq[i];
-            if ((d >> 30) == 3u) atomicAdd(&words[2 * (d & 0xFFu) + ((d >> 8) & 1u)], 256u - VG);
-        }
-        qn = 0;
-    };
-
-    auto place = [&](const bool on, const u64 key, const u64 (&val)[NV], const unsigned delta) __attribute__((always_inline)) {
-        const u64 kh = HK ? rfx_hash_index_u64(RFX_U64_HASH_SEED, key) : key;
-        const unsigned p = P192 ? (unsigned)(((kh >> 32) * (u64)PARTS) >> 32) : (HK ? (unsigned)(kh >> (64 - PBITS)) : ((unsigned)key & (unsigned)(PARTS - 1)));
-        unsigned seq = 0;
-        if (on) {
-            const i64 k = (i64)key;
-            mn = k < mn ? k : mn;
-            mx = k > mx ? k : mx;
-            seq = atomicAdd(&tail[p], 1u);
-            if (seq >= A.c0) PL_ST(&L.dead, 1u);
-        }
-        const unsigned g = seq >> VGL;
-        unsigned *w = &words[2 * p + (g & 1u)];
-        bool todo = on && seq < A.c0;
-        for (unsigned it = 0;; it++) {
-            bool ready = false;
-            if (todo) ready = (PL_LD(w) >> 8) == (g >> 1);
-            bool comp = false;
-            if (ready) {
-                const unsigned at = p * RING + (seq & (RING - 1u));
-#pragma unroll
-                for (int j = 0; j < NV; j++) vring[(size_t)j * PARTS * RING + at] = val[j];
-                mring[at] = ((unsigned)(P192 ? (kh >> 18) : (HK ? (kh >> (64 - PBITS - PL_SLOT_BITS)) : (key >> PBITS))) & ((1u << PL_SLOT_BITS) - 1u)) | (delta << PL_SLOT_BITS);
-                asm volatile("" ::: "memory");
-                comp = (atomicAdd(w, 1u) & 0xFFu) == VG - 1u;
-                todo = false;
-            }
-            const u64 cb = __ballot(comp);
-            if (cb) {
-                if (comp) {
-                    const unsigned at = (unsigned)qn + (unsigned)(NV + 1) * __builtin_amdgcn_mbcnt_hi((unsigned)(cb >> 32), __builtin_amdgcn_mbcnt_lo((unsigned)cb, 0u));
-#pragma unroll
-                    for (int j = 0; j < NV; j++) myq[at + j] = p | (g << 8) | ((unsigned)j << 30);
-                    myq[at + NV] = p | (g << 8) | (3u << 30);
-                }
-                qn += (NV + 1) * __popcll(cb);
-            }
-            if (!__any(todo)) break;
-            flush_queue();
-            if (PL_LD(&L.dead) || it > PL_SPIN_LIMIT) {
-                PL_ST(&L.dead, 1u);
-                break;
-            }
-            if (it) __builtin_amdgcn_s_sleep(4);
-        }
-        if (qn >= PL_QFLUSH) flush_queue();
-    };
-
-    bool alive = true;
-    auto step = [&](const u64 (&v)[NC][8], const unsigned m, const i64 sbase) __attribute__((always_inline)) {
-        const unsigned dbase = (unsigned)(sbase - r0);
-        const unsigned valid = m;
-        if constexpr (NP == 0) {
-            nsel += (unsigned)__popc(valid);
-#pragma unroll
-            for (int e = 0; e < 8; e++) {
-                u64 val[NV];
-#pragma unroll
-                for (int j = 0; j < NV; j++) val[j] = v[1 + j][e];
-                place((valid >> e) & 1u, v[0][e], val, dbase + (unsigned)((e >> 1) * 128 + (e & 1)));
-            }
-        } else {
-            unsigned rem = m;
-            nsel += (unsigned)__popc(rem);
-            u64 t[1 + NV][8];
-#pragma unroll
-            for (int c = 0; c < 1 + NV; c++) {
-#pragma unroll
-                for (int q = 0; q < 8; q++) {
-                    t[c][q] = v[c][q];
-                    if constexpr (NV > 1) asm volatile("" : "+v"(t[c][q]));
-                }
-            }
-            while (__any(rem != 0u)) {
-                const bool on = rem != 0u;
-                const unsigned e = (unsigned)__builtin_ctz(rem | 0x100u);
-                rem &= rem - 1u;
-                u64 key = t[0][0], val[NV];
-#pragma unroll
-                for (int j = 0; j < NV; j++) val[j] = t[1 + j][0];
-#pragma unroll
-                for (int q = 1; q < 8; q++) {
-                    const bool is = e == (unsigned)q;
-                    key = is ? t[0][q] : key;
-#pragma unroll
-                    for (int j = 0; j < NV; j++) val[j] = is ? t[1 + j][q] : val[j];
-                }
-                place(on, key, val, dbase + (e >> 1) * 128u + (e & 1u));
-            }
-        }
-        flush_queue();
-        if (PL_LD(&L.dead)) alive = false;
-    };
-
-    const i64 nsteps = (r1 - r0 + PL_WROWS - 1) / PL_WROWS;
-    const i64 nfull = (r1 - r0) / PL_WROWS;
-    {
-        u64 va[NC][8];
-        for (i64 s = wv; s < nfull && alive; s += PL_WAVES) {
-            const i64 base = r0 + s * PL_WROWS + lane * 2;
-            if constexpr (NP == 0) {
-#pragma unroll
-                for (int c = 0; c < NC; c++) {
-#pragma unroll
-                    for (int j = 0; j < 4; j++) {
-                        const u64x2 t = rfx_ld2(P.cols[c] + base + j * 128);
-                        va[c][2 * j] = t.x;
-                        va[c][2 * j + 1] = t.y;
-                    }
-                }
-                step(va, 0xffu, base);
-            } else {
-#pragma unroll
-                for (int c = 0; c < NC; c++) {
-                    if ((A.pmask >> c) & 1u) {
-#pragma unroll
-                        for (int j = 0; j < 4; j++) {
-                            const u64x2 t = rfx_ld2(P.cols[c] + base + j * 128);
-                            va[c][2 * j] = t.x;
-                            va[c][2 * j + 1] = t.y;
-                        }
-                    } else {
-#pragma unroll
-                        for (int e = 0; e < 8; e++) va[c][e] = 0;
-                    }
-                }
-                const unsigned m = eval_preds<NC, 8, NP>(S, va, 0xffu);
-#pragma unroll
-                for (int c = 0; c < NC; c++) {
-                    if (!((A.pmask >> c) & 1u)) {
-#pragma unroll
-                        for (int j = 0; j < 4; j++) {
-                            if ((m >> (2 * j)) & 3u) {
-                                const u64x2 t = rfx_ld2(P.cols[c] + base + j * 128);
-                                va[c][2 * j] = t.x;
-                                va[c][2 * j + 1] = t.y;
-                            }
-                        }
-                    }
-                }
-                step(va, m, base);
-            }
-        }
-    }
-    if (nfull < nsteps && (nfull % PL_WAVES) == wv && alive) {
-        u64 va[NC][8];
-        const i64 base = r0 + nfull * PL_WROWS + lane * 2;
-        unsigned valid = 0;
-#pragma unroll
-        for (int e = 0; e < 8; e++) {
-            const i64 row = base + (e >> 1) * 128 + (e & 1);
-            const bool in = row < r1;
-            valid |= (unsigned)in << e;
-#pragma unroll
-            for (int c = 0; c < NC; c++) va[c][e] = in ? P.cols[c][row] : 0ULL;
-        }
-        step(va, (NP == 0) ? valid : eval_preds<NC, 8, NP>(S, va, valid), base);
-    }
-    __syncthreads();
-    if (L.dead) {
-        if (tid == 0) atomicExch(&A.ctl[1], 1u);
-        return;
-    }
-    for (int i = tid; i < PARTS * (NV + 1) * (int)LPD; i += PL_T) {
-        const unsigned sub = (unsigned)i & (LPD - 1u), p = ((unsigned)i / LPD) % (unsigned)PARTS, pl = ((unsigned)i / LPD) / (unsigned)PARTS;
-        const unsigned t = tail[p];
-        if (!(t & (VG - 1u))) continue;
-        const unsigned gi = t >> VGL;
-        if (pl < (unsigned)NV) {
-            const pl_v2 x = *(const pl_v2 *)(vring + ((size_t)pl * PARTS + p) * RING + (gi & 1u) * VG + sub * 2);
-            if constexpr (KVI) {
-                *(pl_v2 *)(A.vals[0] + 2 * (region + (u64)p * A.c0 + (u64)gi * VG) + (u64)pl * VG + sub * 2) = x;
-            } else {
-                u64 *dst = (NV == 1 ? A.vals[0] : (pl == 0 ? A.vals[0] : (pl == 1 ? A.vals[1] : A.vals[2])));
-                *(pl_v2 *)(dst + region + (u64)p * A.c0 + (u64)gi * VG + sub * 2) = x;
-            }
-        } else if (sub < LPD / 2) {
-            const pl_v2 x = *(const pl_v2 *)(mring + (size_t)p * RING + (gi & 1u) * VG + sub * 4);
-            *(pl_v2 *)(A.meta + region + (u64)p * A.c0 + (u64)gi * VG + sub * 4) = x;
-        }
-    }
-    for (int i = tid; i < PARTS; i += PL_T) A.cnt[(size_t)blockIdx.x * PARTS + i] = tail[i];
-    i64 sel = (i64)nsel;
-    for (int s2 = 32; s2 >= 1; s2 >>= 1) {
-        const i64 omn = (i64)rfx_shfl_xor_u64((u64)mn, s2), omx = (i64)rfx_shfl_xor_u64((u64)mx, s2);
-        mn = omn < mn ? omn : mn;
-        mx = omx > mx ? omx : mx;
-        sel += (i64)rfx_shfl_xor_u64((u64)sel, s2);
-    }
-    if (lane == 0) {
-        L.red[0][wv] = mn;
-        L.red[1][wv] = mx;
-        L.red[2][wv] = sel;
-    }
-    __syncthreads();
-    if (tid == 0) {
-        for (int w2 = 1; w2 < PL_WAVES; w2++) {
-            mn = L.red[0][w2] < mn ? L.red[0][w2] : mn;
-            mx = L.red[1][w2] > mx ? L.red[1][w2] : mx;
-            sel += L.red[2][w2];
-        }
-        unsigned long long *g = (unsigned long long *)A.ctl + 8;
-        if (sel > 0) {
-            atomicMax(&g[0], ~((unsigned long long)mn ^ 0x8000000000000000ULL));
-            atomicMax(&g[1], (unsigned long long)mx ^ 0x8000000000000000ULL);
-            atomicAdd(&g[2], (unsigned long long)sel);
-        }
-    }
+    plane_scatter_body<NC, NP, NV, PBITS, VGL, HK, false, 0u>(P, P, A);
 }
 
 struct PlaneAggArgs {
@@ -512,6 +206,7 @@
 static int launch_plane_scatter_inst(rfx_ctx *c, const Plan &P, const PlaneArgs &A) {
     constexpr size_t lds = pl_lds_bytes<NV, PBITS, VGL, HK>();
     static_assert(lds <= 160 * 1024, "rings beyond a CU's LDS");
+    if (rfx_rtc_plane_scatter(c, P, A, PlaneShape{NC, NP, NV, PBITS, VGL, HK ? 1 : 0}, lds) == RFX_OK) return RFX_OK;
     static unsigned long long attr_set = 0;
     if (!((attr_set >> (c->device & 63)) & 1ull)) {
         RFX_HIP_CHECK(hipFuncSetAttribute((const void *)k_plane_scatter<NC, NP, NV, PBITS, VGL, HK>, hipFuncAttributeMaxDynamicSharedMemorySize, (int)lds));
@@ -572,6 +267,71 @@
     return P.nagg >= 1;
 }
 
+static bool plane_plan_cols(const Plan &P, int key_idx, const int *vcol, int nv, Plan *out, unsigned *pmask) {
+    Plan &Pc = *out;
+    Pc = P;
+    int perm[RFX_MAX_COLS + PL_MAX_NV], inv[RFX_MAX_COLS], n2 = 0;
+    for (int i = 0; i < P.ncols; i++) inv[i] = -1;
+    perm[n2++] = key_idx;
+    inv[key_idx] = 0;
+    for (int j = 0; j < nv; j++) {
+        if (inv[vcol[j]] < 0) inv[vcol[j]] = n2;
+        perm[n2++] = vcol[j];
+    }
+    for (int i = 0; i < P.ncols; i++)
+        if (inv[i] < 0) {
+            inv[i] = n2;
+            perm[n2++] = i;
+        }
+    if (n2 > 1 + nv + 2 || n2 > RFX_MAX_COLS) return false;
+    Pc.ncols = n2;
+    for (int i = 0; i < n2; i++) Pc.cols[i] = P.cols[perm[i]];
+    *pmask = 0;
+    for (int i = 0; i < P.npred; i++) {
+        Pc.preds[i].col = inv[P.preds[i].col];
+        if (P.preds[i].rhs_col >= 0) Pc.preds[i].rhs_col = inv[P.preds[i].rhs_col];
+        *pmask |= 1u << Pc.preds[i].col;
+        if (Pc.preds[i].rhs_col >= 0) *pmask |= 1u << Pc.preds[i].rhs_col;
+    }
+    return true;
+}
+static int plane_dense_pbits(const Plan &P, unsigned long long est_range, int nv) {
+    int pbits = 7;
+    static const char *force = getenv("RFX_PLANE_PBITS");
+    const i64 l7 = (i64)((est_range + 127) >> 7);
+    if (l7 + l7 / 16 > (1 << PL_SLOT_BITS) || !plane_agg_fits(P, l7 + l7 / 16)) pbits = 8;
+    if (force && nv == 1) pbits = atoi(force) == 7 ? 7 : 8;
+    return pbits;
+}
+
+static bool plane_hash_plan_cols(const Plan &P, int key_idx, const int *vcol, int nv, Plan *out, unsigned *pmask) {
+    Plan &Pc = *out;
+    Pc = P;
+    int perm[RFX_MAX_COLS + 2], inv[RFX_MAX_COLS], n2 = 0;
+    for (int i = 0; i < P.ncols; i++) inv[i] = -1;
+    perm[n2++] = key_idx;
+    inv[key_idx] = 0;
+    perm[n2++] = key_idx;
+    perm[n2++] = nv == 1 ? vcol[0] : key_idx;
+    if (nv == 1 && inv[vcol[0]] < 0) inv[vcol[0]] = 2;
+    for (int i = 0; i < P.ncols; i++)
+        if (inv[i] < 0) {
+            inv[i] = n2;
+            perm[n2++] = i;
+        }
+    if (n2 > 4 || n2 > RFX_MAX_COLS) return false;
+    Pc.ncols = n2;
+    for (int i = 0; i < n2; i++) Pc.cols[i] = P.cols[perm[i]];
+    *pmask = 0;
+    for (int i = 0; i < P.npred; i++) {
+        Pc.preds[i].col = inv[P.preds[i].col];
+        if (P.preds[i].rhs_col >= 0) Pc.preds[i].rhs_col = inv[P.preds[i].rhs_col];
+        *pmask |= 1u << Pc.preds[i].col;
+        if (Pc.preds[i].rhs_col >= 0) *pmask |= 1u << Pc.preds[i].rhs_col;
+    }
+    return true;
+}
+
 struct PlaneState {
     int valid, npred, logic, nblk, pbits, nv;
     unsigned c0;
@@ -613,13 +373,7 @@
     int vcol[PL_MAX_NV], agg_plane[RFX_MAX_AGGS];
     const int nv = plane_value_cols(P, vcol, agg_plane);
     if (nv < 1 || P.nx > 0) return RFX_ESTATE;
-    int pbits = 7;
-    {
-        static const char *force = getenv("RFX_PLANE_PBITS");
-        const i64 l7 = (i64)((est_range + 127) >> 7);
-        if (l7 + l7 / 16 > (1 << PL_SLOT_BITS) || !plane_agg_fits(P, l7 + l7 / 16)) pbits = 8;
-        if (force && nv == 1) pbits = atoi(force) == 7 ? 7 : 8;
-    }
+    const int pbits = plane_dense_pbits(P, est_range, nv);
     if (pbits == 8 && nv > 1) return RFX_ESTATE;
     const i64 est_local = (i64)((est_range + (1ULL << pbits) - 1) >> pbits);
     if (est_local > (1 << PL_SLOT_BITS) || !plane_agg_fits(P, est_local)) return RFX_ESTATE;
@@ -637,33 +391,8 @@
     if (rfx_chunk_reserve(c, need) != RFX_OK) return RFX_ESTATE;
     plane_layout(c, (int)nblk64, pbits, c0, nv, &A, NULL);
     A.block_rows = PL_BLOCK_ROWS;
-    Plan Pc = P;
-    {
-        int perm[RFX_MAX_COLS + PL_MAX_NV], inv[RFX_MAX_COLS], n2 = 0;
-        for (int i = 0; i < P.ncols; i++) inv[i] = -1;
-        perm[n2++] = key_idx;
-        inv[key_idx] = 0;
-        for (int j = 0; j < nv; j++) {
-            if (inv[vcol[j]] < 0) inv[vcol[j]] = n2;
-            perm[n2++] = vcol[j];
-        }
-        for (int i = 0; i < P.ncols; i++)
-            if (inv[i] < 0) {
-                inv[i] = n2;
-                perm[n2++] = i;
-            }
-        if (n2 > 1 + nv + 2 || n2 > RFX_MAX_COLS) return RFX_ESTATE;
-        Pc.ncols = n2;
-        for (int i = 0; i < n2; i++) Pc.cols[i] = P.cols[perm[i]];
-        for (int i = 0; i < P.npred; i++) {
-            Pc.preds[i].col = inv[P.preds[i].col];
-            if (P.preds[i].rhs_col >= 0) Pc.preds[i].rhs_col = inv[P.preds[i].rhs_col];
-        }
-    }
-    for (int i = 0; i < Pc.npred; i++) {
-        A.pmask |= 1u << Pc.preds[i].col;
-        if (Pc.preds[i].rhs_col >= 0) A.pmask |= 1u << Pc.preds[i].rhs_col;
-    }
+    Plan Pc;
+    if (!plane_plan_cols(P, key_idx, vcol, nv, &Pc, &A.pmask)) return RFX_ESTATE;
     if (getenv("RFX_PLANE_LOAD_ALL")) A.pmask = 0xFFu;
     RFX_HIP_CHECK(hipMemsetAsync(A.ctl, 0, 256, c->stream));
     c->ext_i[3 + RFX_STAT_PLANE_SCATTER]++;
@@ -1196,28 +925,9 @@
     }
     const i64 nblk64 = (nrows + PL_BLOCK_ROWS - 1) / PL_BLOCK_ROWS;
     if (nblk64 > (1 << 20)) return RFX_ESTATE;
-    Plan Pc = P;
-    {
-        int perm[RFX_MAX_COLS + 2], inv[RFX_MAX_COLS], n2 = 0;
-        for (int i = 0; i < P.ncols; i++) inv[i] = -1;
-        perm[n2++] = key_idx;
-        inv[key_idx] = 0;
-        perm[n2++] = key_idx;
-        perm[n2++] = nv == 1 ? vcol[0] : key_idx;
-        if (nv == 1 && inv[vcol[0]] < 0) inv[vcol[0]] = 2;
-        for (int i = 0; i < P.ncols; i++)
-            if (inv[i] < 0) {
-                inv[i] = n2;
-                perm[n2++] = i;
-            }
-        if (n2 > 4 || n2 > RFX_MAX_COLS) return RFX_ESTATE;
-        Pc.ncols = n2;
-        for (int i = 0; i < n2; i++) Pc.cols[i] = P.cols[perm[i]];
-        for (int i = 0; i < P.npred; i++) {
-            Pc.preds[i].col = inv[P.preds[i].col];
-            if (P.preds[i].rhs_col >= 0) Pc.preds[i].rhs_col = inv[P.preds[i].rhs_col];
-        }
-    }
+    Plan Pc;
+    unsigned pmask = 0;
+    if (!plane_hash_plan_cols(P, key_idx, vcol, nv, &Pc, &pmask)) return RFX_ESTATE;
     double share = (double)PL_BLOCK_ROWS / (double)parts;
     unsigned c0 = (unsigned)(share * 1.25 + 160.0);
     c0 = (c0 + 127u) & ~127u;
@@ -1228,10 +938,7 @@
     if (rfx_chunk_reserve(c, need) != RFX_OK) return RFX_ESTATE;
     plane_layout(c, (int)nblk64, pbits, c0, 2, &A, NULL, parts);
     A.block_rows = PL_BLOCK_ROWS;
-    for (int i = 0; i < Pc.npred; i++) {
-        A.pmask |= 1u << Pc.preds[i].col;
-        if (Pc.preds[i].rhs_col >= 0) A.pmask |= 1u << Pc.preds[i].rhs_col;
-    }
+    A.pmask = pmask;
     c->ck_valid = 0;
     rfx_plane_invalidate(c);
     RFX_HIP_CHECK(hipMemsetAsync(A.ctl, 0, 256, c->stream));
@@ -1300,3 +1007,33 @@
     RFX_HIP_CHECK(hipGetLastError());
     return RFX_OK;
 }
+
+static int plane_np_of(int npred) { return npred == 0 ? 0 : (npred == 1 ? 1 : (npred <= 3 ? 3 : RFX_MAX_PREDS)); }
+extern "C" int rfx_hip_rtc_prewarm_plane_scatter(const rfx_pred_t *preds, int npred, int logic, const rfx_agg_t *aggs, int nagg, const void *d_key,
+                                                 int64_t key_range, int sparse_parts) {
+    RFX_REQUIRE(d_key && key_range > 0, RFX_EINVAL, "prewarm_plane_scatter: key column / key range missing");
+    Plan P;
+    int key_idx = -1;
+    int rc = rfx_plan_build(&P, preds, npred, logic, aggs, nagg, d_key, &key_idx, 1LL << 24, 0);
+    if (rc != RFX_OK) return rc;
+    int vcol[PL_MAX_NV], agg_plane[RFX_MAX_AGGS];
+    const int nv = plane_value_cols(P, vcol, agg_plane);
+    if (nv < 0 || P.nx > 0 || key_idx < 0) return RFX_ESTATE;
+    Plan Pc;
+    unsigned pmask = 0;
+    PlaneShape K;
+    if (sparse_parts) {
+        if (nv > 1 || !plane_hash_plan_cols(P, key_idx, vcol, nv, &Pc, &pmask)) return RFX_ESTATE;
+        if (sparse_parts == 192) K = PlaneShape{Pc.ncols, plane_np_of(Pc.npred), 2, 8, 4, 1};
+        else if (sparse_parts == 128) K = PlaneShape{Pc.ncols, plane_np_of(Pc.npred), 2, 7, 4, 1};
+        else if (sparse_parts == 256) K = PlaneShape{Pc.ncols, plane_np_of(Pc.npred), 2, 8, 3, 1};
+        else return RFX_EINVAL;
+    } else {
+        if (nv < 1 || !plane_plan_cols(P, key_idx, vcol, nv, &Pc, &pmask)) return RFX_ESTATE;
+        const int pbits = plane_dense_pbits(P, (unsigned long long)key_range, nv);
+        const int extra = Pc.ncols - 1 - nv;
+        if (extra < 0 || extra > 2 || (nv > 1 && (pbits != 7 || extra > 1))) return RFX_ESTATE;
+        K = PlaneShape{Pc.ncols, plane_np_of(Pc.npred), nv, pbits, nv == 1 ? (pbits == 7 ? 5 : 4) : 4, 0};
+    }
+    return rfx_rtc_plane_scatter_prewarm(Pc, pmask, K);
+}
diff --git a/rayforce_amd/csrc/rfx_group_plane_kernel.hpp b/rayforce_amd/csrc/rfx_group_plane_kernel.hpp
--- /dev/null
+++ b/rayforce_amd/csrc/rfx_group_plane_kernel.hpp
@@ -0,0 +1,361 @@
+#pragma once
+#include "rfx_group_common.hpp"
+
+#define PL_T 1024
+#define PL_WAVES (PL_T / RFX_WAVE)
+#define PL_WROWS 512
+#define PL_BLOCK_ROWS (1 << 18)
+#define PL_DELTA_BITS 18
+#define PL_SLOT_BITS 14
+#define PL_QCAP 320
+#define PL_QFLUSH 24
+#define PL_SPIN_LIMIT (1u << 14)
+#define PL_MAX_NV 3
+#ifndef PL_META64_PLAIN
+#define PL_META64_PLAIN 1
+#endif
+#ifndef PL_ABLATE
+#define PL_ABLATE 0
+#endif
+
+struct PlaneArgs {
+    int nblk;
+    int nv;
+    unsigned pmask;
+    i64 block_rows;
+    unsigned c0;
+    u64 *vals[PL_MAX_NV];
+    unsigned *meta;
+    unsigned *cnt;
+    unsigned *ctl;
+};
+struct PlaneShape {
+    int nc, np, nv, pbits, vgl, hk;
+};
+#ifndef __HIPCC_RTC__
+int rfx_rtc_plane_scatter(rfx_ctx *c, const Plan &P, const PlaneArgs &A, const PlaneShape &K, size_t lds);
+int rfx_rtc_plane_scatter_prewarm(const Plan &P, unsigned pmask, const PlaneShape &K);
+#endif
+struct PlSh {
+    unsigned dead, _pad[3];
+    i64 red[3][PL_WAVES];
+};
+template <int PBITS, int VGL, bool HK>
+__host__ __device__ constexpr int pl_parts() { return (HK && PBITS == 8 && VGL == 4) ? 192 : (1 << PBITS); }
+template <int NV, int PBITS, int VGL, bool HK = false>
+__host__ __device__ constexpr size_t pl_lds_bytes() {
+    return (size_t)pl_parts<PBITS, VGL, HK>() * ((size_t)(2 << VGL) * (NV * 8 + 4) + 8 + 4) + (size_t)PL_WAVES * PL_QCAP * 4 + sizeof(PlSh) + 64;
+}
+typedef u64 pl_v2 __attribute__((ext_vector_type(2)));
+typedef unsigned pl_m2 __attribute__((ext_vector_type(2)));
+#define PL_LD(ptr) __hip_atomic_load((ptr), __ATOMIC_RELAXED, __HIP_MEMORY_SCOPE_WORKGROUP)
+#define PL_ST(ptr, v) __hip_atomic_store((ptr), (v), __ATOMIC_RELAXED, __HIP_MEMORY_SCOPE_WORKGROUP)
+
+__device__ __forceinline__ unsigned long long pl_uniform(u64 x) {
+    return ((unsigned long long)(unsigned)__builtin_amdgcn_readfirstlane((int)(x >> 32)) << 32) | (unsigned)__builtin_amdgcn_readfirstlane((int)x);
+}
+
+template <int NC, int NP, int NV, int PBITS, int VGL, bool HK, bool PLAN, unsigned PMASK>
+__device__ __forceinline__ void plane_scatter_body(const Plan &D, const Plan &P, const PlaneArgs &A) {
+    constexpr int PARTS = pl_parts<PBITS, VGL, HK>();
+    constexpr bool P192 = PARTS != (1 << PBITS);
+    constexpr unsigned VG = 1u << VGL, RING = 2u << VGL;
+    constexpr bool KVI = HK && NV == 2 && PBITS == 8 && VGL == 3;
+    constexpr unsigned LPD = VG / 2;
+    extern __shared__ __attribute__((aligned(16))) unsigned char pl_smem[];
+    u64 *vring = (u64 *)pl_smem;
+    unsigned *mring = (unsigned *)(vring + (size_t)NV * PARTS * RING);
+    unsigned *words = mring + (size_t)PARTS * RING;
+    unsigned *tail = words + PARTS * 2;
+    unsigned *fq = tail + PARTS;
+    PlSh &L = *(PlSh *)(fq + PL_WAVES * PL_QCAP);
+    PredSet<NP> S;
+    predset_load<NP>(D, S);
+    if constexpr (PLAN) {
+#pragma unroll
+        for (int i = 0; i < NP; i++) S.p[i].rhs = P.preds[i].rhs_bits;
+    }
+    const int tid = threadIdx.x, lane = tid & 63, wv = tid >> 6;
+    unsigned *myq = fq + wv * PL_QCAP;
+    const i64 r0 = (i64)blockIdx.x * A.block_rows;
+    const i64 r1 = (r0 + A.block_rows < P.nrows) ? r0 + A.block_rows : P.nrows;
+    const u64 region = ((u64)blockIdx.x * (u64)PARTS) * A.c0;
+    for (int i = tid; i < PARTS; i += PL_T) {
+        tail[i] = 0;
+        words[2 * i] = 0;
+        words[2 * i + 1] = 0;
+    }
+    if (tid == 0) L.dead = 0;
+    __syncthreads();
+    i64 mn = RFX_INF_I64_D, mx = RFX_NULL_I64_D;
+    unsigned nsel = 0;
+    int qn = 0;
+    [[maybe_unused]] u64 abl = 0;
+
+    auto flush_queue = [&]() __attribute__((always_inline)) {
+        asm volatile("" ::: "memory");
+        for (int i0 = 0; i0 < qn; i0 += 64 / (int)LPD) {
+            const int idx = i0 + (lane / (int)LPD);
+            if (idx < qn) {
+                const unsigned d = myq[idx];
+                const unsigned p = d & 0xFFu, gi = (d >> 8) & 0x3FFFFFu, pl = d >> 30, sub = lane & (LPD - 1u);
+                if (pl < 3) {
+                    const pl_v2 x = *(const pl_v2 *)(vring + ((size_t)pl * PARTS + p) * RING + (gi & 1u) * VG + sub * 2);
+                    if constexpr (PL_ABLATE == 3) {
+                        abl ^= x.x ^ x.y;
+                    } else if constexpr (KVI) {
+                        __builtin_nontemporal_store(x, (pl_v2 *)(A.vals[0] + 2 * (region + (u64)p * A.c0 + (u64)gi * VG) + (u64)pl * VG + sub * 2));
+                    } else {
+                        u64 *dst = (NV == 1 ? A.vals[0] : (pl == 0 ? A.vals[0] : (pl == 1 ? A.vals[1] : A.vals[2])));
+                        __builtin_nontemporal_store(x, (pl_v2 *)(dst + region + (u64)p * A.c0 + (u64)gi * VG + sub * 2));
+                    }
+                } else if (sub < LPD / 2) {
+                    const pl_v2 x = *(const pl_v2 *)(mring + (size_t)p * RING + (gi & 1u) * VG + sub * 4);
+                    if constexpr (PL_ABLATE == 3) abl ^= x.x ^ x.y;
+                    else if constexpr (KVI || (VGL == 4 && PL_META64_PLAIN)) *(pl_v2 *)(A.meta + region + (u64)p * A.c0 + (u64)gi * VG + sub * 4) = x;
+                    else __builtin_nontemporal_store(x, (pl_v2 *)(A.meta + region + (u64)p * A.c0 + (u64)gi * VG + sub * 4));
+                }
+            }
+        }
+        asm volatile("" ::: "memory");
+        for (int i = lane; i < qn; i += 64) {
+            const unsigned d = myq[i];
+            if ((d >> 30) == 3u) atomicAdd(&words[2 * (d & 0xFFu) + ((d >> 8) & 1u)], 256u - VG);
+        }
+        qn = 0;
+    };
+
+    auto place = [&](const bool on, const u64 key, const u64 (&val)[NV], const unsigned delta) __attribute__((always_inline)) {
+        const u64 kh = HK ? rfx_hash_index_u64(RFX_U64_HASH_SEED, key) : key;
+        const unsigned p = P192 ? (unsigned)(((kh >> 32) * (u64)PARTS) >> 32) : (HK ? (unsigned)(kh >> (64 - PBITS)) : ((unsigned)key & (unsigned)(PARTS - 1)));
+        unsigned seq = 0;
+        if (on) {
+            const i64 k = (i64)key;
+            mn = k < mn ? k : mn;
+            mx = k > mx ? k : mx;
+            seq = atomicAdd(&tail[p], 1u);
+            if (seq >= A.c0) PL_ST(&L.dead, 1u);
+        }
+        const unsigned g = seq >> VGL;
+        unsigned *w = &words[2 * p + (g & 1u)];
+        bool todo = on && seq < A.c0;
+        for (unsigned it = 0;; it++) {
+            bool ready = false;
+            if (todo) ready = (PL_LD(w) >> 8) == (g >> 1);
+            bool comp = false;
+            if (ready) {
+                const unsigned at = p * RING + (seq & (RING - 1u));
+#pragma unroll
+                for (int j = 0; j < NV; j++) vring[(size_t)j * PARTS * RING + at] = val[j];
+                mring[at] = ((unsigned)(P192 ? (kh >> 18) : (HK ? (kh >> (64 - PBITS - PL_SLOT_BITS)) : (key >> PBITS))) & ((1u << PL_SLOT_BITS) - 1u)) | (delta << PL_SLOT_BITS);
+                asm volatile("" ::: "memory");
+                comp = (atomicAdd(w, 1u) & 0xFFu) == VG - 1u;
+                todo = false;
+            }
+            const u64 cb = __ballot(comp);
+            if (cb) {
+                if (comp) {
+                    const unsigned at = (unsigned)qn + (unsigned)(NV + 1) * __builtin_amdgcn_mbcnt_hi((unsigned)(cb >> 32), __builtin_amdgcn_mbcnt_lo((unsigned)cb, 0u));
+#pragma unroll
+                    for (int j = 0; j < NV; j++) myq[at + j] = p | (g << 8) | ((unsigned)j << 30);
+                    myq[at + NV] = p | (g << 8) | (3u << 30);
+                }
+                qn += (NV + 1) * __popcll(cb);
+            }
+            if (!__any(todo)) break;
+            flush_queue();
+            if (PL_LD(&L.dead) || it > PL_SPIN_LIMIT) {
+                PL_ST(&L.dead, 1u);
+                break;
+            }
+            if (it) __builtin_amdgcn_s_sleep(4);
+        }
+        if (qn >= PL_QFLUSH) flush_queue();
+    };
+
+    bool alive = true;
+    auto step = [&](const u64 (&v)[NC][8], const unsigned m, const i64 sbase) __attribute__((always_inline)) {
+        const unsigned dbase = (unsigned)(sbase - r0);
+        const unsigned valid = m;
+        if constexpr (PL_ABLATE == 1 || PL_ABLATE == 2) {
+            nsel += (unsigned)__popc(m);
+            if constexpr (PL_ABLATE == 2) {
+#pragma unroll
+                for (int c = 0; c < 1 + NV; c++) {
+#pragma unroll
+                    for (int e = 0; e < 8; e++) abl ^= ((m >> e) & 1u) ? v[c][e] : 0ULL;
+                }
+            }
+            return;
+        }
+        if constexpr (NP == 0) {
+            nsel += (unsigned)__popc(valid);
+#pragma unroll
+            for (int e = 0; e < 8; e++) {
+                u64 val[NV];
+#pragma unroll
+                for (int j = 0; j < NV; j++) val[j] = v[1 + j][e];
+                place((valid >> e) & 1u, v[0][e], val, dbase + (unsigned)((e >> 1) * 128 + (e & 1)));
+            }
+        } else {
+            unsigned rem = m;
+            nsel += (unsigned)__popc(rem);
+            u64 t[1 + NV][8];
+#pragma unroll
+            for (int c = 0; c < 1 + NV; c++) {
+#pragma unroll
+                for (int q = 0; q < 8; q++) {
+                    t[c][q] = v[c][q];
+                    if constexpr (NV > 1) asm volatile("" : "+v"(t[c][q]));
+                }
+            }
+            while (__any(rem != 0u)) {
+                const bool on = rem != 0u;
+                const unsigned e = (unsigned)__builtin_ctz(rem | 0x100u);
+                rem &= rem - 1u;
+                u64 key = t[0][0], val[NV];
+#pragma unroll
+                for (int j = 0; j < NV; j++) val[j] = t[1 + j][0];
+#pragma unroll
+                for (int q = 1; q < 8; q++) {
+                    const bool is = e == (unsigned)q;
+                    key = is ? t[0][q] : key;
+#pragma unroll
+                    for (int j = 0; j < NV; j++) val[j] = is ? t[1 + j][q] : val[j];
+                }
+                place(on, key, val, dbase + (e >> 1) * 128u + (e & 1u));
+            }
+        }
+        flush_queue();
+        if (PL_LD(&L.dead)) alive = false;
+    };
+
+    const i64 nsteps = (r1 - r0 + PL_WROWS - 1) / PL_WROWS;
+    const i64 nfull = (r1 - r0) / PL_WROWS;
+    auto load_pred = [&](u64 (&v)[NC][8], const i64 base, const unsigned pmask) __attribute__((always_inline)) {
+#pragma unroll
+        for (int c = 0; c < NC; c++) {
+            if ((pmask >> c) & 1u) {
+#pragma unroll
+                for (int j = 0; j < 4; j++) {
+                    const u64x2 t = rfx_ld2(P.cols[c] + base + j * 128);
+                    v[c][2 * j] = t.x;
+                    v[c][2 * j + 1] = t.y;
+                }
+            } else {
+#pragma unroll
+                for (int e = 0; e < 8; e++) v[c][e] = 0;
+            }
+        }
+    };
+    auto load_rest = [&](u64 (&v)[NC][8], const i64 base, const unsigned pmask, const unsigned m) __attribute__((always_inline)) {
+#pragma unroll
+        for (int c = 0; c < NC; c++) {
+            if (!((pmask >> c) & 1u)) {
+#pragma unroll
+                for (int j = 0; j < 4; j++) {
+                    if ((m >> (2 * j)) & 3u) {
+                        const u64x2 t = rfx_ld2(P.cols[c] + base + j * 128);
+                        v[c][2 * j] = t.x;
+                        v[c][2 * j + 1] = t.y;
+                    }
+                }
+            }
+        }
+    };
+    {
+        u64 va[NC][8];
+        const unsigned pmask = PLAN ? PMASK : A.pmask;
+        for (i64 s = wv; s < nfull && alive; s += PL_WAVES) {
+            const i64 base = r0 + s * PL_WROWS + lane * 2;
+            if constexpr (NP == 0) {
+#pragma unroll
+                for (int c = 0; c < NC; c++) {
+#pragma unroll
+                    for (int j = 0; j < 4; j++) {
+                        const u64x2 t = rfx_ld2(P.cols[c] + base + j * 128);
+                        va[c][2 * j] = t.x;
+                        va[c][2 * j + 1] = t.y;
+                    }
+                }
+                step(va, 0xffu, base);
+            } else {
+                load_pred(va, base, pmask);
+                const unsigned m = eval_preds<NC, 8, NP>(S, va, 0xffu);
+                if constexpr (PL_ABLATE != 1) load_rest(va, base, pmask, m);
+                step(va, m, base);
+            }
+        }
+    }
+    if (nfull < nsteps && (nfull % PL_WAVES) == wv && alive) {
+        u64 va[NC][8];
+        const i64 base = r0 + nfull * PL_WROWS + lane * 2;
+        unsigned valid = 0;
+#pragma unroll
+        for (int e = 0; e < 8; e++) {
+            const i64 row = base + (e >> 1) * 128 + (e & 1);
+            const bool in = row < r1;
+            valid |= (unsigned)in << e;
+#pragma unroll
+            for (int c = 0; c < NC; c++) va[c][e] = in ? P.cols[c][row] : 0ULL;
+        }
+        step(va, (NP == 0) ? valid : eval_preds<NC, 8, NP>(S, va, valid), base);
+    }
+    __syncthreads();
+    if (L.dead) {
+        if (tid == 0) atomicExch(&A.ctl[1], 1u);
+        return;
+    }
+    for (int i = tid; i < PARTS * (NV + 1) * (int)LPD; i += PL_T) {
+        const unsigned sub = (unsigned)i & (LPD - 1u), p = ((unsigned)i / LPD) % (unsigned)PARTS, pl = ((unsigned)i / LPD) / (unsigned)PARTS;
+        const unsigned t = tail[p];
+        if (!(t & (VG - 1u))) continue;
+        const unsigned gi = t >> VGL;
+        if (pl < (unsigned)NV) {
+            const pl_v2 x = *(const pl_v2 *)(vring + ((size_t)pl * PARTS + p) * RING + (gi & 1u) * VG + sub * 2);
+            if constexpr (PL_ABLATE == 3) {
+                abl ^= x.x ^ x.y;
+            } else if constexpr (KVI) {
+                *(pl_v2 *)(A.vals[0] + 2 * (region + (u64)p * A.c0 + (u64)gi * VG) + (u64)pl * VG + sub * 2) = x;
+            } else {
+                u64 *dst = (NV == 1 ? A.vals[0] : (pl == 0 ? A.vals[0] : (pl == 1 ? A.vals[1] : A.vals[2])));
+                *(pl_v2 *)(dst + region + (u64)p * A.c0 + (u64)gi * VG + sub * 2) = x;
+            }
+        } else if (sub < LPD / 2) {
+            const pl_v2 x = *(const pl_v2 *)(mring + (size_t)p * RING + (gi & 1u) * VG + sub * 4);
+            if constexpr (PL_ABLATE == 3) abl ^= x.x ^ x.y;
+            else *(pl_v2 *)(A.meta + region + (u64)p * A.c0 + (u64)gi * VG + sub * 4) = x;
+        }
+    }
+    for (int i = tid; i < PARTS; i += PL_T) A.cnt[(size_t)blockIdx.x * PARTS + i] = tail[i];
+    i64 sel = (i64)nsel;
+    if constexpr (PL_ABLATE != 0) {
+        asm volatile("" : : "v"(nsel), "v"(abl));
+        sel = 0;
+    }
+    for (int s2 = 32; s2 >= 1; s2 >>= 1) {
+        const i64 omn = (i64)rfx_shfl_xor_u64((u64)mn, s2), omx = (i64)rfx_shfl_xor_u64((u64)mx, s2);
+        mn = omn < mn ? omn : mn;
+        mx = omx > mx ? omx : mx;
+        sel += (i64)rfx_shfl_xor_u64((u64)sel, s2);
+    }
+    if (lane == 0) {
+        L.red[0][wv] = mn;
+        L.red[1][wv] = mx;
+        L.red[2][wv] = sel;
+    }
+    __syncthreads();
+    if (tid == 0) {
+        for (int w2 = 1; w2 < PL_WAVES; w2++) {
+            mn = L.red[0][w2] < mn ? L.red[0][w2] : mn;
+            mx = L.red[1][w2] > mx ? L.red[1][w2] : mx;
+            sel += L.red[2][w2];
+        }
+        unsigned long long *g = (unsigned long long *)A.ctl + 8;
+        if (sel > 0) {
+            atomicMax(&g[0], pl_uniform(~((u64)mn ^ 0x8000000000000000ULL)));
+            atomicMax(&g[1], pl_uniform((u64)mx ^ 0x8000000000000000ULL));
+            atomicAdd(&g[2], pl_uniform((u64)sel));
+        }
+    }
+}
diff --git a/rayforce_amd/csrc/rfx_rtc.hip b/rayforce_amd/csrc/rfx_rtc.hip
--- a/rayforce_amd/csrc/rfx_rtc.hip
+++ b/rayforce_amd/csrc/rfx_rtc.hip
@@ -9,6 +9,7 @@
 #include <string>
 #include "rfx_group_common.hpp"
 #include "rfx_where_once_kernel.hpp"
+#include "rfx_group_plane_kernel.hpp"
 #include "build/rfx_rtc_headers.inc"
 
 typedef struct _hiprtcProgram *rtcProgram;
@@ -347,6 +348,63 @@
     __atomic_fetch_add(&g_launches, 1, __ATOMIC_RELAXED);
     return RFX_OK;
 }
+static void plane_scatter_text(const Plan &P, unsigned pmask, const PlaneShape &K, std::string &sig, std::string &src) {
+    char head[384];
+    int n = snprintf(head, sizeof(head), "#define PLS_NC %d\n#define PLS_NP %d\n#define PLS_NV %d\n#define PLS_PBITS %d\n#define PLS_VGL %d\n#define PLS_HK %s\n#define PLS_PMASK %uu\n", K.nc, K.np,
+                     K.nv, K.pbits, K.vgl, K.hk ? "true" : "false", pmask);
+    if (const char *e = getenv("RFX_PLANE_ABLATE"))
+        if (atoi(e) >= 1 && atoi(e) <= 3) n += snprintf(head + n, sizeof(head) - (size_t)n, "#define PL_ABLATE %d\n", atoi(e));
+    Plan Q = P;
+    Q.nagg = 0;
+    Q.nx = 0;
+    std::string cond;
+    plan_text(Q, NULL, cond);
+    sig = std::string("//plane_scatter\n") + head + cond;
+    src = sig +
+          "#include \"rfx_group_plane_kernel.hpp\"\n"
+          "extern \"C\" __global__ __launch_bounds__(PL_T) void k_plane_scatter_plan(const Plan P0, const PlaneArgs A) {\n"
+          "    constexpr Plan D = RTC_PLAN;\n"
+          "    plane_scatter_body<PLS_NC, PLS_NP, PLS_NV, PLS_PBITS, PLS_VGL, PLS_HK, true, PLS_PMASK>(D, P0, A);\n"
+          "}\n";
+}
+int rfx_rtc_plane_scatter(rfx_ctx *c, const Plan &P, const PlaneArgs &A, const PlaneShape &K, size_t lds) {
+    if (c->flags & RFX_TUNE_NO_RTC) return RFX_ESTATE;
+    if (const char *e = getenv("RFX_PLANE_NO_PLAN"))
+        if (e[0] && strcmp(e, "0") != 0) return RFX_ESTATE;
+    if (!rtc_ready()) return RFX_ESTATE;
+    std::string sig, src;
+    plane_scatter_text(P, A.pmask, K, sig, src);
+    const long long before = g_compiles;
+    hipFunction_t fn = plan_kernel(c->device, sig, src, "k_plane_scatter_plan", P.nrows, "a plane scatter kernel for this plan");
+    rfx_ext(c)->plane_plan_compiles += g_compiles - before;
+    if (!fn) return RFX_ESTATE;
+    Plan Pv = P;
+    PlaneArgs Av = A;
+    void *args[] = {&Pv, &Av};
+    RFX_HIP_CHECK(hipModuleLaunchKernel(fn, (unsigned)A.nblk, 1, 1, PL_T, 1, 1, (unsigned)lds, c->stream, args, NULL));
+    __atomic_fetch_add(&g_launches, 1, __ATOMIC_RELAXED);
+    rfx_ext(c)->plane_plan_launches++;
+    return RFX_OK;
+}
+int rfx_rtc_plane_scatter_prewarm(const Plan &P, unsigned pmask, const PlaneShape &K) {
+    if (!rtc_ready() || R.cache_dir.empty()) return RFX_ESTATE;
+    std::string sig, src, code;
+    plane_scatter_text(P, pmask, K, sig, src);
+    if (const char *dump = getenv("RFX_RTC_DUMP")) {
+        char fn[512];
+        snprintf(fn, sizeof(fn), "%s/k_plane_scatter_plan_%zx.hip", dump, std::hash<std::string>()(src));
+        if (FILE *f = fopen(fn, "w")) {
+            fwrite(src.data(), 1, src.size(), f);
+            fclose(f);
+        }
+    }
+    const std::string path = cache_path(src);
+    if (read_code(path, code)) return RFX_OK;
+    std::lock_guard<std::mutex> hold(g_rtc_lock);
+    if (!compile(src, code)) return RFX_ESTATE;
+    write_code(path, code);
+    return read_code(path, code) ? RFX_OK : RFX_ESTATE;
+}
 extern "C" int rfx_hip_rtc_prewarm_where(const rfx_pred_t *preds, int npred, int logic) {
     Plan P;
     int rc = rfx_plan_build(&P, preds, npred, logic, NULL, 0, NULL, NULL, 1, 0);
diff --git a/rayforce_amd/prewarm.py b/rayforce_amd/prewarm.py
--- a/rayforce_amd/prewarm.py
+++ b/rayforce_amd/prewarm.py
@@ -56,6 +56,17 @@
     return lib.rfx_hip_rtc_prewarm_filter_aggr(parr, npred, logic, aarr, len(aggs)) == L.RFX_OK
 
 
+def plane_scatter(where, aggs: Sequence[Tuple[str, Optional[str]]], by: str, types: Dict[str, str], key_range: int, sparse_parts: int = 0) -> bool:
+    lib = L.load_library()
+    ident = {name: 4096 * (i + 1) for i, name in enumerate(types)}
+    parr, npred, logic = _preds(where, types, ident)
+    aarr = (L.Agg * max(1, len(aggs)))()
+    for a, (fn, col) in zip(aarr, aggs):
+        a.kind = L.AGGS[fn]
+        a.d_col, a.col_type = (ident[col], _TYPES[types[col]]) if col is not None else (None, L.RFX_I64)
+    return lib.rfx_hip_rtc_prewarm_plane_scatter(parr, npred, logic, aarr, len(aggs), ident[by], int(key_range), int(sparse_parts)) == L.RFX_OK
+
+
 BASELINE_PLANS = {
     "c1": (None, [("sum", "v")], {"v": "f64"}),
     "c2": (("<", "a", 100_000), [("sum", "a")], {"a": "i64"}),
@@ -70,9 +81,17 @@
 }
 
 
+PLANE_PLANS = {
+    "c3w": (("<", "a", 100_000), [("sum", "v")], "k", {"k": "i64", "v": "f64", "a": "i64"}, 1_000_000, 0),
+    "c3": (None, [("sum", "v")], "k", {"k": "i64", "v": "f64"}, 1_000_000, 0),
+    "k9": (None, [("sum", "v")], "k", {"k": "i64", "v": "f64"}, 1_000_000, 256),
+}
+
+
 def baseline() -> Dict[str, bool]:
     done = {name: filter_aggr(*plan) for name, plan in BASELINE_PLANS.items()}
     done.update({name: where(*plan) for name, plan in WHERE_PLANS.items()})
+    done.update({name + ":scatter": plane_scatter(*plan) for name, plan in PLANE_PLANS.items()})
     return done
 
 
```
